# better62/MM-VQA-Healthcare

Measured on AMD Instinct MI355X. Metric: image-question pairs/sec, M3AE-base fine-tune step (fwd+bwd+AdamW) @384px, higher is better.
Workload: dtype bf16

## Files before the change

include/m3ae_hip.h:

```cpp
#ifndef M3AE_HIP_H
#define M3AE_HIP_H

#include <stdint.h>

#ifdef __cplusplus
extern "C" {
#endif

#define M3AE_ABI_VERSION 4

enum { M3AE_F32 = 0, M3AE_BF16 = 1 };
enum { M3AE_ACT_NONE = 0, M3AE_ACT_GELU = 1, M3AE_ACT_QUICKGELU = 2, M3AE_ACT_TANH = 3, M3AE_ACT_RELU = 4,
       M3AE_ACT_MULAUX = 5  };
enum { M3AE_ERR_ARG = -1, M3AE_ERR_UNSUPPORTED = -2, M3AE_ERR_ALIGN = -3, M3AE_ERR_WORKSPACE = -4 };

int m3ae_abi_version(void);
void m3ae_desc_sizes(int64_t out3[3]);
const char* m3ae_last_gemm_path(void);

typedef struct {
    int64_t M, N, K;
    int64_t batch1, batch2;
    const void* A; int64_t a_sm, a_sk, a_sb1, a_sb2;
    const void* B; int64_t b_sk, b_sn, b_sb1, b_sb2;
    void* C;       int64_t c_sm, c_sn, c_sb1, c_sb2;
    int32_t dtype_a, dtype_b, dtype_c;
    float alpha;
    int32_t accumulate;
    const float* bias;
    int32_t act;
    void* preact;
    const void* residual;
    const void* dact_aux;
    int32_t dact;
    int32_t force_generic;
    float* a_rowsum;
    float dropout_p;
    uint64_t dropout_seed;
    int32_t preact_grad;
    int32_t launch_flags;
    const void* dropout_salt;
} m3ae_gemm_desc;
enum { M3AE_GEMM_NO_PERSISTENT = 1,
       M3AE_GEMM_F32_X3 = 2,
       M3AE_GEMM_DETERMINISTIC = 4  };
#define M3AE_GEMM_NT_VARIANT(v) ((((v) + 1) & 0xf) << 8)
#define M3AE_GEMM_TN_VARIANT(v) ((((v) + 1) & 0xf) << 12)
#define M3AE_GEMM_COL_GROUP(g) (((g) & 0xf) << 16)
int m3ae_gemm(const m3ae_gemm_desc* d, void* stream);
int m3ae_gemm_rows(const m3ae_gemm_desc* d, int64_t row_base, int64_t row_step, void* stream);
int64_t m3ae_gemm_det_workspace_bytes(const m3ae_gemm_desc* d);
int m3ae_gemm_det(const m3ae_gemm_desc* d, void* workspace, int64_t workspace_bytes, void* stream);

typedef struct {
    int64_t B, H, Lq, Lk, Dh;
    const void* q; int64_t q_sb, q_sl;
    const void* k; int64_t k_sb, k_sl;
    const void* v; int64_t v_sb, v_sl;
    void* o;       int64_t o_sb, o_sl;
    const float* key_mask;
    const float* pos_bias;
    float scale;
    int32_t causal;
    float* lse; int64_t lse_stride;
    int32_t dtype;
    void* workspace; int64_t workspace_bytes;
    const void* d_o;
    void* dq; void* dk; void* dv;
    float* delta;
    float* d_pos_bias;
    float dropout_p;
    uint64_t dropout_seed;
    const void* dropout_salt;
    int32_t launch_flags;
} m3ae_attn_desc;
enum { M3AE_ATTN_LEGACY_KERNELS = 1,
       M3AE_ATTN_F32_X3 = 2    };
int64_t m3ae_attn_workspace_bytes(const m3ae_attn_desc* d, int backward);
int m3ae_attn_fwd(const m3ae_attn_desc* d, void* stream);
int m3ae_attn_bwd(const m3ae_attn_desc* d, void* stream);
int m3ae_attn_fwd_rows(const m3ae_attn_desc* d, int64_t row_base, int64_t row_step, void* stream);
int m3ae_attn_bwd_rows(const m3ae_attn_desc* d, int64_t row_base, int64_t row_step, void* stream);
int m3ae_attn_probs(const m3ae_attn_desc* d, float* probs, int64_t p_sb, int64_t p_sh, int64_t p_sq, void* stream);

typedef struct {
    int32_t dir;
    int64_t B, Lq, Lk, D, H;
    const void* x;
    const void* y;
    const float* key_mask;
    const void *wq, *wq_t, *wkv, *wkv_t, *wo, *wo_t;
    const float *bq, *bkv, *bo, *ln_g, *ln_b;
    float ln_eps;
    float dropout_p;
    uint64_t seed_attn, seed_hidden;
    void* proj;
    void* prime;
    float* colbias;
    void* probs;
    void* probs_drop;
    float* rowsum;
    void* zctx;
    void* ctx;
    void* s;
    void* out;
    float *mean, *rstd;
    const void* d_out;
    void* dx;
    void* dy;
    float *g_wq, *g_wkv, *g_wo, *g_bq, *g_bkv, *g_bo, *g_ln_g, *g_ln_b;
    void* ws_ds;
    void* ws_dsd;
    void* ws_dscores;
    void* ws_dprime;
    void* ws_dproj;
    void* ws_dz;
    void* ws_dctx;
    float* ws_vec;
    float* ws_ln;
    int32_t launch_flags;
    const void* dropout_salt;
} m3ae_xattn_desc;
enum { M3AE_XATTN_NO_PERSISTENT = 1,
       M3AE_XATTN_LEGACY_CHAIN = 2     };
int m3ae_xattn_supported(const m3ae_xattn_desc* d);
int m3ae_xattn_bwd_supported(const m3ae_xattn_desc* d);
int64_t m3ae_xattn_probs_ld(const m3ae_xattn_desc* d);
int m3ae_xattn_fwd(const m3ae_xattn_desc* d, void* stream);
int m3ae_xattn_bwd(const m3ae_xattn_desc* d, void* stream);
int m3ae_xattn_probs_export(const m3ae_xattn_desc* d, int dropped, float* out, int64_t o_sb, int64_t o_sh, int64_t o_sq,
                            void* stream);

int m3ae_layernorm_fwd(const void* x, const float* gamma, const float* beta, void* y, float* mean, float* rstd,
                       int64_t M, int64_t D, float eps, int dtype, int act, int rms, void* stream);
int64_t m3ae_layernorm_bwd_blocks(int64_t M);
int m3ae_layernorm_bwd(const void* dy, const void* x, const float* gamma, const float* beta, const float* mean,
                       const float* rstd, void* dx, const void* dx_add, float* dgamma, float* dbeta, float* workspace,
                       int64_t M, int64_t D, int dtype, int act, int rms, void* stream);
int m3ae_layernorm_bwd_drop(const void* dy, const void* x, const float* gamma, const float* beta, const float* mean,
                            const float* rstd, void* dx, void* dx_drop, float dropout_p, uint64_t dropout_seed,
                            const void* dropout_salt, float* dgamma, float* dbeta, float* workspace, int64_t M, int64_t D,
                            int dtype, void* stream);
int m3ae_layernorm_bwd_drop_rows(const void* dy, const void* x, const float* gamma, const float* beta, const float* mean,
                                 const float* rstd, void* dx, void* dx_drop, float dropout_p, uint64_t dropout_seed,
                                 const void* dropout_salt, float* dgamma, float* dbeta, float* workspace, int64_t M, int64_t D,
                                 int dtype, int64_t row_base, int64_t row_step, void* stream);
int m3ae_layernorm_fwd_mixed(const float* x, const float* gamma, const float* beta, void* y, float* mean, float* rstd,
                             int64_t M, int64_t D, float eps, void* stream);
int m3ae_layernorm_bwd_mixed(const void* dy, const float* x, const float* gamma, const float* mean, const float* rstd,
                             float* dx, const float* dx_add, void* dx_lo, float* dgamma, float* dbeta, float* workspace,
                             int64_t M, int64_t D, void* stream);
int m3ae_layernorm_bwd_mixed_det(const void* dy, const float* x, const float* gamma, const float* mean, const float* rstd,
                                 float* dx, const float* dx_add, void* dx_lo, float* dgamma, float* dbeta, float* workspace,
                                 int64_t M, int64_t D, void* stream);
int m3ae_dropout(const void* x, void* out, uint8_t* keep_mask, int64_t rows, int64_t cols, float p, uint64_t seed,
                 const void* salt, int dtype, void* stream);
int m3ae_dropout_rows(const void* x, void* out, uint8_t* keep_mask, int64_t rows, int64_t cols, float p, uint64_t seed,
                      const void* salt, int dtype, int64_t row_base, int64_t row_step, void* stream);

int m3ae_colsum(const void* x, float* out, int64_t M, int64_t N, int64_t ldx, int dtype, int accumulate,
                void* stream);

int m3ae_roberta_embed_fwd(const int64_t* ids, const float* word, const float* pos, const float* type, void* out,
                           int64_t B, int64_t S, int64_t D, int64_t pad_id, int dtype, void* stream);
int m3ae_roberta_embed_bwd(const int64_t* ids, const void* d_out, float* d_word, float* d_pos, float* d_type,
                           int64_t B, int64_t S, int64_t D, int64_t pad_id, int dtype, void* stream);

int m3ae_patchify(const float* img, void* out, int64_t B, int64_t R, int64_t P, int dtype, void* stream);
int m3ae_image_normalize_u8(const uint8_t* in, float* out, int64_t B, int64_t H, int64_t W, const float* mean3,
                            const float* std3, void* stream);
int64_t m3ae_image_resample_workspace_bytes(int64_t total_rows, int64_t size);
int m3ae_image_resample_u8(const uint8_t* src, int64_t src_bytes, const int64_t* plan, const int32_t* tab, int64_t tab_ints, int64_t B,
                           int64_t size, uint8_t* workspace, int64_t workspace_bytes, float* out, uint8_t* out_u8,
                           const float* mean3, const float* std3, void* stream);
int m3ae_vit_tokens_fwd(const void* patch, const float* cls, const float* pos, void* out, int64_t B, int64_t G,
                        int64_t D, int dtype, void* stream);
int m3ae_vit_tokens_bwd(const void* d_out, void* d_patch, float* d_cls, float* d_pos, int64_t B, int64_t G,
                        int64_t D, int dtype, void* stream);

int m3ae_bce_logits(const void* logits, const float* targets, float* loss, void* d_logits, int64_t B, int64_t C,
                    float grad_scale, int dtype, void* stream);
int m3ae_xent(const void* logits, const int64_t* labels, float* loss, void* d_logits, float* workspace,
              int64_t rows, int64_t C, int64_t ld, float grad_scale, int dtype, void* stream);

int m3ae_adamw(float* p, const float* g, float* m, float* v, void* shadow_bf16, int64_t n, float lr, float beta1,
               float beta2, float eps, float wd, int64_t step, float grad_scale, const float* hyper_dev, void* stream);

int m3ae_cast_transpose(const float* in, void* out, void* out_t, int64_t R, int64_t C, void* stream);
int m3ae_cast_transpose_batched(const void* jobs_dev, int njobs, int64_t total_tiles, void* stream);
int m3ae_transpose_bf16_batched(const void* jobs_dev, int njobs, int64_t total_tiles, void* stream);
int m3ae_cast(const void* in, void* out, int64_t n, int dtype_in, int dtype_out, void* stream);
int m3ae_zero(void* p, int64_t bytes, void* stream);
int m3ae_add(const void* a, const void* b, void* out, int64_t n, int dtype, void* stream);
int m3ae_act_fwd(const void* x, void* y, int64_t n, int act, int dtype, void* stream);
int m3ae_act_bwd(const void* dy, const void* x_pre, void* dx, int64_t n, int act, int dtype, void* stream);
int m3ae_gather_rows(const void* in, const int64_t* idx, void* out, int64_t n_out, int64_t D, int dtype,
                     void* stream);
int m3ae_scatter_add_rows(const void* d_out, const int64_t* idx, void* d_in, int64_t n_out, int64_t D, int dtype,
                          void* stream);

int m3ae_mask_ranks(const float* noise, int64_t* ids_restore, int64_t* keep_rows, float* mask, int64_t B, int64_t L,
                    int64_t len_keep, void* stream);
int m3ae_mim_targets(const float* img, float* out, int64_t B, int64_t C, int64_t H, int64_t W, int64_t P, int norm_pix,
                     void* stream);
int m3ae_mim_loss_fwd(const void* x, const float* target, const float* mask, float* acc, float* loss, int64_t B, int64_t L,
                      int64_t D, int dtype, void* stream);
int m3ae_mim_loss_bwd(const void* x, const float* target, const float* mask, const float* acc, const float* gout, void* dx,
                      int64_t B, int64_t L, int64_t D, int dtype, void* stream);

enum { M3AE_DET_COLSUM = 0, M3AE_DET_EMBED_BWD = 1, M3AE_DET_BCE = 2, M3AE_DET_XENT = 3, M3AE_DET_MIM = 4 };
int64_t m3ae_det_workspace_bytes(int op, int64_t rows, int64_t cols);
int m3ae_colsum_det(const void* x, float* out, int64_t M, int64_t N, int64_t ldx, int dtype, int accumulate, void* workspace,
                    int64_t workspace_bytes, void* stream);
int m3ae_layernorm_bwd_det(const void* dy, const void* x, const float* gamma, const float* beta, const float* mean,
                           const float* rstd, void* dx, const void* dx_add, float* dgamma, float* dbeta, float* workspace,
                           int64_t M, int64_t D, int dtype, int act, int rms, void* stream);
int m3ae_layernorm_bwd_drop_det(const void* dy, const void* x, const float* gamma, const float* beta, const float* mean,
                                const float* rstd, void* dx, void* dx_drop, float dropout_p, uint64_t dropout_seed,
                                const void* dropout_salt, float* dgamma, float* dbeta, float* workspace, int64_t M, int64_t D,
                                int dtype, void* stream);
int m3ae_roberta_embed_bwd_det(const int64_t* ids, const void* d_out, float* d_word, float* d_pos, float* d_type, int64_t B,
                               int64_t S, int64_t D, int64_t pad_id, int dtype, void* workspace, int64_t workspace_bytes,
                               void* stream);
int m3ae_bce_logits_det(const void* logits, const float* targets, float* loss, void* d_logits, int64_t B, int64_t C,
                        float grad_scale, int dtype, void* workspace, int64_t workspace_bytes, void* stream);
int m3ae_xent_det(const void* logits, const int64_t* labels, float* loss, void* d_logits, int64_t rows, int64_t C, int64_t ld,
                  float grad_scale, int dtype, void* workspace, int64_t workspace_bytes, void* stream);
int m3ae_mim_loss_fwd_det(const void* x, const float* target, const float* mask, float* acc, float* loss, int64_t B, int64_t L,
                          int64_t D, int dtype, void* workspace, int64_t workspace_bytes, void* stream);

int64_t m3ae_beam_topk_workspace_bytes(int64_t B, int64_t nb, int64_t V, int64_t chunk);
int m3ae_beam_topk(const float* logits, int64_t ld, const float* beam_scores, int64_t B, int64_t nb, int64_t V, int64_t chunk,
                   void* workspace, int64_t workspace_bytes, float* top_s, int32_t* top_i, void* stream);
int m3ae_beam_step(const float* top_s, const int32_t* top_i, const int64_t* ids_in, int64_t* ids_out, int64_t* last_tok,
                   float* beam_scores, int64_t* order, int32_t* done, int32_t* n_hyp, double* hyp_score, int32_t* hyp_len,
                   int64_t* hyp_tok, int32_t* open_count, int64_t* err, int64_t B, int64_t nb, int64_t V, int64_t max_length,
                   int64_t cur_len, int64_t eos, int64_t pad, double div, void* stream);
int m3ae_beam_finalize(const int64_t* ids, const float* beam_scores, const int32_t* done, int32_t* n_hyp, double* hyp_score,
                       int32_t* hyp_len, int64_t* hyp_tok, int64_t* seq, int64_t* len, int64_t B, int64_t nb, int64_t max_length,
                       int64_t cur_len, int64_t eos, int64_t pad, double div, void* stream);

int m3ae_expand_samples(const void* in, const int64_t* src, void* out, int64_t n_out, int64_t n_in, int64_t R, int dtype,
                        void* stream);
int m3ae_segment_sum_rows(const void* d_out, const int64_t* offsets, const int64_t* members, void* d_in, int64_t n_in,
                          int64_t n_out, int64_t R, int dtype, void* stream);

int m3ae_selftest(int32_t* out, void* stream);

#ifdef __cplusplus
}
#endif
#endif
```

mm-vqa-healthcare_amd/csrc/norm.hip:

```cpp
#include "common.h"
#include "det_fold.h"
#include "launch.h"
#include <type_traits>

namespace {

template <typename T> DEVINL void ld4(const T* p, float* x);
template <> DEVINL void ld4<float>(const float* p, float* x) {
    const f32x4 v = *(const f32x4*)p;
    x[0] = v[0]; x[1] = v[1]; x[2] = v[2]; x[3] = v[3];
}
template <> DEVINL void ld4<bf16_t>(const bf16_t* p, float* x) {
    const u32x2 v = *(const u32x2*)p;
    x[0] = __uint_as_float(v[0] << 16); x[1] = __uint_as_float(v[0] & 0xffff0000u);
    x[2] = __uint_as_float(v[1] << 16); x[3] = __uint_as_float(v[1] & 0xffff0000u);
}
template <typename T> struct Raw4;
template <> struct Raw4<float> {
    f32x4 v;
    DEVINL void ld(const float* p) { v = *(const f32x4*)p; }
    DEVINL void get(float* x) const { x[0] = v[0]; x[1] = v[1]; x[2] = v[2]; x[3] = v[3]; }
};
template <> struct Raw4<bf16_t> {
    u32x2 v;
    DEVINL void ld(const bf16_t* p) { v = *(const u32x2*)p; }
    DEVINL void get(float* x) const {
        x[0] = __uint_as_float(v[0] << 16); x[1] = __uint_as_float(v[0] & 0xffff0000u);
        x[2] = __uint_as_float(v[1] << 16); x[3] = __uint_as_float(v[1] & 0xffff0000u);
    }
};
template <typename T> DEVINL void st4(T* p, const float* x);
template <> DEVINL void st4<float>(float* p, const float* x) { *(f32x4*)p = (f32x4){x[0], x[1], x[2], x[3]}; }
template <> DEVINL void st4<bf16_t>(bf16_t* p, const float* x) {
    *(u32x2*)p = (u32x2){pack2bf(x[0], x[1]), pack2bf(x[2], x[3])};
}

template <typename T, int CPL, typename TO = T>
__global__ __launch_bounds__(256) void ln_fwd_kernel(const T* x, const float* gamma, const float* beta, TO* y,
                                                     float* mean_o, float* rstd_o, int64_t M, int D, float eps,
                                                     int act, int rms) {
    const int lane = threadIdx.x & 63;
    const int nch = D >> 2;
    const int64_t stride = (int64_t)gridDim.x * 4;
    int64_t row = (int64_t)blockIdx.x * 4 + (threadIdx.x >> 6);
    Raw4<T> raw[CPL];
    if (row < M) {
#pragma unroll
        for (int c = 0; c < CPL; ++c) {
            const int ch = lane + c * 64;
            if (ch < nch) raw[c].ld(x + row * D + ch * 4);
        }
    }
    for (; row < M; row += stride) {
        float v[CPL][4];
        float sum = 0.f;
#pragma unroll
        for (int c = 0; c < CPL; ++c) {
            const int ch = lane + c * 64;
            if (ch < nch) {
                raw[c].get(v[c]);
                sum += (v[c][0] + v[c][1]) + (v[c][2] + v[c][3]);
            } else {
                v[c][0] = v[c][1] = v[c][2] = v[c][3] = 0.f;
            }
        }
        const int64_t nrow = row + stride;
        if (nrow < M) {
#pragma unroll
            for (int c = 0; c < CPL; ++c) {
                const int ch = lane + c * 64;
                if (ch < nch) raw[c].ld(x + nrow * D + ch * 4);
            }
        }
        const float mean = rms ? 0.f : wave_sum(sum) / (float)D;
        float sq = 0.f;
#pragma unroll
        for (int c = 0; c < CPL; ++c) {
            const int ch = lane + c * 64;
            if (ch < nch) {
#pragma unroll
                for (int t = 0; t < 4; ++t) {
                    const float dlt = v[c][t] - mean;
                    sq += dlt * dlt;
                }
            }
        }
        const float var = wave_sum(sq) / (float)D;
        const float rstd = 1.0f / sqrtf(var + eps);
        if (lane == 0) {
            if (mean_o) mean_o[row] = mean;
            if (rstd_o) rstd_o[row] = rstd;
        }
        TO* yr = y + row * D;
#pragma unroll
        for (int c = 0; c < CPL; ++c) {
            const int ch = lane + c * 64;
            if (ch < nch) {
                float g[4], b[4] = {0.f, 0.f, 0.f, 0.f}, o[4];
                ld4<float>(gamma + ch * 4, g);
                if (beta) ld4<float>(beta + ch * 4, b);
#pragma unroll
                for (int t = 0; t < 4; ++t) o[t] = act_fwd((v[c][t] - mean) * rstd * g[t] + b[t], act);
                st4<TO>(yr + ch * 4, o);
            }
        }
    }
}

template <int NP>
__global__ __launch_bounds__(256) void ln_fwd_pair_kernel(const bf16_t* x, const float* gamma, const float* beta, bf16_t* y,
                                                          float* mean_o, float* rstd_o, int64_t M, float eps) {
    constexpr int D = NP * 256, PPR = D / 8;
    const int lane = threadIdx.x & 63;
    const int64_t npair = (M + 1) >> 1;
    const int64_t stride = (int64_t)gridDim.x * 4;
    int64_t pr = (int64_t)blockIdx.x * 4 + (threadIdx.x >> 6);
    int sel[NP], col[NP];
#pragma unroll
    for (int c = 0; c < NP; ++c) {
        const int p = lane + 64 * c;
        sel[c] = p >= PPR;
        col[c] = (p - sel[c] * PPR) * 8;
    }
    u32x4 raw[NP];
    auto load = [&](int64_t pair) {
        const bf16_t* base = x + pair * 2 * D;
        const bool two = pair * 2 + 1 < M;
#pragma unroll
        for (int c = 0; c < NP; ++c)
            raw[c] = (two || !sel[c]) ? *(const u32x4*)(base + (lane + 64 * c) * 8) : (u32x4){0u, 0u, 0u, 0u};
    };
    if (pr < npair) load(pr);
    for (; pr < npair; pr += stride) {
        float v[NP][8];
        float s0 = 0.f, s1 = 0.f;
#pragma unroll
        for (int c = 0; c < NP; ++c) {
            float t = 0.f;
#pragma unroll
            for (int q = 0; q < 4; ++q) {
                v[c][2 * q] = __uint_as_float(raw[c][q] << 16);
                v[c][2 * q + 1] = __uint_as_float(raw[c][q] & 0xffff0000u);
                t += v[c][2 * q] + v[c][2 * q + 1];
            }
            if (sel[c]) s1 += t; else s0 += t;
        }
        const int64_t cur = pr;
        if (pr + stride < npair) load(pr + stride);
        const float m0 = wave_sum(s0) / (float)D, m1 = wave_sum(s1) / (float)D;
        float q0 = 0.f, q1 = 0.f;
#pragma unroll
        for (int c = 0; c < NP; ++c) {
            const float mu = sel[c] ? m1 : m0;
            float t = 0.f;
#pragma unroll
            for (int e = 0; e < 8; ++e) { const float dlt = v[c][e] - mu; t += dlt * dlt; }
            if (sel[c]) q1 += t; else q0 += t;
        }
        const float r0 = 1.0f / sqrtf(wave_sum(q0) / (float)D + eps), r1 = 1.0f / sqrtf(wave_sum(q1) / (float)D + eps);
        const bool two = cur * 2 + 1 < M;
        if (lane == 0) {
            if (mean_o) { mean_o[cur * 2] = m0; if (two) mean_o[cur * 2 + 1] = m1; }
            if (rstd_o) { rstd_o[cur * 2] = r0; if (two) rstd_o[cur * 2 + 1] = r1; }
        }
        bf16_t* yb = y + cur * 2 * D;
#pragma unroll
        for (int c = 0; c < NP; ++c) {
            if (!two && sel[c]) continue;
            const float mu = sel[c] ? m1 : m0, rs = sel[c] ? r1 : r0;
            const f32x4 g0 = *(const f32x4*)(gamma + col[c]), g1 = *(const f32x4*)(gamma + col[c] + 4);
            f32x4 b0 = {0.f, 0.f, 0.f, 0.f}, b1 = {0.f, 0.f, 0.f, 0.f};
            if (beta) { b0 = *(const f32x4*)(beta + col[c]); b1 = *(const f32x4*)(beta + col[c] + 4); }
            float o[8];
#pragma unroll
            for (int e = 0; e < 4; ++e) {
                o[e] = (v[c][e] - mu) * rs * g0[e] + b0[e];
                o[4 + e] = (v[c][4 + e] - mu) * rs * g1[e] + b1[e];
            }
            *(u32x4*)(yb + (lane + 64 * c) * 8) = (u32x4){pack2bf(o[0], o[1]), pack2bf(o[2], o[3]), pack2bf(o[4], o[5]), pack2bf(o[6], o[7])};
        }
    }
}

template <typename T, int CPL, bool ACT, typename TD = T>
__global__ __launch_bounds__(256) void ln_bwd_kernel(const TD* dy, const T* x, const float* gamma, const float* beta,
                                                     const float* mean_i, const float* rstd_i, T* dx, const T* dx_add,
                                                     float* part, int64_t M, int D, int act, int rms, T* dx_drop,
                                                     DropState drop, bf16_t* dx_lo) {
    if (dx_drop) drop_resolve(drop);
    extern __shared__ float red[];
    const int lane = threadIdx.x & 63, wave = threadIdx.x >> 6;
    const int nch = D >> 2;
    float dg[CPL][4], db[CPL][4], g[CPL][4], bt[ACT ? CPL : 1][4];
#pragma unroll
    for (int c = 0; c < CPL; ++c) {
        const int ch = lane + c * 64;
#pragma unroll
        for (int t = 0; t < 4; ++t) { dg[c][t] = 0.f; db[c][t] = 0.f; g[c][t] = 0.f; if (ACT) bt[c][t] = 0.f; }
        if (ch < nch) {
            ld4<float>(gamma + ch * 4, g[c]);
            if (ACT && beta) ld4<float>(beta + ch * 4, bt[c]);
        }
    }
    const int64_t stride = (int64_t)gridDim.x * 4;
    int64_t row = (int64_t)blockIdx.x * 4 + wave;
    Raw4<T> xr[CPL];
    Raw4<TD> dr[CPL];
    float mean_n = 0.f, rstd_n = 0.f;
    if (row < M) {
#pragma unroll
        for (int c = 0; c < CPL; ++c) {
            const int ch = lane + c * 64;
            if (ch < nch) { xr[c].ld(x + row * D + ch * 4); dr[c].ld(dy + row * D + ch * 4); }
        }
        mean_n = rms ? 0.f : mean_i[row];
        rstd_n = rstd_i[row];
    }
    for (; row < M; row += stride) {
        const float mean = mean_n;
        const float rstd = rstd_n;
        float xh[CPL][4], dxh[CPL][4];
        float s1 = 0.f, s2 = 0.f;
#pragma unroll
        for (int c = 0; c < CPL; ++c) {
            const int ch = lane + c * 64;
            if (ch < nch) {
                float xv[4], dv[4];
                xr[c].get(xv);
                dr[c].get(dv);
#pragma unroll
                for (int t = 0; t < 4; ++t) {
                    const float h = (xv[t] - mean) * rstd;
                    float d = dv[t];
                    if (ACT) d *= act_bwd(h * g[c][t] + bt[c][t], act);
                    dg[c][t] += d * h;
                    db[c][t] += d;
                    const float dh = d * g[c][t];
                    xh[c][t] = h;
                    dxh[c][t] = dh;
                    s1 += dh;
                    s2 += dh * h;
                }
            } else {
#pragma unroll
                for (int t = 0; t < 4; ++t) { xh[c][t] = 0.f; dxh[c][t] = 0.f; }
            }
        }
        const int64_t nrow = row + stride;
        if (nrow < M) {
#pragma unroll
            for (int c = 0; c < CPL; ++c) {
                const int ch = lane + c * 64;
                if (ch < nch) { xr[c].ld(x + nrow * D + ch * 4); dr[c].ld(dy + nrow * D + ch * 4); }
            }
            mean_n = rms ? 0.f : mean_i[nrow];
            rstd_n = rstd_i[nrow];
        }
        const float c1 = rms ? 0.f : wave_sum(s1) / (float)D;
        const float c2 = wave_sum(s2) / (float)D;
#pragma unroll
        for (int c = 0; c < CPL; ++c) {
            const int ch = lane + c * 64;
            if (ch < nch) {
                float o[4];
#pragma unroll
                for (int t = 0; t < 4; ++t) o[t] = rstd * (dxh[c][t] - c1 - xh[c][t] * c2);
                if (dx_drop) {
                    float od[4];
#pragma unroll
                    for (int t = 0; t < 4; ++t) od[t] = o[t];
                    drop_apply4(drop, (uint64_t)(drop_row(drop, row) * D + ch * 4), od);
                    st4<T>(dx_drop + row * D + ch * 4, od);
                }
                if (dx_add) {
                    float e[4];
                    ld4<T>(dx_add + row * D + ch * 4, e);
#pragma unroll
                    for (int t = 0; t < 4; ++t) o[t] += e[t];
                }
                st4<T>(dx + row * D + ch * 4, o);
                if constexpr (!std::is_same<TD, T>::value) {
                    if (dx_lo) st4<bf16_t>(dx_lo + row * D + ch * 4, o);
                }
            }
        }
    }
#pragma unroll
    for (int c = 0; c < CPL; ++c) {
        const int ch = lane + c * 64;
        if (ch < nch) {
#pragma unroll
            for (int t = 0; t < 4; ++t) {
                red[(wave * 2 + 0) * D + ch * 4 + t] = dg[c][t];
                red[(wave * 2 + 1) * D + ch * 4 + t] = db[c][t];
            }
        }
    }
    __syncthreads();
    for (int i = threadIdx.x; i < 2 * D; i += 256) {
        const int which = i / D, col = i - which * D;
        float s = 0.f;
#pragma unroll
        for (int w = 0; w < 4; ++w) s += red[(w * 2 + which) * D + col];
        part[((int64_t)blockIdx.x * 2 + which) * D + col] = s;
    }
}

__global__ __launch_bounds__(256) void ln_bwd_reduce_kernel(const float* part, float* dgamma, float* dbeta, int nblk,
                                                            int D) {
    __shared__ float red[8][33];
    const int cl = threadIdx.x & 31, rl = threadIdx.x >> 5;
    const int i = blockIdx.x * 32 + cl;
    const int b0 = blockIdx.y * 64;
    const int b1 = b0 + 64 < nblk ? b0 + 64 : nblk;
    float s = 0.f;
    if (i < 2 * D) {
        const int which = i / D, col = i - which * D;
        for (int b = b0 + rl; b < b1; b += 8) s += part[((int64_t)b * 2 + which) * D + col];
    }
    red[rl][cl] = s;
    __syncthreads();
    if (rl == 0 && i < 2 * D) {
        float t = 0.f;
#pragma unroll
        for (int r = 0; r < 8; ++r) t += red[r][cl];
        const int which = i / D, col = i - which * D;
        if (which == 0) atomicAdd(dgamma + col, t);
        else if (dbeta) atomicAdd(dbeta + col, t);
    }
}

inline int ln_bwd_fold(const float* part, float* dgamma, float* dbeta, int nblk, int D, int det, hipStream_t s) {
    if (det)
        det_fold(part, dgamma, dbeta, nblk, dbeta ? 2 * D : D, 2 * D, D, 1.0f, 1, s);
    else
        hipLaunchKernelGGL(ln_bwd_reduce_kernel, dim3((unsigned)cdiv(2 * D, 32), (unsigned)cdiv(nblk, 64)), dim3(256), 0, s, part, dgamma,
                           dbeta, nblk, D);
    return hip_launch_status();
}

template <typename K> int resident_blocks(K kernel, size_t lds) {
    int per_cu = 0;
    if (hipOccupancyMaxActiveBlocksPerMultiprocessor(&per_cu, kernel, 256, lds) != hipSuccess || per_cu <= 0) return 1 << 30;
    return per_cu * device_cus();
}
template <typename T, int CPL, typename TO = T>
int launch_fwd(const void* x, const float* g, const float* b, void* y, float* mean, float* rstd, int64_t M, int D,
               float eps, int act, int rms, hipStream_t s) {
    static const int cap = resident_blocks(ln_fwd_kernel<T, CPL, TO>, 0);
    const int64_t want = cdiv(M, 4);
    hipLaunchKernelGGL((ln_fwd_kernel<T, CPL, TO>), dim3((unsigned)(want < cap ? want : cap)), dim3(256), 0, s, (const T*)x, g, b,
                       (TO*)y, mean, rstd, M, D, eps, act, rms);
    return hip_launch_status();
}
template <typename T, int CPL, typename TD = T>
int launch_bwd(const void* dy, const void* x, const float* g, const float* b, const float* mean, const float* rstd,
               void* dx, const void* dx_add, float* part, int* nblk_io, int64_t M, int D, int act, int rms, hipStream_t s,
               void* dx_drop = nullptr, DropState drop = DropState{}, void* dx_lo = nullptr) {
    const size_t lds = (size_t)8 * D * sizeof(float);
    static int cap_act = 0, cap_plain = 0, cap_d = -1;
    constexpr bool MIXED = !std::is_same<TD, T>::value;
    if (cap_d != D) {
        if constexpr (!MIXED) cap_act = resident_blocks(ln_bwd_kernel<T, CPL, true, TD>, lds);
        cap_plain = resident_blocks(ln_bwd_kernel<T, CPL, false, TD>, lds);
        cap_d = D;
    }
    const int cap = act != M3AE_ACT_NONE ? cap_act : cap_plain;
    const int nblk = *nblk_io < cap ? *nblk_io : cap;
    *nblk_io = nblk;
    if constexpr (MIXED) {
        if (act != M3AE_ACT_NONE) return M3AE_ERR_UNSUPPORTED;
    }
    if (act != M3AE_ACT_NONE) {
        if constexpr (!MIXED)
            hipLaunchKernelGGL((ln_bwd_kernel<T, CPL, true, TD>), dim3((unsigned)nblk), dim3(256), lds, s,
                               (const TD*)dy, (const T*)x, g, b, mean, rstd, (T*)dx, (const T*)dx_add, part, M, D, act, rms,
                               (T*)dx_drop, drop, (bf16_t*)dx_lo);
    } else
        hipLaunchKernelGGL((ln_bwd_kernel<T, CPL, false, TD>), dim3((unsigned)nblk), dim3(256), lds, s,
                           (const TD*)dy, (const T*)x, g, b, mean, rstd, (T*)dx, (const T*)dx_add, part, M, D, act, rms,
                           (T*)dx_drop, drop, (bf16_t*)dx_lo);
    return hip_launch_status();
}

template <typename T, int CPL>
int launch_fwd_mixed(const void* x, const float* g, const float* b, void* y, float* mean, float* rstd, int64_t M, int D, float eps,
                     hipStream_t s) {
    return launch_fwd<T, CPL, bf16_t>(x, g, b, y, mean, rstd, M, D, eps, M3AE_ACT_NONE, 0, s);
}
template <typename T, int CPL>
int launch_bwd_mixed(const void* dy, const void* x, const float* g, const float* mean, const float* rstd, void* dx, const void* dx_add,
                     void* dx_lo, float* part, int* nblk_io, int64_t M, int D, hipStream_t s) {
    return launch_bwd<T, CPL, bf16_t>(dy, x, g, nullptr, mean, rstd, dx, dx_add, part, nblk_io, M, D, M3AE_ACT_NONE, 0, s, nullptr,
                                      DropState{}, dx_lo);
}

#define DISPATCH_CPL(FN, T, ...)                                                  \
    do {                                                                          \
        const int cpl = (int)cdiv(D / 4, 64);                                     \
        if (cpl <= 1) return FN<T, 1>(__VA_ARGS__);                               \
        if (cpl <= 2) return FN<T, 2>(__VA_ARGS__);                               \
        if (cpl <= 3) return FN<T, 3>(__VA_ARGS__);                               \
        if (cpl <= 4) return FN<T, 4>(__VA_ARGS__);                               \
        if (cpl <= 6) return FN<T, 6>(__VA_ARGS__);                               \
        if (cpl <= 8) return FN<T, 8>(__VA_ARGS__);                               \
        if (cpl <= 16) return FN<T, 16>(__VA_ARGS__);                             \
        return M3AE_ERR_UNSUPPORTED;                                              \
    } while (0)

}

template <int NP>
int launch_fwd_pair(const void* x, const float* g, const float* b, void* y, float* mean, float* rstd, int64_t M, float eps,
                    hipStream_t s) {
    static const int cap = resident_blocks(ln_fwd_pair_kernel<NP>, 0);
    const int64_t want = cdiv((M + 1) / 2, 4);
    hipLaunchKernelGGL((ln_fwd_pair_kernel<NP>), dim3((unsigned)(want < cap ? want : cap)), dim3(256), 0, s, (const bf16_t*)x, g, b,
                       (bf16_t*)y, mean, rstd, M, eps);
    return hip_launch_status();
}

extern "C" int m3ae_layernorm_fwd(const void* x, const float* gamma, const float* beta, void* y, float* mean,
                                  float* rstd, int64_t M, int64_t D, float eps, int dtype, int act, int rms,
                                  void* stream) {
    if (!x || !gamma || !y || M <= 0 || D <= 0) return M3AE_ERR_ARG;
    if (D % 4 != 0 || D > 4096) return M3AE_ERR_UNSUPPORTED;
    hipStream_t s = (hipStream_t)stream;
    const bool pair_off = (rms & 2) != 0;
    rms &= 1;
    if (dtype == M3AE_BF16 && act == M3AE_ACT_NONE && !rms && M >= 1024 && ((((uintptr_t)x) | ((uintptr_t)y)) & 15) == 0 &&
        ((((uintptr_t)gamma) | ((uintptr_t)beta)) & 15) == 0 && !pair_off) {
        if (D == 512) return launch_fwd_pair<2>(x, gamma, beta, y, mean, rstd, M, eps, s);
        if (D == 768) return launch_fwd_pair<3>(x, gamma, beta, y, mean, rstd, M, eps, s);
        if (D == 1024) return launch_fwd_pair<4>(x, gamma, beta, y, mean, rstd, M, eps, s);
    }
    if (dtype == M3AE_F32) DISPATCH_CPL(launch_fwd, float, x, gamma, beta, y, mean, rstd, M, (int)D, eps, act, rms, s);
    if (dtype == M3AE_BF16) DISPATCH_CPL(launch_fwd, bf16_t, x, gamma, beta, y, mean, rstd, M, (int)D, eps, act, rms, s);
    return M3AE_ERR_UNSUPPORTED;
}

extern "C" int64_t m3ae_layernorm_bwd_blocks(int64_t M) {
    int64_t n = cdiv(M, 4);
    return n < 1024 ? n : 1024;
}

static int layernorm_bwd_impl(const void* dy, const void* x, const float* gamma, const float* beta, const float* mean,
                              const float* rstd, void* dx, const void* dx_add, float* dgamma, float* dbeta, float* workspace,
                              int64_t M, int64_t D, int dtype, int act, int rms, void* stream, int det) {
    if (!dy || !x || !gamma || !rstd || !dx || !workspace || M <= 0) return M3AE_ERR_ARG;
    if (D % 4 != 0 || D > 2048) return M3AE_ERR_UNSUPPORTED;
    hipStream_t s = (hipStream_t)stream;
    int nblk = (int)m3ae_layernorm_bwd_blocks(M);
    int rc = M3AE_ERR_UNSUPPORTED;
    auto run = [&]() -> int {
        if (dtype == M3AE_F32)
            DISPATCH_CPL(launch_bwd, float, dy, x, gamma, beta, mean, rstd, dx, dx_add, workspace, &nblk, M, (int)D, act, rms, s);
        if (dtype == M3AE_BF16)
            DISPATCH_CPL(launch_bwd, bf16_t, dy, x, gamma, beta, mean, rstd, dx, dx_add, workspace, &nblk, M, (int)D, act, rms, s);
        return M3AE_ERR_UNSUPPORTED;
    };
    rc = run();
    if (rc) return rc;
    if (!dgamma) return 0;
    return ln_bwd_fold(workspace, dgamma, dbeta, nblk, (int)D, det, s);
}
extern "C" int m3ae_layernorm_bwd(const void* dy, const void* x, const float* gamma, const float* beta,
                                  const float* mean, const float* rstd, void* dx, const void* dx_add, float* dgamma,
                                  float* dbeta, float* workspace, int64_t M, int64_t D, int dtype, int act, int rms,
                                  void* stream) {
    return layernorm_bwd_impl(dy, x, gamma, beta, mean, rstd, dx, dx_add, dgamma, dbeta, workspace, M, D, dtype, act, rms, stream, 0);
}
extern "C" int m3ae_layernorm_bwd_det(const void* dy, const void* x, const float* gamma, const float* beta,
                                      const float* mean, const float* rstd, void* dx, const void* dx_add, float* dgamma,
                                      float* dbeta, float* workspace, int64_t M, int64_t D, int dtype, int act, int rms,
                                      void* stream) {
    return layernorm_bwd_impl(dy, x, gamma, beta, mean, rstd, dx, dx_add, dgamma, dbeta, workspace, M, D, dtype, act, rms, stream, 1);
}

static int layernorm_bwd_drop_impl(const void* dy, const void* x, const float* gamma, const float* beta, const float* mean,
                                   const float* rstd, void* dx, void* dx_drop, float dropout_p, uint64_t dropout_seed,
                                   const void* dropout_salt, float* dgamma, float* dbeta, float* workspace, int64_t M, int64_t D,
                                   int dtype, void* stream, int det, DropRows rows = DropRows{0, 1}) {
    if (!dy || !x || !gamma || !rstd || !dx || !dx_drop || !workspace || M <= 0) return M3AE_ERR_ARG;
    if (!drop_rows_ok(rows, M, D)) return M3AE_ERR_ARG;
    if (D % 4 != 0 || D > 2048) return M3AE_ERR_UNSUPPORTED;
    hipStream_t s = (hipStream_t)stream;
    int nblk = (int)m3ae_layernorm_bwd_blocks(M);
    const DropState drop = make_drop(dropout_p, dropout_seed, dropout_salt, rows);
    auto run = [&]() -> int {
        if (dtype == M3AE_F32)
            DISPATCH_CPL(launch_bwd, float, dy, x, gamma, beta, mean, rstd, dx, nullptr, workspace, &nblk, M, (int)D, 0, 0, s, dx_drop, drop);
        if (dtype == M3AE_BF16)
            DISPATCH_CPL(launch_bwd, bf16_t, dy, x, gamma, beta, mean, rstd, dx, nullptr, workspace, &nblk, M, (int)D, 0, 0, s, dx_drop, drop);
        return M3AE_ERR_UNSUPPORTED;
    };
    int rc = run();
    if (rc) return rc;
    if (!dgamma) return 0;
    return ln_bwd_fold(workspace, dgamma, dbeta, nblk, (int)D, det, s);
}
extern "C" int m3ae_layernorm_bwd_drop(const void* dy, const void* x, const float* gamma, const float* beta,
                                       const float* mean, const float* rstd, void* dx, void* dx_drop, float dropout_p,
                                       uint64_t dropout_seed, const void* dropout_salt, float* dgamma, float* dbeta,
                                       float* workspace, int64_t M, int64_t D, int dtype, void* stream) {
    return layernorm_bwd_drop_impl(dy, x, gamma, beta, mean, rstd, dx, dx_drop, dropout_p, dropout_seed, dropout_salt, dgamma, dbeta,
                                   workspace, M, D, dtype, stream, 0);
}
extern "C" int m3ae_layernorm_bwd_drop_rows(const void* dy, const void* x, const float* gamma, const float* beta,
                                            const float* mean, const float* rstd, void* dx, void* dx_drop, float dropout_p,
                                            uint64_t dropout_seed, const void* dropout_salt, float* dgamma, float* dbeta,
                                            float* workspace, int64_t M, int64_t D, int dtype, int64_t row_base, int64_t row_step,
                                            void* stream) {
    return layernorm_bwd_drop_impl(dy, x, gamma, beta, mean, rstd, dx, dx_drop, dropout_p, dropout_seed, dropout_salt, dgamma, dbeta,
                                   workspace, M, D, dtype, stream, 0, DropRows{row_base, row_step});
}
extern "C" int m3ae_layernorm_bwd_drop_det(const void* dy, const void* x, const float* gamma, const float* beta,
                                           const float* mean, const float* rstd, void* dx, void* dx_drop, float dropout_p,
                                           uint64_t dropout_seed, const void* dropout_salt, float* dgamma, float* dbeta,
                                           float* workspace, int64_t M, int64_t D, int dtype, void* stream) {
    return layernorm_bwd_drop_impl(dy, x, gamma, beta, mean, rstd, dx, dx_drop, dropout_p, dropout_seed, dropout_salt, dgamma, dbeta,
                                   workspace, M, D, dtype, stream, 1);
}

extern "C" int m3ae_layernorm_fwd_mixed(const float* x, const float* gamma, const float* beta, void* y, float* mean, float* rstd,
                                        int64_t M, int64_t D, float eps, void* stream) {
    if (!x || !gamma || !y || M <= 0 || D <= 0) return M3AE_ERR_ARG;
    if (D % 4 != 0 || D > 2048) return M3AE_ERR_UNSUPPORTED;
    if (((((uintptr_t)x) | ((uintptr_t)gamma) | ((uintptr_t)beta)) & 15) != 0 || (((uintptr_t)y) & 7) != 0) return M3AE_ERR_ALIGN;
    hipStream_t s = (hipStream_t)stream;
    DISPATCH_CPL(launch_fwd_mixed, float, x, gamma, beta, y, mean, rstd, M, (int)D, eps, s);
}

static int layernorm_bwd_mixed_impl(const void* dy, const float* x, const float* gamma, const float* mean, const float* rstd,
                                    float* dx, const float* dx_add, void* dx_lo, float* dgamma, float* dbeta, float* workspace,
                                    int64_t M, int64_t D, void* stream, int det) {
    if (!dy || !x || !gamma || !mean || !rstd || !dx || !workspace || M <= 0) return M3AE_ERR_ARG;
    if (D % 4 != 0 || D > 2048) return M3AE_ERR_UNSUPPORTED;
    if (((((uintptr_t)x) | ((uintptr_t)dx) | ((uintptr_t)dx_add) | ((uintptr_t)gamma)) & 15) != 0 ||
        ((((uintptr_t)dy) | ((uintptr_t)dx_lo)) & 7) != 0)
        return M3AE_ERR_ALIGN;
    hipStream_t s = (hipStream_t)stream;
    int nblk = (int)m3ae_layernorm_bwd_blocks(M);
    auto run = [&]() -> int {
        DISPATCH_CPL(launch_bwd_mixed, float, dy, x, gamma, mean, rstd, dx, dx_add, dx_lo, workspace, &nblk, M, (int)D, s);
    };
    int rc = run();
    if (rc) return rc;
    if (!dgamma) return 0;
    return ln_bwd_fold(workspace, dgamma, dbeta, nblk, (int)D, det, s);
}
extern "C" int m3ae_layernorm_bwd_mixed(const void* dy, const float* x, const float* gamma, const float* mean, const float* rstd,
                                        float* dx, const float* dx_add, void* dx_lo, float* dgamma, float* dbeta, float* workspace,
                                        int64_t M, int64_t D, void* stream) {
    return layernorm_bwd_mixed_impl(dy, x, gamma, mean, rstd, dx, dx_add, dx_lo, dgamma, dbeta, workspace, M, D, stream, 0);
}
extern "C" int m3ae_layernorm_bwd_mixed_det(const void* dy, const float* x, const float* gamma, const float* mean, const float* rstd,
                                            float* dx, const float* dx_add, void* dx_lo, float* dgamma, float* dbeta,
                                            float* workspace, int64_t M, int64_t D, void* stream) {
    return layernorm_bwd_mixed_impl(dy, x, gamma, mean, rstd, dx, dx_add, dx_lo, dgamma, dbeta, workspace, M, D, stream, 1);
}
```

mm-vqa-healthcare_amd/csrc/xattn.hip:

```cpp
#include "xattn_common.h"
#include "launch.h"

namespace {

enum { FORM_K = 0, FORM_T = 1 };
enum { XE_STORE = 0, XE_DENSE = 1, XE_SOFTMAX32 = 2, XE_SOFTMAXROW = 3, XE_ATOMIC = 4, XE_DSOFT = 5 };

struct XgArgs {
    const bf16_t* A; int64_t lda, a_sb;
    const bf16_t* B; int64_t ldb, b_sb;
    int M, N, K;
    int tiles_m, tiles_n;
    bf16_t* C; int64_t ldc, c_sb;
    bf16_t* C2;
    int rdiv, rmul;
    float alpha;
    const float* bias; int64_t bias_sb;
    const float* rowscale; int64_t rs_sm, rs_sb;
    int rs_div, rs_mul;
    int b_rows;
    const bf16_t* residual;
    const float* colbias; int64_t cb_sb;
    float* rowsum_out;
    int n_valid;
// ... 827 lines not shown
            u32x4 v[4];
#pragma unroll
            for (int u = 0; u < 4; ++u) v[u] = *(const u32x4*)(p + (int64_t)(i + 16 * u) * R);
#pragma unroll
            for (int u = 0; u < 4; ++u) add(v[u]);
        }
        for (; i < I; i += 16) add(*(const u32x4*)(p + (int64_t)i * R));
    }
#pragma unroll
    for (int t = 0; t < 8; ++t) part[rl][cg][t] = acc[t];
    __syncthreads();
    if (rl == 0 && n0 < R) {
#pragma unroll
        for (int t = 0; t < 8; ++t) {
            float s_ = 0.f;
#pragma unroll
            for (int r = 0; r < 16; ++r) s_ += part[r][cg][t];
            out[(int64_t)b * R + n0 + t] = scale * s_;
        }
    }
}

__global__ __launch_bounds__(256) void xattn_headvec_kernel(const float* w, const bf16_t* X, int64_t ldx, float* out, int Mrows,
                                                            int T, int R, int w_t, int w_h, int dh) {
    __shared__ float part[256];
    const int h = blockIdx.x, d = threadIdx.x % dh, sub = threadIdx.x / dh, nsub = 256 / dh;
    const int r0 = blockIdx.y * 256, r1 = r0 + 256 < Mrows ? r0 + 256 : Mrows;
    float acc = 0.f;
    if (sub < nsub)
        for (int m = r0 + sub; m < r1; m += nsub) {
            const float wt = w ? w[(int64_t)(m / T) * R + (m % T) * w_t + h * w_h] : 1.0f;
            acc = fmaf(wt, bf2f(X[(int64_t)m * ldx + h * dh + d]), acc);
        }
    part[threadIdx.x] = acc;
    __syncthreads();
    if (sub == 0) {
        for (int q = 1; q < nsub; ++q) acc += part[q * dh + d];
        atomicAdd(out + h * dh + d, acc);
    }
}

__global__ __launch_bounds__(256) void xattn_rowdot_kernel(const bf16_t* dZ, const bf16_t* Z, const bf16_t* dctx, const float* bv,
                                                           const float* rowsum, float* delta, float* radd, int64_t rows, int D,
                                                           int T, int H, int dh) {
    const int lane = threadIdx.x & 63;
    const int64_t row = (int64_t)blockIdx.x * 4 + (threadIdx.x >> 6);
    if (row >= rows) return;
    const bf16_t* a = dZ + row * D;
    const bf16_t* z = Z + row * D;
    float acc = 0.f;
    for (int c = lane * 8; c < D; c += 512) {
        const u32x4 x = *(const u32x4*)(a + c), y = *(const u32x4*)(z + c);
#pragma unroll
        for (int q = 0; q < 4; ++q) {
            acc = fmaf(__uint_as_float(x[q] << 16), __uint_as_float(y[q] << 16), acc);
            acc = fmaf(__uint_as_float(x[q] & 0xffff0000u), __uint_as_float(y[q] & 0xffff0000u), acc);
        }
    }
    acc = wave_sum(acc);
    float ra = 0.f;
    if (radd) {
        const int R = T * H, r = (int)(row % R), b = (int)(row / R), t = r / H, h = r % H;
        float s_ = 0.f;
        for (int d = lane; d < dh; d += 64) s_ = fmaf(bf2f(dctx[((int64_t)b * T + t) * D + h * dh + d]), bv[h * dh + d], s_);
        ra = wave_sum(s_);
    }
    if (lane == 0) {
        if (radd) radd[row] = ra;
        delta[row] = acc + (radd ? ra * rowsum[row] : 0.f);
    }
}

}

#ifdef M3AE_XG_TRACE
extern "C" int m3ae_xg_trace_dump(uint64_t* host_out) {
    g_trace_next = 0;
    return (int)hipMemcpyFromSymbol(host_out, HIP_SYMBOL(g_xg_trace), sizeof(uint64_t) * 8 * 16 * 4096);
}
#endif

extern "C" int m3ae_xattn_supported(const m3ae_xattn_desc* d) {
    if (!d) return 0;
    const int64_t T = d->dir == 0 ? d->Lq : d->Lk, I = d->dir == 0 ? d->Lk : d->Lq;
    if (d->H <= 0 || d->D % d->H != 0) return 0;
    const int64_t dh = d->D / d->H;
    if (I < 1 || dh % 32 != 0 || d->D % 128 != 0) return 0;
    if (d->dir == 0) return ((T == 32 || T == 64) && I <= 640) ? 1 : 0;
    if (d->launch_flags & M3AE_XATTN_LEGACY_CHAIN) return (T == 32 && I <= 640) ? 1 : 0;
    return ((T == 32 || T == 64) && d->H * T == (T == 32 ? 384 : 768) && d->D % 256 == 0) ? 1 : 0;
}

extern "C" int m3ae_xattn_bwd_supported(const m3ae_xattn_desc* d) {
    if (!m3ae_xattn_supported(d)) return 0;
    return 1;
}

extern "C" int64_t m3ae_xattn_probs_ld(const m3ae_xattn_desc* d) {
    return d->dir == 0 ? 640 : d->H * d->Lk;
}

#define XCHK(e) do { const int rc_ = (e); if (rc_ != 0) return rc_; } while (0)

namespace {
m3ae_gemm_desc dense_desc(const m3ae_xattn_desc& d, const void* A, const void* B, void* C) {
    m3ae_gemm_desc g{};
    g.batch1 = g.batch2 = 1;
    g.dtype_a = g.dtype_b = g.dtype_c = M3AE_BF16;
    g.alpha = 1.0f;
    g.launch_flags = (d.launch_flags & M3AE_XATTN_NO_PERSISTENT) ? M3AE_GEMM_NO_PERSISTENT : 0;
    g.A = A; g.B = B; g.C = C; g.c_sn = 1;
    return g;
}
int64_t text_rows(const m3ae_xattn_desc& d) { return d.B * (d.dir == 0 ? d.Lq : d.Lk); }
m3ae_gemm_desc dense_fwd(const m3ae_xattn_desc& d, int64_t N, const void* X, const void* W, const float* bias, void* Y) {
    m3ae_gemm_desc g = dense_desc(d, X, W, Y);
    g.M = text_rows(d); g.N = N; g.K = d.D;
    g.a_sm = d.D; g.a_sk = 1; g.b_sk = 1; g.b_sn = d.D; g.c_sm = N; g.bias = bias;
    return g;
}
m3ae_gemm_desc dense_wgrad(const m3ae_xattn_desc& d, int64_t N, const void* dY, const void* X, float* dW, float* db) {
    m3ae_gemm_desc g = dense_desc(d, dY, X, dW);
    g.M = N; g.N = d.D; g.K = text_rows(d);
    g.a_sm = 1; g.a_sk = N; g.b_sk = d.D; g.b_sn = 1; g.c_sm = d.D; g.dtype_c = M3AE_F32; g.accumulate = 1; g.a_rowsum = db;
    return g;
}
m3ae_gemm_desc dense_dgrad(const m3ae_xattn_desc& d, int64_t K, const void* dY, const void* Wt, void* dX, const void* residual = nullptr) {
    m3ae_gemm_desc g = dense_desc(d, dY, Wt, dX);
    g.M = text_rows(d); g.N = d.D; g.K = K;
    g.a_sm = K; g.a_sk = 1; g.b_sk = 1; g.b_sn = K; g.c_sm = d.D; g.residual = residual;
    return g;
}
}

extern "C" int m3ae_xattn_fwd(const m3ae_xattn_desc* dp, void* stream) {
    if (!dp || !m3ae_xattn_supported(dp)) return M3AE_ERR_UNSUPPORTED;
    const m3ae_xattn_desc& d = *dp;
    hipStream_t s = (hipStream_t)stream;
    const int B = (int)d.B, H = (int)d.H, D = (int)d.D, dh = D / H;
    const int Lq = (int)d.Lq, Lk = (int)d.Lk;
    const float scale = 1.0f / sqrtf((float)dh);
    const bool drop = d.dropout_p > 0.f;
    if (!d.x || !d.y || !d.proj || !d.prime || !d.s || !d.out) return M3AE_ERR_ARG;
    if (d.dir == 0 && (!d.probs || (drop && !d.probs_drop))) return M3AE_ERR_ARG;

    const DropState drop_attn = make_drop(d.dropout_p, d.seed_attn, d.dropout_salt);
    const DropState drop_hidden = make_drop(d.dropout_p, d.seed_hidden, d.dropout_salt);

    if (d.dir == 0) {
        const int T = Lq, I = Lk, R = T * H;
        if (!d.zctx || !d.ctx || (drop && !d.rowsum)) return M3AE_ERR_ARG;
        const m3ae_gemm_desc g = dense_fwd(d, D, d.x, d.wq, d.bq, d.proj);
        XCHK(m3ae_gemm(&g, stream));
        {
            XgArgs a{};
            a.A = (const bf16_t*)d.proj; a.lda = D; a.a_sb = dh;
            a.B = (const bf16_t*)d.wkv_t; a.ldb = 2 * D; a.b_sb = dh;
            a.M = B * T; a.N = D; a.K = dh;
            a.C = (bf16_t*)d.prime; a.ldc = (int64_t)H * D; a.c_sb = D;
            a.alpha = scale;
            XCHK(launch_xbuild(a, H, s));
        }
        {
            XgArgs a{};
            a.A = (const bf16_t*)d.prime; a.lda = D; a.a_sb = (int64_t)R * D;
            a.B = (const bf16_t*)d.y; a.ldb = D; a.b_sb = (int64_t)I * D;
            a.M = R; a.N = I; a.K = D;
            a.C = (bf16_t*)d.probs; a.ldc = 640; a.c_sb = (int64_t)R * 640;
            a.C2 = drop ? (bf16_t*)d.probs_drop : nullptr;
            a.alpha = 1.0f;
            a.colbias = d.key_mask; a.cb_sb = I;
            a.rowsum_out = drop ? d.rowsum : nullptr;
            a.n_valid = I;
            a.has_drop = drop; a.drop = drop_attn;
            a.H = H; a.Lq = T; a.drop_ld = (int)drop_ld(I);
            XCHK((launch_xg<128, 640, 2, 3, 0, FORM_K, FORM_K, XE_SOFTMAXROW>(a, B, s)));
        }
        {
            XgArgs a{};
            a.A = (const bf16_t*)(drop ? d.probs_drop : d.probs); a.lda = 640; a.a_sb = (int64_t)R * 640;
            a.B = (const bf16_t*)d.y; a.ldb = D; a.b_sb = (int64_t)I * D;
            a.M = R; a.N = D; a.K = I;
            a.C = (bf16_t*)d.zctx; a.ldc = D; a.c_sb = (int64_t)R * D;
            a.alpha = 1.0f;
            XCHK((launch_xg<128, 384, 2, 4, 4, FORM_K, FORM_T, XE_STORE>(a, B, s)));
        }
        {
            XgArgs a{};
            a.A = (const bf16_t*)d.zctx; a.lda = (int64_t)H * D; a.a_sb = D;
            a.B = (const bf16_t*)d.wkv + (int64_t)D * D; a.ldb = D; a.b_sb = (int64_t)dh * D;
            a.M = B * T; a.N = dh; a.K = D;
            a.C = (bf16_t*)d.ctx; a.ldc = D; a.c_sb = dh;
            a.alpha = 1.0f;
            a.bias = d.bkv + D; a.bias_sb = dh;
            if (drop) { a.rowscale = d.rowsum; a.rs_sm = H; a.rs_sb = 1; }
            XCHK((launch_xg<384, 128, 4, 4, 4, FORM_K, FORM_K, XE_STORE>(a, H, s)));
        }
        m3ae_gemm_desc o = dense_fwd(d, D, d.ctx, d.wo, d.bo, d.s);
        o.residual = d.x;
        o.dropout_p = d.dropout_p; o.dropout_seed = d.seed_hidden; o.dropout_salt = d.dropout_salt;
        XCHK(m3ae_gemm(&o, stream));
    } else {
        const int I = Lq, T = Lk, R = H * T;
        if (!d.colbias) return M3AE_ERR_ARG;
        const m3ae_gemm_desc g = dense_fwd(d, 2 * D, d.y, d.wkv, d.bkv, d.proj);
        XCHK(m3ae_gemm(&g, stream));
        bf16_t* Kp = (bf16_t*)d.prime;
        bf16_t* Vp = Kp + (int64_t)B * R * D;
        bool fused_build = false;
        {
            XgArgs a{};
            a.A = (const bf16_t*)d.proj; a.lda = 2 * D; a.a_sb = dh;
            a.B = (const bf16_t*)d.wq_t; a.ldb = D; a.b_sb = dh;
            a.M = B * T; a.N = D; a.K = dh;
            a.C = Kp; a.ldc = D; a.c_sb = (int64_t)T * D;
            a.rdiv = T; a.rmul = R;
            a.alpha = scale;
            fused_build = dh == 64;
            if (fused_build) {
                XbPair pr{};
                pr.A2 = (const bf16_t*)d.proj + D; pr.B2 = (const bf16_t*)d.wo; pr.C2 = Vp; pr.alpha2 = 1.0f;
                pr.bq = d.bq; pr.mask = d.key_mask; pr.cb = d.colbias; pr.T = T; pr.H = H; pr.scale = scale;
                XCHK(launch_xbuild_pair(a, pr, s));
            } else {
                XCHK(launch_xbuild(a, H, s));
                a.A = (const bf16_t*)d.proj + D;
                a.B = (const bf16_t*)d.wo; a.ldb = D; a.b_sb = dh;
                a.C = Vp;
                a.alpha = 1.0f;
                XCHK(launch_xbuild(a, H, s));
            }
        }
        if (!fused_build) {
            const int rows = B * T;
            hipLaunchKernelGGL(xattn_colbias_kernel, dim3((rows + 3) / 4), dim3(256), 0, s, (const bf16_t*)d.proj,
                               (int64_t)2 * D, d.bq, d.key_mask, d.colbias, rows, T, H, dh, scale);
            XCHK(hip_launch_status());
        }
        if (!(d.launch_flags & M3AE_XATTN_LEGACY_CHAIN)) {
            if (drop && d.probs && !d.probs_drop) return M3AE_ERR_ARG;
            XfArgs f{};
            f.X = (const bf16_t*)d.x; f.Kp = Kp; f.Vp = Vp; f.colbias = d.colbias; f.bo = d.bo;
            f.S = (bf16_t*)d.s; f.P = (bf16_t*)d.probs; f.Pd = drop ? (bf16_t*)d.probs_drop : nullptr;
            f.B = B; f.I = I; f.D = D; f.H = H;
            f.has_drop = drop; f.drop_a = drop_attn; f.drop_h = drop_hidden;
            f.drop_ld = (int)drop_ld(T);
            XCHK(m3ae_xflash_dir1(f, T, s));
        } else {
            if (T != 32 || !d.probs || (drop && !d.probs_drop)) return M3AE_ERR_UNSUPPORTED;
            {
                XgArgs a{};
                a.A = (const bf16_t*)d.x; a.lda = D; a.a_sb = (int64_t)I * D;
                a.B = Kp; a.ldb = D; a.b_sb = (int64_t)R * D;
                a.M = I; a.N = R; a.K = D;
                a.C = (bf16_t*)d.probs; a.ldc = R; a.c_sb = (int64_t)I * R;
                a.C2 = drop ? (bf16_t*)d.probs_drop : nullptr;
                a.alpha = 1.0f;
                a.colbias = d.colbias; a.cb_sb = R;
                a.has_drop = drop; a.drop = drop_attn;
                a.H = H; a.Lq = I; a.drop_ld = (int)drop_ld(T);
                XCHK((launch_xg<128, 384, 2, 4, 4, FORM_K, FORM_K, XE_SOFTMAX32>(a, B, s)));
            }
            {
                XgArgs a{};
                a.A = (const bf16_t*)(drop ? d.probs_drop : d.probs); a.lda = R; a.a_sb = (int64_t)I * R;
                a.B = Vp; a.ldb = D; a.b_sb = (int64_t)R * D;
                a.M = I; a.N = D; a.K = R;
                a.C = (bf16_t*)d.s; a.ldc = D;
                a.bias = d.bo;
                a.residual = (const bf16_t*)d.x;
                a.has_drop = drop; a.drop = drop_hidden;
                XCHK((launch_xg<128, 384, 2, 4, 4, FORM_K, FORM_T, XE_DENSE>(a, B, s)));
            }
        }
    }
    return m3ae_layernorm_fwd(d.s, d.ln_g, d.ln_b, d.out, d.mean, d.rstd, (int64_t)B * Lq, D, d.ln_eps, M3AE_BF16,
                              M3AE_ACT_NONE, 0, stream);
}

namespace {
void pick_split(XgArgs& a, int nchunks, int tiles) {
    int ks = 256 / (tiles > 0 ? tiles : 1);
    if (ks > nchunks / 8) ks = nchunks / 8;
    if (ks < 1) ks = 1;
    a.kchunks = (nchunks + ks - 1) / ks;
    a.ksplit = (nchunks + a.kchunks - 1) / a.kchunks;
}
}

extern "C" int m3ae_xattn_bwd(const m3ae_xattn_desc* dp, void* stream) {
    if (!dp || !m3ae_xattn_bwd_supported(dp)) return M3AE_ERR_UNSUPPORTED;
    const m3ae_xattn_desc& d = *dp;
    hipStream_t s = (hipStream_t)stream;
    const int B = (int)d.B, H = (int)d.H, D = (int)d.D, dh = D / H;
    const int Lq = (int)d.Lq, Lk = (int)d.Lk;
    const float scale = 1.0f / sqrtf((float)dh);
    const bool drop = d.dropout_p > 0.f;
    if (!d.d_out || !d.dx || !d.x || !d.y || !d.proj || !d.prime || !d.probs || !d.s || !d.mean || !d.rstd || !d.ws_ds ||
        !d.ws_dscores || !d.ws_dprime || !d.ws_dproj || !d.ws_vec || !d.ws_ln || (drop && (!d.probs_drop || !d.ws_dsd)) ||
        !d.g_wq || !d.g_wkv || !d.g_wo || !d.g_bq || !d.g_bkv || !d.g_bo)
        return M3AE_ERR_ARG;
    const int64_t Mq = (int64_t)B * Lq;
    const void* dsd = d.ws_ds;
    if (drop) {
        XCHK(m3ae_layernorm_bwd_drop(d.d_out, d.s, d.ln_g, d.ln_b, d.mean, d.rstd, d.ws_ds, d.ws_dsd, d.dropout_p, d.seed_hidden,
                                     d.dropout_salt, d.g_ln_g, d.g_ln_b, d.ws_ln, Mq, D, M3AE_BF16, stream));
        dsd = d.ws_dsd;
    } else {
        XCHK(m3ae_layernorm_bwd(d.d_out, d.s, d.ln_g, d.ln_b, d.mean, d.rstd, d.ws_ds, nullptr, d.g_ln_g, d.g_ln_b, d.ws_ln, Mq, D,
                                M3AE_BF16, M3AE_ACT_NONE, 0, stream));
    }
    const bf16_t* Pd = (const bf16_t*)(drop ? d.probs_drop : d.probs);
    const DropState drop_attn = make_drop(d.dropout_p, d.seed_attn, d.dropout_salt);

    if (d.dir == 1) {
        const int I = Lq, T = Lk, R = H * T;
        if (!d.colbias) return M3AE_ERR_ARG;
        const bf16_t* Kp = (const bf16_t*)d.prime;
        const bf16_t* Vp = Kp + (int64_t)B * R * D;
        bf16_t* dKp = (bf16_t*)d.ws_dprime;
        bf16_t* dVp = dKp + (int64_t)B * R * D;
        bf16_t* dS = (bf16_t*)d.ws_dscores;
        bf16_t* dkv = (bf16_t*)d.ws_dproj;
        float* dcb = d.ws_vec;
        XCHK(m3ae_colsum(dsd, d.g_bo, Mq, D, D, M3AE_BF16, 1, stream));
        {
            XgArgs a{};
            a.A = (const bf16_t*)dsd; a.lda = D; a.a_sb = (int64_t)I * D;
            a.B = Vp; a.ldb = D; a.b_sb = (int64_t)R * D;
            a.M = I; a.N = R; a.K = D;
            a.C = dS; a.ldc = R; a.c_sb = (int64_t)I * R;
            a.P = (const bf16_t*)d.probs;
            a.has_drop = drop; a.drop = drop_attn;
            a.drop_mode = 1; a.H = H; a.Lq = I; a.drop_ld = (int)drop_ld(T); a.tkeys = T;
            if (T == 32) XCHK((launch_xg<128, 384, 2, 4, 4, FORM_K, FORM_K, XE_DSOFT>(a, B, s)));
            else XCHK((launch_xg<128, 256, 2, 4, 4, FORM_K, FORM_K, XE_DSOFT>(a, B, s)));
        }
        {
            XgArgs a{};
            a.A = Pd; a.lda = R; a.a_sb = (int64_t)I * R;
            a.B = (const bf16_t*)dsd; a.ldb = D; a.b_sb = (int64_t)I * D;
            a.M = R; a.N = D; a.K = I;
            a.C = dVp; a.ldc = D; a.c_sb = (int64_t)R * D; a.alpha = 1.0f;
            XCHK((launch_xg<128, 384, 2, 4, 4, FORM_T, FORM_T, XE_STORE>(a, B, s)));
            a.A = dS; a.B = (const bf16_t*)d.x; a.C = dKp;
            XCHK((launch_xg<128, 384, 2, 4, 4, FORM_T, FORM_T, XE_STORE>(a, B, s)));
        }
        {
            XgArgs a{};
            a.A = dS; a.lda = R; a.a_sb = (int64_t)I * R;
            a.B = Kp; a.ldb = D; a.b_sb = (int64_t)R * D;
            a.M = I; a.N = D; a.K = R;
            a.C = (bf16_t*)d.dx; a.ldc = D;
            a.residual = (const bf16_t*)d.ws_ds;
            XCHK((launch_xg<128, 384, 2, 4, 4, FORM_K, FORM_T, XE_DENSE>(a, B, s)));
        }
        hipLaunchKernelGGL(xattn_colsum_kernel, dim3((R + 127) / 128, B), dim3(256), 0, s, dS, dcb, I, R, scale);
        XCHK(hip_launch_status());
        {
            XgArgs a{};
            a.A = dKp; a.lda = D; a.a_sb = (int64_t)T * D; a.a_div = T; a.a_mul = R;
            a.B = (const bf16_t*)d.wq; a.ldb = D; a.b_sb = (int64_t)dh * D;
            a.M = B * T; a.N = dh; a.K = D;
            a.C = dkv; a.ldc = 2 * D; a.c_sb = dh; a.alpha = scale;
            a.bias = d.bq; a.bias_sb = dh;
            a.rowscale = dcb; a.rs_sm = 1; a.rs_sb = T; a.rs_div = T; a.rs_mul = R;
            XCHK((launch_xg<384, 128, 4, 4, 4, FORM_K, FORM_K, XE_STORE, 1>(a, H, s)));
            XgArgs v{};
            v.A = dVp; v.lda = D; v.a_sb = (int64_t)T * D; v.a_div = T; v.a_mul = R;
            v.B = (const bf16_t*)d.wo_t; v.ldb = D; v.b_sb = (int64_t)dh * D;
            v.M = B * T; v.N = dh; v.K = D;
            v.C = dkv + D; v.ldc = 2 * D; v.c_sb = dh; v.alpha = 1.0f;
            XCHK((launch_xg<384, 128, 4, 4, 4, FORM_K, FORM_K, XE_STORE, 1>(v, H, s)));
        }
        {
            XgArgs a{};
            a.A = (const bf16_t*)d.proj; a.lda = 2 * D; a.a_sb = dh;
            a.B = dKp; a.ldb = D; a.b_sb = (int64_t)T * D; a.b_div = T; a.b_mul = R;
            a.M = dh; a.N = D; a.K = B * T;
            a.Cf = d.g_wq; a.ldc = D; a.c_sb = (int64_t)dh * D; a.alpha = scale;
            pick_split(a, (B * T + 31) / 32, H * ((D + 383) / 384));
            XCHK((launch_xg<128, 384, 2, 4, 4, FORM_T, FORM_T, XE_ATOMIC, 1>(a, H, s)));
            XgArgs o{};
            o.A = dVp; o.lda = D; o.a_sb = (int64_t)T * D; o.a_div = T; o.a_mul = R;
            o.B = (const bf16_t*)d.proj + D; o.ldb = 2 * D; o.b_sb = dh;
            o.M = D; o.N = dh; o.K = B * T;
            o.Cf = d.g_wo; o.ldc = D; o.c_sb = dh; o.alpha = 1.0f;
            pick_split(o, (B * T + 31) / 32, H * ((D + 383) / 384));
            XCHK((launch_xg<384, 128, 4, 4, 4, FORM_T, FORM_T, XE_ATOMIC, 1>(o, H, s)));
        }
        hipLaunchKernelGGL(xattn_headvec_kernel, dim3(H, (B * T + 255) / 256), dim3(256), 0, s, (const float*)dcb,
                           (const bf16_t*)d.proj, (int64_t)2 * D, d.g_bq, B * T, T, R, 1, T, dh);
        XCHK(hip_launch_status());
        const m3ae_gemm_desc w = dense_wgrad(d, 2 * D, dkv, d.y, d.g_wkv, d.g_bkv);
        XCHK(m3ae_gemm(&w, stream));
        if (d.dy) {
            const m3ae_gemm_desc y = dense_dgrad(d, 2 * D, dkv, d.wkv_t, d.dy);
            XCHK(m3ae_gemm(&y, stream));
        }
        return 0;
    }

    const int T = Lq, I = Lk, R = T * H;
    if (!d.zctx || !d.ctx || !d.ws_dz || !d.ws_dctx || (drop && !d.rowsum)) return M3AE_ERR_ARG;
    bf16_t* dctx = (bf16_t*)d.ws_dctx;
    bf16_t* dZ = (bf16_t*)d.ws_dz;
    bf16_t* dS = (bf16_t*)d.ws_dscores;
    bf16_t* dQp = (bf16_t*)d.ws_dprime;
    bf16_t* dq = (bf16_t*)d.ws_dproj;
    float* delta = d.ws_vec;
    float* radd = drop ? d.ws_vec + (int64_t)B * R : nullptr;
    const m3ae_gemm_desc wo_grad = dense_wgrad(d, D, dsd, d.ctx, d.g_wo, d.g_bo), dctx_grad = dense_dgrad(d, D, dsd, d.wo_t, dctx);
    XCHK(m3ae_gemm(&wo_grad, stream));
    XCHK(m3ae_gemm(&dctx_grad, stream));
    {
        XgArgs a{};
        a.A = dctx; a.lda = D; a.a_sb = dh;
        a.B = (const bf16_t*)d.wkv_t + D; a.ldb = 2 * D; a.b_sb = dh;
        a.M = B * T; a.N = D; a.K = dh;
        a.C = dZ; a.ldc = (int64_t)H * D; a.c_sb = D; a.alpha = 1.0f;
        XCHK(launch_xbuild(a, H, s));
        XgArgs w{};
        w.A = dctx; w.lda = D; w.a_sb = dh;
        w.B = (const bf16_t*)d.zctx; w.ldb = (int64_t)H * D; w.b_sb = D;
        w.M = dh; w.N = D; w.K = B * T;
        w.Cf = d.g_wkv + (int64_t)D * D; w.ldc = D; w.c_sb = (int64_t)dh * D; w.alpha = 1.0f;
        pick_split(w, (B * T + 31) / 32, H * ((D + 383) / 384));
        XCHK((launch_xg<128, 384, 2, 4, 4, FORM_T, FORM_T, XE_ATOMIC>(w, H, s)));
        hipLaunchKernelGGL(xattn_headvec_kernel, dim3(H, (B * T + 255) / 256), dim3(256), 0, s,
                           (const float*)(drop ? d.rowsum : nullptr), (const bf16_t*)dctx, (int64_t)D, d.g_bkv + D, B * T, T, R, H, 1, dh);
        XCHK(hip_launch_status());
    }
    hipLaunchKernelGGL(xattn_rowdot_kernel, dim3((unsigned)(((int64_t)B * R + 3) / 4)), dim3(256), 0, s, (const bf16_t*)dZ,
                       (const bf16_t*)d.zctx, (const bf16_t*)dctx, d.bkv + D, (const float*)d.rowsum, delta, radd, (int64_t)B * R, D, T, H, dh);
    XCHK(hip_launch_status());
    {
        XgArgs a{};
        a.A = dZ; a.lda = D; a.a_sb = (int64_t)R * D;
        a.B = (const bf16_t*)d.y; a.ldb = D; a.b_sb = (int64_t)I * D; a.b_rows = I;
        a.M = R; a.N = 640; a.K = D;
        a.C = dS; a.ldc = 640; a.c_sb = (int64_t)R * 640;
        a.P = (const bf16_t*)d.probs; a.delta = delta; a.radd = radd;
        a.has_drop = drop; a.drop = drop_attn;
        a.drop_mode = 0; a.H = H; a.Lq = T; a.drop_ld = (int)drop_ld(I);
        XCHK((launch_xg<128, 640, 2, 3, 0, FORM_K, FORM_K, XE_DSOFT>(a, B, s)));
    }
    {
        XgArgs a{};
        a.A = dS; a.lda = 640; a.a_sb = (int64_t)R * 640;
        a.B = (const bf16_t*)d.y; a.ldb = D; a.b_sb = (int64_t)I * D;
        a.M = R; a.N = D; a.K = I;
        a.C = dQp; a.ldc = D; a.c_sb = (int64_t)R * D; a.alpha = 1.0f;
        XCHK((launch_xg<128, 384, 2, 4, 4, FORM_K, FORM_T, XE_STORE>(a, B, s)));
    }
    if (d.dy) {
        XgArgs a{};
        a.A = Pd; a.lda = 640; a.a_sb = (int64_t)R * 640;
        a.B = dZ; a.ldb = D; a.b_sb = (int64_t)R * D;
        a.M = I; a.N = D; a.K = 2 * R;
        a.A2 = dS; a.B2 = (const bf16_t*)d.prime; a.k_switch = R / 32;
        a.C = (bf16_t*)d.dy; a.ldc = D; a.c_sb = (int64_t)I * D; a.alpha = 1.0f;
        XCHK((launch_xg<128, 384, 2, 4, 4, FORM_T, FORM_T, XE_STORE, 1>(a, B, s)));
    }
    {
        XgArgs a{};
        a.A = dQp; a.lda = (int64_t)H * D; a.a_sb = D;
        a.B = (const bf16_t*)d.wkv; a.ldb = D; a.b_sb = (int64_t)dh * D;
        a.M = B * T; a.N = dh; a.K = D;
        a.C = dq; a.ldc = D; a.c_sb = dh; a.alpha = scale;
        XCHK((launch_xg<384, 128, 4, 4, 4, FORM_K, FORM_K, XE_STORE>(a, H, s)));
        XgArgs w{};
        w.A = (const bf16_t*)d.proj; w.lda = D; w.a_sb = dh;
        w.B = dQp; w.ldb = (int64_t)H * D; w.b_sb = D;
        w.M = dh; w.N = D; w.K = B * T;
        w.Cf = d.g_wkv; w.ldc = D; w.c_sb = (int64_t)dh * D; w.alpha = scale;
        pick_split(w, (B * T + 31) / 32, H * ((D + 383) / 384));
        XCHK((launch_xg<128, 384, 2, 4, 4, FORM_T, FORM_T, XE_ATOMIC>(w, H, s)));
    }
    const m3ae_gemm_desc wq_grad = dense_wgrad(d, D, dq, d.x, d.g_wq, d.g_bq), dx_grad = dense_dgrad(d, D, dq, d.wq_t, d.dx, d.ws_ds);
    XCHK(m3ae_gemm(&wq_grad, stream));
    XCHK(m3ae_gemm(&dx_grad, stream));
    return 0;
}

namespace {
__global__ __launch_bounds__(256) void xattn_probs_export_kernel(const bf16_t* __restrict__ src, int64_t s_b, int64_t s_h,
                                                                  int64_t s_q, float* __restrict__ out, int64_t o_sb, int64_t o_sh,
                                                                  int64_t o_sq, int64_t H, int64_t Lq, int64_t Lk, int64_t rows) {
    const int lane = threadIdx.x & 63;
    const int64_t row = (int64_t)blockIdx.x * 4 + __builtin_amdgcn_readfirstlane(threadIdx.x >> 6);
    if (row >= rows) return;
    const int64_t q = row % Lq, bh = row / Lq;
    const int64_t h = bh % H, b = bh / H;
    const bf16_t* sp = src + b * s_b + h * s_h + q * s_q;
    float* op = out + b * o_sb + h * o_sh + q * o_sq;
    for (int64_t k = lane; k < Lk; k += 64) op[k] = bf2f(sp[k]);
}
}

extern "C" int m3ae_xattn_probs_export(const m3ae_xattn_desc* d, int dropped, float* out, int64_t o_sb, int64_t o_sh, int64_t o_sq,
                                       void* stream) {
    if (!d || !out) return M3AE_ERR_ARG;
    const void* src = dropped ? d->probs_drop : d->probs;
    if (!src || d->B <= 0 || d->H <= 0 || d->Lq <= 0 || d->Lk <= 0) return M3AE_ERR_ARG;
    if (o_sq < d->Lk || o_sh <= 0 || o_sb <= 0) return M3AE_ERR_ARG;
    const int64_t H = d->H, Lq = d->Lq, Lk = d->Lk;
    int64_t s_b, s_h, s_q;
    if (d->dir == 0) {
        if (Lk > 640) return M3AE_ERR_UNSUPPORTED;
        s_h = 640; s_q = H * 640; s_b = Lq * H * 640;
    } else if (d->dir == 1) {
        s_h = Lk; s_q = H * Lk; s_b = Lq * H * Lk;
    } else {
        return M3AE_ERR_ARG;
    }
    const int64_t rows = d->B * H * Lq;
    hipLaunchKernelGGL(xattn_probs_export_kernel, dim3((unsigned)cdiv(rows, 4)), dim3(256), 0, (hipStream_t)stream,
                       (const bf16_t*)src, s_b, s_h, s_q, out, o_sb, o_sh, o_sq, H, Lq, Lk, rows);
    return hip_launch_status();
}
```

mm-vqa-healthcare_amd/m3ae_amd/_lib.py:

```python
import ctypes as C
import os

_PKG = os.path.dirname(os.path.abspath(__file__))
DIAGNOSTIC = os.environ.get("M3AE_DIAGNOSTIC_LIB", "") == "1"
LIB_PATH = os.path.join(_PKG, "lib_diag" if DIAGNOSTIC else "lib", "libm3ae_hip.so")

F32, BF16 = 0, 1
ACT_NONE, ACT_GELU, ACT_QUICKGELU, ACT_TANH, ACT_RELU, ACT_MULAUX = 0, 1, 2, 3, 4, 5

vp, i64, i32, f32 = C.c_void_p, C.c_int64, C.c_int32, C.c_float


class GemmDesc(C.Structure):
    _fields_ = [
        ("M", i64), ("N", i64), ("K", i64), ("batch1", i64), ("batch2", i64),
        ("A", vp), ("a_sm", i64), ("a_sk", i64), ("a_sb1", i64), ("a_sb2", i64),
        ("B", vp), ("b_sk", i64), ("b_sn", i64), ("b_sb1", i64), ("b_sb2", i64),
        ("C", vp), ("c_sm", i64), ("c_sn", i64), ("c_sb1", i64), ("c_sb2", i64),
        ("dtype_a", i32), ("dtype_b", i32), ("dtype_c", i32),
        ("alpha", f32), ("accumulate", i32), ("bias", vp), ("act", i32), ("preact", vp), ("residual", vp),
        ("dact_aux", vp), ("dact", i32), ("force_generic", i32), ("a_rowsum", vp),
        ("dropout_p", f32), ("dropout_seed", C.c_uint64), ("preact_grad", i32), ("launch_flags", i32), ("dropout_salt", vp),
    ]


class AttnDesc(C.Structure):
    _fields_ = [
        ("B", i64), ("H", i64), ("Lq", i64), ("Lk", i64), ("Dh", i64),
        ("q", vp), ("q_sb", i64), ("q_sl", i64),
        ("k", vp), ("k_sb", i64), ("k_sl", i64),
        ("v", vp), ("v_sb", i64), ("v_sl", i64),
        ("o", vp), ("o_sb", i64), ("o_sl", i64),
        ("key_mask", vp), ("pos_bias", vp), ("scale", f32), ("causal", i32),
        ("lse", vp), ("lse_stride", i64), ("dtype", i32), ("workspace", vp), ("workspace_bytes", i64),
        ("d_o", vp), ("dq", vp), ("dk", vp), ("dv", vp), ("delta", vp), ("d_pos_bias", vp),
        ("dropout_p", f32), ("dropout_seed", C.c_uint64), ("dropout_salt", vp), ("launch_flags", i32),
    ]


class XattnDesc(C.Structure):
    _fields_ = [
        ("dir", i32), ("B", i64), ("Lq", i64), ("Lk", i64), ("D", i64), ("H", i64),
        ("x", vp), ("y", vp), ("key_mask", vp),
        ("wq", vp), ("wq_t", vp), ("wkv", vp), ("wkv_t", vp), ("wo", vp), ("wo_t", vp),
        ("bq", vp), ("bkv", vp), ("bo", vp), ("ln_g", vp), ("ln_b", vp),
        ("ln_eps", f32), ("dropout_p", f32), ("seed_attn", C.c_uint64), ("seed_hidden", C.c_uint64),
        ("proj", vp), ("prime", vp), ("colbias", vp), ("probs", vp), ("probs_drop", vp), ("rowsum", vp),
        ("zctx", vp), ("ctx", vp), ("s", vp), ("out", vp), ("mean", vp), ("rstd", vp),
        ("d_out", vp), ("dx", vp), ("dy", vp),
        ("g_wq", vp), ("g_wkv", vp), ("g_wo", vp), ("g_bq", vp), ("g_bkv", vp), ("g_bo", vp), ("g_ln_g", vp), ("g_ln_b", vp),
        ("ws_ds", vp), ("ws_dsd", vp), ("ws_dscores", vp), ("ws_dprime", vp), ("ws_dproj", vp), ("ws_dz", vp), ("ws_dctx", vp),
        ("ws_vec", vp), ("ws_ln", vp), ("launch_flags", i32), ("dropout_salt", vp),
    ]


GEMM_NO_PERSISTENT, GEMM_F32_X3, GEMM_DETERMINISTIC = 1, 2, 4
DET_COLSUM, DET_EMBED_BWD, DET_BCE, DET_XENT, DET_MIM = 0, 1, 2, 3, 4
ATTN_LEGACY_KERNELS, ATTN_F32_X3 = 1, 2
XATTN_NO_PERSISTENT, XATTN_LEGACY_CHAIN = 1, 2
ABI_VERSION = 4


_SIGS = {
    "m3ae_abi_version": (C.c_int, []),
    "m3ae_desc_sizes": (None, [C.POINTER(i64)]),
    "m3ae_last_gemm_path": (C.c_char_p, []),
    "m3ae_gemm": (C.c_int, [C.POINTER(GemmDesc), vp]),
    "m3ae_attn_workspace_bytes": (i64, [C.POINTER(AttnDesc), C.c_int]),
    "m3ae_attn_fwd": (C.c_int, [C.POINTER(AttnDesc), vp]),
    "m3ae_attn_bwd": (C.c_int, [C.POINTER(AttnDesc), vp]),
    "m3ae_attn_probs": (C.c_int, [C.POINTER(AttnDesc), vp, i64, i64, i64, vp]),
    "m3ae_xattn_supported": (C.c_int, [C.POINTER(XattnDesc)]),
    "m3ae_xattn_bwd_supported": (C.c_int, [C.POINTER(XattnDesc)]),
    "m3ae_xattn_probs_ld": (i64, [C.POINTER(XattnDesc)]),
    "m3ae_xattn_fwd": (C.c_int, [C.POINTER(XattnDesc), vp]),
    "m3ae_xattn_bwd": (C.c_int, [C.POINTER(XattnDesc), vp]),
    "m3ae_xattn_probs_export": (C.c_int, [C.POINTER(XattnDesc), C.c_int, vp, i64, i64, i64, vp]),
    "m3ae_layernorm_fwd": (C.c_int, [vp, vp, vp, vp, vp, vp, i64, i64, f32, C.c_int, C.c_int, C.c_int, vp]),
    "m3ae_layernorm_bwd_blocks": (i64, [i64]),
    "m3ae_layernorm_bwd": (C.c_int, [vp, vp, vp, vp, vp, vp, vp, vp, vp, vp, vp, i64, i64, C.c_int, C.c_int, C.c_int, vp]),
    "m3ae_layernorm_bwd_drop": (C.c_int, [vp, vp, vp, vp, vp, vp, vp, vp, f32, C.c_uint64, vp, vp, vp, vp, i64, i64, C.c_int, vp]),
    "m3ae_dropout": (C.c_int, [vp, vp, vp, i64, i64, f32, C.c_uint64, vp, C.c_int, vp]),
    "m3ae_colsum": (C.c_int, [vp, vp, i64, i64, i64, C.c_int, C.c_int, vp]),
    "m3ae_roberta_embed_fwd": (C.c_int, [vp, vp, vp, vp, vp, i64, i64, i64, i64, C.c_int, vp]),
    "m3ae_roberta_embed_bwd": (C.c_int, [vp, vp, vp, vp, vp, i64, i64, i64, i64, C.c_int, vp]),
    "m3ae_patchify": (C.c_int, [vp, vp, i64, i64, i64, C.c_int, vp]),
    "m3ae_image_normalize_u8": (C.c_int, [vp, vp, i64, i64, i64, C.POINTER(C.c_float), C.POINTER(C.c_float), vp]),
    "m3ae_vit_tokens_fwd": (C.c_int, [vp, vp, vp, vp, i64, i64, i64, C.c_int, vp]),
    "m3ae_vit_tokens_bwd": (C.c_int, [vp, vp, vp, vp, i64, i64, i64, C.c_int, vp]),
    "m3ae_bce_logits": (C.c_int, [vp, vp, vp, vp, i64, i64, f32, C.c_int, vp]),
    "m3ae_xent": (C.c_int, [vp, vp, vp, vp, vp, i64, i64, i64, f32, C.c_int, vp]),
    "m3ae_adamw": (C.c_int, [vp, vp, vp, vp, vp, i64, f32, f32, f32, f32, f32, i64, f32, vp, vp]),
    "m3ae_cast_transpose": (C.c_int, [vp, vp, vp, i64, i64, vp]),
    "m3ae_cast_transpose_batched": (C.c_int, [vp, C.c_int, i64, vp]),
    "m3ae_transpose_bf16_batched": (C.c_int, [vp, C.c_int, i64, vp]),
    "m3ae_cast": (C.c_int, [vp, vp, i64, C.c_int, C.c_int, vp]),
    "m3ae_zero": (C.c_int, [vp, i64, vp]),
    "m3ae_add": (C.c_int, [vp, vp, vp, i64, C.c_int, vp]),
    "m3ae_act_fwd": (C.c_int, [vp, vp, i64, C.c_int, C.c_int, vp]),
    "m3ae_act_bwd": (C.c_int, [vp, vp, vp, i64, C.c_int, C.c_int, vp]),
    "m3ae_gather_rows": (C.c_int, [vp, vp, vp, i64, i64, C.c_int, vp]),
    "m3ae_scatter_add_rows": (C.c_int, [vp, vp, vp, i64, i64, C.c_int, vp]),
    "m3ae_mask_ranks": (C.c_int, [vp, vp, vp, vp, i64, i64, i64, vp]),
    "m3ae_mim_targets": (C.c_int, [vp, vp, i64, i64, i64, i64, i64, C.c_int, vp]),
    "m3ae_mim_loss_fwd": (C.c_int, [vp, vp, vp, vp, vp, i64, i64, i64, C.c_int, vp]),
    "m3ae_mim_loss_bwd": (C.c_int, [vp, vp, vp, vp, vp, vp, i64, i64, i64, C.c_int, vp]),
    "m3ae_selftest": (C.c_int, [vp, vp]),
    "m3ae_gemm_det_workspace_bytes": (i64, [C.POINTER(GemmDesc)]),
    "m3ae_gemm_det": (C.c_int, [C.POINTER(GemmDesc), vp, i64, vp]),
    "m3ae_det_workspace_bytes": (i64, [C.c_int, i64, i64]),
    "m3ae_colsum_det": (C.c_int, [vp, vp, i64, i64, i64, C.c_int, C.c_int, vp, i64, vp]),
    "m3ae_layernorm_bwd_det": (C.c_int, [vp, vp, vp, vp, vp, vp, vp, vp, vp, vp, vp, i64, i64, C.c_int, C.c_int, C.c_int, vp]),
    "m3ae_layernorm_bwd_drop_det": (C.c_int, [vp, vp, vp, vp, vp, vp, vp, vp, f32, C.c_uint64, vp, vp, vp, vp, i64, i64, C.c_int, vp]),
    "m3ae_roberta_embed_bwd_det": (C.c_int, [vp, vp, vp, vp, vp, i64, i64, i64, i64, C.c_int, vp, i64, vp]),
    "m3ae_bce_logits_det": (C.c_int, [vp, vp, vp, vp, i64, i64, f32, C.c_int, vp, i64, vp]),
    "m3ae_xent_det": (C.c_int, [vp, vp, vp, vp, i64, i64, i64, f32, C.c_int, vp, i64, vp]),
    "m3ae_mim_loss_fwd_det": (C.c_int, [vp, vp, vp, vp, vp, i64, i64, i64, C.c_int, vp, i64, vp]),
    "m3ae_image_resample_workspace_bytes": (i64, [i64, i64]),
    "m3ae_image_resample_u8": (C.c_int, [vp, i64, vp, vp, i64, i64, i64, vp, i64, vp, vp, C.POINTER(C.c_float), C.POINTER(C.c_float), vp]),
    "m3ae_gemm_rows": (C.c_int, [C.POINTER(GemmDesc), i64, i64, vp]),
    "m3ae_attn_fwd_rows": (C.c_int, [C.POINTER(AttnDesc), i64, i64, vp]),
    "m3ae_attn_bwd_rows": (C.c_int, [C.POINTER(AttnDesc), i64, i64, vp]),
    "m3ae_layernorm_bwd_drop_rows": (C.c_int, [vp, vp, vp, vp, vp, vp, vp, vp, f32, C.c_uint64, vp, vp, vp, vp, i64, i64, C.c_int, i64, i64, vp]),
    "m3ae_dropout_rows": (C.c_int, [vp, vp, vp, i64, i64, f32, C.c_uint64, vp, C.c_int, i64, i64, vp]),
    "m3ae_beam_topk_workspace_bytes": (i64, [i64, i64, i64, i64]),
    "m3ae_beam_topk": (C.c_int, [vp, i64, vp, i64, i64, i64, i64, vp, i64, vp, vp, vp]),
    "m3ae_beam_step": (C.c_int, [vp, vp, vp, vp, vp, vp, vp, vp, vp, vp, vp, vp, vp, vp, i64, i64, i64, i64, i64, i64, i64, C.c_double, vp]),
    "m3ae_beam_finalize": (C.c_int, [vp, vp, vp, vp, vp, vp, vp, vp, vp, i64, i64, i64, i64, i64, i64, C.c_double, vp]),
    "m3ae_expand_samples": (C.c_int, [vp, vp, vp, i64, i64, i64, C.c_int, vp]),
    "m3ae_segment_sum_rows": (C.c_int, [vp, vp, vp, vp, i64, i64, i64, C.c_int, vp]),
    "m3ae_layernorm_fwd_mixed": (C.c_int, [vp, vp, vp, vp, vp, vp, i64, i64, f32, vp]),
    "m3ae_layernorm_bwd_mixed": (C.c_int, [vp, vp, vp, vp, vp, vp, vp, vp, vp, vp, vp, i64, i64, vp]),
    "m3ae_layernorm_bwd_mixed_det": (C.c_int, [vp, vp, vp, vp, vp, vp, vp, vp, vp, vp, vp, i64, i64, vp]),
}

EXPORTS = tuple(_SIGS)
_lib = None


class M3AEHipError(RuntimeError):
    pass


def lib():
    global _lib
    if _lib is None:
        if not os.path.exists(LIB_PATH):
            raise M3AEHipError(f"{LIB_PATH} is missing: build it with `python -m m3ae_amd.build` "
                               f"(or __graft_entry__.build()); this package has no CPU fallback")
        import torch
        if DIAGNOSTIC:
            import warnings
            warnings.warn(f"m3ae_amd: loading the DIAGNOSTIC library {LIB_PATH} (timing-only builds may compute wrong results)")
        l = C.CDLL(LIB_PATH)
        for name, (res, args) in _SIGS.items():
            fn = getattr(l, name)
            fn.restype, fn.argtypes = res, args
        if l.m3ae_abi_version() != ABI_VERSION:
            raise M3AEHipError(f"ABI version mismatch: library {l.m3ae_abi_version()}, binding {ABI_VERSION}")
        sizes = (i64 * 3)()
        l.m3ae_desc_sizes(sizes)
        mine = (C.sizeof(GemmDesc), C.sizeof(AttnDesc), C.sizeof(XattnDesc))
        if tuple(sizes) != mine:
            raise M3AEHipError(f"descriptor layout mismatch: library {tuple(sizes)}, binding {mine}")
        _lib = l
    return _lib


def check(rc, what):
    if rc != 0:
        kind = {-1: "invalid argument", -2: "unsupported shape/dtype", -3: "misaligned", -4: "workspace too small"}.get(
            rc, f"hipError_t {rc}" if rc > 0 else f"error {rc}")
        raise M3AEHipError(f"{what} failed: {kind}")
```

mm-vqa-healthcare_amd/m3ae_amd/ops.py:

```python
import contextlib
import ctypes as C
import functools
import math
import os
import threading

import torch

from . import _lib
from ._lib import (ACT_GELU, ACT_MULAUX, ACT_NONE, ACT_QUICKGELU, ACT_RELU, ACT_TANH, BF16, F32, AttnDesc, GemmDesc, XattnDesc,
                   check)

grad_ready_hook = None
SAVE_DACT = os.environ.get("M3AE_SAVE_DACT", "1") != "0"
NT_NO_PERSISTENT = os.environ.get("M3AE_NT_NO_PERSISTENT", "0") == "1"
GEMM_NT_VARIANT, GEMM_TN_VARIANT, GEMM_COL_GROUP = int(os.environ.get("M3AE_GEMM_NT_VARIANT", -1)), int(os.environ.get("M3AE_GEMM_TN_VARIANT", -1)), int(os.environ.get("M3AE_GEMM_COL_GROUP", 0))


ATTN_LEGACY = os.environ.get("M3AE_ATTN_LEGACY", "0") == "1"
GEMM_ST_POLICY = int(os.environ.get("M3AE_GEMM_ST_POLICY", 0))


def _gemm_flags():
    return ((1 if NT_NO_PERSISTENT else 0) | (((GEMM_NT_VARIANT + 1) & 0xF) << 8) | (((GEMM_TN_VARIANT + 1) & 0xF) << 12)
            | ((GEMM_COL_GROUP & 0xF) << 16) | ((GEMM_ST_POLICY & 0x3) << 20))
PROFILE = None


class _Mode(threading.local):
    x3 = False


_MODE = _Mode()


@contextlib.contextmanager
def f32x3_mode(on):
    prev, _MODE.x3 = _MODE.x3, bool(on)
    try:
        yield
    finally:
        _MODE.x3 = prev


def f32x3_active():
    return _MODE.x3


def model_mode(fn):
    @functools.wraps(fn)
    def run(self, *args, **kwargs):
        with f32x3_mode(getattr(self, "f32x3", False)):
            return fn(self, *args, **kwargs)
    return run


class DeterministicError(_lib.M3AEHipError):
    pass


_DETERMINISTIC = False


def set_deterministic(on):
    global _DETERMINISTIC
    _DETERMINISTIC = bool(on)


def deterministic():
    return _DETERMINISTIC


@contextlib.contextmanager
def deterministic_mode(on=True):
    prev = deterministic()
    set_deterministic(on)
    try:
        yield
    finally:
        set_deterministic(prev)


def _no_ordered_form(op):
    if _DETERMINISTIC:
        raise DeterministicError(f"{op} has no deterministic form (it adds with fp32 atomics) and ops.deterministic() is on: "
                                 f"switch the mode off for this op with ops.set_deterministic(False)")


def _det_ws(nbytes, device):
    return torch.empty(max(int(nbytes), 16), dtype=torch.uint8, device=device)


def _small_ws(op, rows, cols, device):
    n = _lib.lib().m3ae_det_workspace_bytes(op, rows, cols)
    if n < 0:
        check(int(n), "m3ae_det_workspace_bytes")
    return _det_ws(n, device), n


class Function(torch.autograd.Function):

    def __init_subclass__(cls, **kwargs):
        super().__init_subclass__(**kwargs)
        fwd, bwd = cls.__dict__.get("forward"), cls.__dict__.get("backward")
        if fwd is not None:
            f = fwd.__func__ if isinstance(fwd, staticmethod) else fwd

            def forward(ctx, *args):
                ctx.m3ae_x3 = _MODE.x3
                return f(ctx, *args)
            cls.forward = staticmethod(functools.wraps(f)(forward))
        if bwd is not None:
            b = bwd.__func__ if isinstance(bwd, staticmethod) else bwd

            def backward(ctx, *grads):
                prev, _MODE.x3 = _MODE.x3, getattr(ctx, "m3ae_x3", False)
                try:
                    return b(ctx, *grads)
                finally:
                    _MODE.x3 = prev
            cls.backward = staticmethod(functools.wraps(b)(backward))


def _prof_begin():
    if PROFILE is None:
        return None
    e0 = torch.cuda.Event(enable_timing=True)
    e0.record()
    return e0


def _prof_end(e0, kind, dims):
    if e0 is None:
        return
    e1 = torch.cuda.Event(enable_timing=True)
    e1.record()
    PROFILE.append((kind, dims, e0, e1))


_drop_base, _drop_ctr = 0x5EED, 0


def set_dropout_seed(seed):
    global _drop_base, _drop_ctr
    _drop_base, _drop_ctr = int(seed) & 0xFFFFFFFF, 0


DROPOUT_SALT = None


def _salt():
    return None if DROPOUT_SALT is None else C.c_void_p(DROPOUT_SALT.data_ptr())


def next_dropout_seed():
    global _drop_ctr
    _drop_ctr += 1
    return ((_drop_base << 32) | (_drop_ctr & 0xFFFFFFFF)) & 0xFFFFFFFFFFFFFFFF


def dropout_pair(p):
    return (p, next_dropout_seed()) if p > 0 else None


def _set_dropout(d, dropout):
    if dropout is not None and dropout[0] > 0:
        d.dropout_p, d.dropout_seed = dropout
        d.dropout_salt = _salt()


def _dt(t):
    if t.dtype == torch.float32:
        return F32
    if t.dtype == torch.bfloat16:
        return BF16
    raise TypeError(f"unsupported dtype {t.dtype}")


_raw_stream = getattr(torch._C, "_cuda_getCurrentRawStream", None)
_dev_index = None


def _stream():
    global _dev_index
    if _raw_stream is None:
        return C.c_void_p(torch.cuda.current_stream().cuda_stream)
    if _dev_index is None:
        _dev_index = torch.cuda.current_device()
    return C.c_void_p(_raw_stream(_dev_index))


def _p(t):
    return None if t is None else C.c_void_p(t.data_ptr())


def _need_cuda(t):
    if not t.is_cuda:
        raise _lib.M3AEHipError("m3ae_amd ops run on the GPU only (no CPU fallback); got a CPU tensor")
    if _dev_index is not None and t.device.index != _dev_index:
        raise _lib.M3AEHipError(f"m3ae_amd ops were first used on cuda:{_dev_index}; got a tensor on {t.device} "
                                f"(one process drives one GPU: call torch.cuda.set_device before the first op)")


def compute_weight(w):
    return getattr(w, "m3ae_c", w)


def gemm(a, a_sm, a_sk, b, b_sk, b_sn, c, c_sm, M, N, K, *, alpha=1.0, accumulate=False, bias=None, act=ACT_NONE,
         preact=None, residual=None, dact_aux=None, dact=ACT_NONE, force_generic=False, batch=(1, 1),
         a_sb=(0, 0), b_sb=(0, 0), c_sb=(0, 0), a_rowsum=None, dropout=None, preact_grad=False, rows=None):
    _need_cuda(c)
    d = GemmDesc()
    d.M, d.N, d.K = M, N, K
    d.batch1, d.batch2 = batch
    d.A, d.a_sm, d.a_sk, d.a_sb1, d.a_sb2 = a.data_ptr(), a_sm, a_sk, a_sb[0], a_sb[1]
    d.B, d.b_sk, d.b_sn, d.b_sb1, d.b_sb2 = b.data_ptr(), b_sk, b_sn, b_sb[0], b_sb[1]
    d.C, d.c_sm, d.c_sn, d.c_sb1, d.c_sb2 = c.data_ptr(), c_sm, 1, c_sb[0], c_sb[1]
    d.dtype_a, d.dtype_b, d.dtype_c = _dt(a), _dt(b), _dt(c)
    d.alpha = alpha
    d.accumulate = int(accumulate)
    if bias is not None:
        assert bias.dtype == torch.float32
        d.bias = bias.data_ptr()
    d.act = act
    for name, t in (("preact", preact), ("residual", residual), ("dact_aux", dact_aux)):
        if t is not None:
            assert t.dtype == c.dtype and t.stride(-1) == 1 and t.stride(-2) == c_sm, name
            setattr(d, name, t.data_ptr())
    d.dact = dact
    d.preact_grad = int(preact_grad)
    d.launch_flags = _gemm_flags()
    if _MODE.x3 and d.dtype_a == F32 and d.dtype_b == F32 and d.dtype_c == F32:
        d.launch_flags |= _lib.GEMM_F32_X3
    d.force_generic = int(force_generic)
    if a_rowsum is not None:
        assert a_rowsum.dtype == torch.float32 and a_rowsum.numel() >= M and batch == (1, 1)
        d.a_rowsum = a_rowsum.data_ptr()
    _set_dropout(d, dropout)
    e0 = _prof_begin()
    nws = _lib.lib().m3ae_gemm_det_workspace_bytes(C.byref(d)) if _DETERMINISTIC else 0
    if nws > 0:
        d.launch_flags |= _lib.GEMM_DETERMINISTIC
        ws = _det_ws(nws, c.device)
        check(_lib.lib().m3ae_gemm_det(C.byref(d), _p(ws), nws, _stream()), "m3ae_gemm_det")
        del ws
    elif rows is not None:
        check(_lib.lib().m3ae_gemm_rows(C.byref(d), rows[0], rows[1], _stream()), "m3ae_gemm_rows")
    else:
        check(_lib.lib().m3ae_gemm(C.byref(d), _stream()), "m3ae_gemm")
    if e0 is not None:
        _prof_end(e0, "gemm:" + last_gemm_path(), (M, N, K, batch[0] * batch[1]))


def last_gemm_path():
    return _lib.lib().m3ae_last_gemm_path().decode()


def _rows(x):
    K = x.shape[-1]
    if x.dim() == 2:
        assert x.stride(1) == 1
        return x, x.shape[0], K, x.stride(0)
    if not x.is_contiguous():
        x = x.contiguous()
    x2 = x.view(-1, K)
    return x2, x2.shape[0], K, K


_LAUNCH_STREAM = None


def launch_stream():
    global _LAUNCH_STREAM
    if _LAUNCH_STREAM is None:
        _LAUNCH_STREAM = torch.cuda.Stream(priority=-1)
    return _LAUNCH_STREAM


def use_launch_stream():
    prev = torch.cuda.current_stream()
    if os.environ.get("M3AE_LAUNCH_PRIORITY", "high") != "high":
        return prev
    torch.cuda.synchronize()
    torch.cuda.set_stream(launch_stream())
    return prev


def mm_nt(x2, ldx, M, w, bias=None, act=ACT_NONE, residual=None, want_preact=False, out_dtype=None, dact_aux=None,
          dact=ACT_NONE, force_generic=False, alpha=1.0, dropout=None, preact_grad=False, rows=None):
    N, K = w.shape
    y = torch.empty((M, N), dtype=out_dtype or x2.dtype, device=x2.device)
    pre = torch.empty_like(y) if want_preact else None
    gemm(x2, ldx, 1, w, 1, w.stride(0), y, N, M, N, K, bias=bias, act=act, preact=pre, residual=residual,
         dact_aux=dact_aux, dact=dact, force_generic=force_generic, alpha=alpha, dropout=dropout,
         preact_grad=preact_grad and want_preact, rows=rows)
    return y, pre


def mm_dgrad(dy, w_param, dact_aux=None, dact=ACT_NONE, residual=None, alpha=1.0, dropout=None, out=None, ld_out=None, rows=None):
    M, N = dy.shape
    wt = getattr(w_param, "m3ae_t", None)
    if wt is not None:
        b, b_sk, b_sn, K = wt, 1, wt.stride(0), wt.shape[0]
    else:
        b = compute_weight(w_param)
        b_sk, b_sn, K = b.stride(0), 1, b.shape[1]
    if out is None:
        out, ld_out = torch.empty((M, K), dtype=dy.dtype, device=dy.device), K
    gemm(dy, dy.stride(0), 1, b, b_sk, b_sn, out, ld_out, M, K, N, dact_aux=dact_aux, dact=dact, residual=residual,
         alpha=alpha, dropout=dropout, rows=rows)
    return out


def mm_wgrad(dy, x2, ldx, w_param, b_param=None, alpha=1.0):
    want_b = b_param is not None and b_param.requires_grad
    if not w_param.requires_grad:
        if want_b:
            bias_grad(dy, b_param)
        return
    g = _grad_buf(w_param)
    M, N = dy.shape
    K = g.shape[1]
    gemm(dy, 1, dy.stride(0), x2, ldx, 1, g, g.stride(0), N, K, M, accumulate=True, alpha=alpha,
         a_rowsum=_grad_buf(b_param) if want_b else None)
    _done(w_param)
    if want_b:
        _done(b_param)


def colsum(x, out, accumulate):
    M, N = x.shape
    if _DETERMINISTIC:
        ws, n = _small_ws(_lib.DET_COLSUM, M, N, x.device)
        check(_lib.lib().m3ae_colsum_det(_p(x), _p(out), M, N, x.stride(0), _dt(x), int(accumulate), _p(ws), n, _stream()),
              "m3ae_colsum_det")
        return
    check(_lib.lib().m3ae_colsum(_p(x), _p(out), M, N, x.stride(0), _dt(x), int(accumulate), _stream()), "m3ae_colsum")


def bias_grad(dy, b_param):
    if b_param is None or not b_param.requires_grad:
        return
    colsum(dy, _grad_buf(b_param), True)
    _done(b_param)


def act_bwd(dy, pre, act):
    dx = torch.empty_like(dy)
    check(_lib.lib().m3ae_act_bwd(_p(dy), _p(pre), _p(dx), dy.numel(), act, _dt(dy), _stream()), "m3ae_act_bwd")
    return dx


def _members(p):
    return getattr(p, "members", None) or ([p] if p is not None else [])


def _done(p):
    if grad_ready_hook is not None and p is not None:
        for m in _members(p):
            grad_ready_hook(m)


def _grad_buf(p):
    if getattr(p, "members", None) is not None:
        g = p.grad
        if g is None:
            raise _lib.M3AEHipError("packed parameters need ParamStore-managed gradients")
        return g
    if p.grad is None:
        p.grad = torch.zeros_like(p, dtype=torch.float32)
    return p.grad


def add(a, b, out=None):
    _need_cuda(a)
    a, b = a.contiguous(), b.contiguous()
    out = torch.empty_like(a) if out is None else out
    check(_lib.lib().m3ae_add(_p(a), _p(b), _p(out), a.numel(), _dt(a), _stream()), "m3ae_add")
    return out


def cast(x, dtype):
    if x.dtype == dtype:
        return x
    _need_cuda(x)
    x = x.contiguous()
    out = torch.empty_like(x, dtype=dtype)
    check(_lib.lib().m3ae_cast(_p(x), _p(out), x.numel(), _dt(x), _dt(out), _stream()), "m3ae_cast")
    return out


class Fork2Fn(Function):

    @staticmethod
    def forward(ctx, x):
        return x.view_as(x), x.view_as(x)

    @staticmethod
    def backward(ctx, ga, gb):
        if ga is None:
            return gb
        if gb is None:
            return ga
        return add(ga, gb)


def fork2(x):
    return Fork2Fn.apply(x) if (x.requires_grad and torch.is_grad_enabled()) else (x, x)


class LinearFn(Function):

    @staticmethod
    def forward(ctx, x, residual, extra_bias, weight, bias, act, alpha, *anchors):
        x2, M, K, ldx = _rows(x)
        w = compute_weight(weight)
        b = None if bias is None else (bias.data if hasattr(bias, "members") else bias.detach())
        if extra_bias is not None:
            b = extra_bias.detach().float() if b is None else b + extra_bias.detach().float()
        res2 = None
        if residual is not None:
            res2 = residual.contiguous().view(M, -1)
        y, pre = mm_nt(x2, ldx, M, w, bias=b, act=act, residual=res2, want_preact=(act != ACT_NONE), alpha=alpha,
                       out_dtype=None if res2 is None else res2.dtype)
        ctx.save_for_backward(x2, pre)
        ctx.weight, ctx.bias, ctx.act, ctx.ldx, ctx.alpha = weight, bias, act, ldx, alpha
        ctx.x_shape, ctx.has_res = x.shape, residual is not None
        ctx.x_needs = x.requires_grad
        ctx.extra_needs = extra_bias is not None and extra_bias.requires_grad
        ctx.n_anchor = len(anchors)
        return y.view(*x.shape[:-1], y.shape[-1])

    @staticmethod
    def backward(ctx, dy):
        x2, pre = ctx.saved_tensors
        N = dy.shape[-1]
        dy2 = cast(dy.contiguous().view(-1, N), x2.dtype)
        dres = dy if ctx.has_res else None
        dz = act_bwd(dy2, pre, ctx.act) if ctx.act != ACT_NONE else dy2
        dextra = None
        dx = None
        if ctx.x_needs:
            dx = mm_dgrad(dz, ctx.weight, alpha=ctx.alpha).view(ctx.x_shape)
        if ctx.extra_needs:
            mm_wgrad(dz, x2, ctx.ldx, ctx.weight, alpha=ctx.alpha)
            dextra = torch.empty(N, dtype=torch.float32, device=dz.device)
            colsum(dz, dextra, False)
            if ctx.bias is not None and ctx.bias.requires_grad:
                _grad_buf(ctx.bias).add_(dextra)
                _done(ctx.bias)
        else:
            mm_wgrad(dz, x2, ctx.ldx, ctx.weight, ctx.bias, alpha=ctx.alpha)
        return (dx, dres, dextra, None, None, None, None) + (None,) * ctx.n_anchor


class GatherLinearFn(Function):

    @staticmethod
    def forward(ctx, x, weight, bias, act):
        B, L, D = x.shape
        xc = x.contiguous()
        w = compute_weight(weight)
        y, pre = mm_nt(xc, L * D, B, w, bias=bias, act=act, want_preact=(act != ACT_NONE))
        ctx.save_for_backward(xc, pre)
        ctx.weight, ctx.bias, ctx.act = weight, bias, act
        return y

    @staticmethod
    def backward(ctx, dy):
        xc, pre = ctx.saved_tensors
        B, L, D = xc.shape
        dy2 = dy.contiguous()
        dz = act_bwd(dy2, pre, ctx.act) if ctx.act != ACT_NONE else dy2
        mm_wgrad(dz, xc, L * D, ctx.weight, ctx.bias)
        dx = mm_dgrad(dz, ctx.weight, out=torch.zeros_like(xc), ld_out=L * D)
        return dx, None, None, None


class MLPFn(Function):

    @staticmethod
    def forward(ctx, x, residual, w1, b1, w2, b2, act):
        x2, M, K, ldx = _rows(x)
        g, u = mm_nt(x2, ldx, M, compute_weight(w1), bias=b1, act=act, want_preact=True, preact_grad=SAVE_DACT)
        res2 = residual.contiguous().view(M, -1) if residual is not None else None
        y, _ = mm_nt(g, g.stride(0), M, compute_weight(w2), bias=b2, residual=res2, out_dtype=None if res2 is None else res2.dtype)
        ctx.save_for_backward(x2, u, g)
        ctx.p = (w1, b1, w2, b2)
        ctx.act, ctx.ldx, ctx.x_shape, ctx.has_res = act, ldx, x.shape, residual is not None
        return y.view(*x.shape[:-1], y.shape[-1])

    @staticmethod
    def backward(ctx, dy):
        x2, u, g = ctx.saved_tensors
        w1, b1, w2, b2 = ctx.p
        dy2 = cast(dy.contiguous().view(-1, dy.shape[-1]), g.dtype)
        dres = dy if ctx.has_res else None
        mm_wgrad(dy2, g, g.stride(0), w2, b2)
        du = mm_dgrad(dy2, w2, dact_aux=u, dact=ACT_MULAUX if SAVE_DACT else ctx.act)
        mm_wgrad(du, x2, ctx.ldx, w1, b1)
        dx = mm_dgrad(du, w1).view(ctx.x_shape)
        return dx, dres, None, None, None, None, None


def linear(x, weight, bias=None, act=ACT_NONE, residual=None, extra_bias=None, alpha=1.0):
    anchors = tuple(_members(weight)) if hasattr(weight, "members") else ()
    if hasattr(bias, "members"):
        anchors = anchors + tuple(bias.members)
    return LinearFn.apply(x, residual, extra_bias, weight, bias, act, alpha, *anchors)


def mlp(x, w1, b1, w2, b2, act, residual=None):
    return MLPFn.apply(x, residual, w1, b1, w2, b2, act)


class LayerNormFn(Function):
    @staticmethod
    def forward(ctx, x, gamma, beta, eps, act, rms, out_dtype=None):
        xc = x.contiguous()
        D = xc.shape[-1]
        M = xc.numel() // D
        y = torch.empty_like(xc, dtype=out_dtype or xc.dtype)
        mean = torch.empty(M, dtype=torch.float32, device=x.device)
        rstd = torch.empty(M, dtype=torch.float32, device=x.device)
        if y.dtype != xc.dtype:
            _ln_mixed_ok(xc, y, act, rms)
            check(_lib.lib().m3ae_layernorm_fwd_mixed(_p(xc), _p(gamma), _p(beta), _p(y), _p(mean), _p(rstd), M, D, eps, _stream()),
                  "m3ae_layernorm_fwd_mixed")
        else:
            check(_lib.lib().m3ae_layernorm_fwd(_p(xc), _p(gamma), _p(beta), _p(y), _p(mean), _p(rstd), M, D, eps, _dt(xc),
                                                act, int(rms), _stream()), "m3ae_layernorm_fwd")
        ctx.save_for_backward(xc, mean, rstd)
        ctx.gamma, ctx.beta, ctx.act, ctx.rms = gamma, beta, act, rms
        return y

    @staticmethod
    def backward(ctx, dy):
        xc, mean, rstd = ctx.saved_tensors
        D = xc.shape[-1]
        M = xc.numel() // D
        dyc = dy.contiguous()
        dx = torch.empty_like(xc)
        L = _lib.lib()
        nblk = L.m3ae_layernorm_bwd_blocks(M)
        ws = torch.empty(2 * nblk * D, dtype=torch.float32, device=xc.device)
        gg = _grad_buf(ctx.gamma)
        gb = _grad_buf(ctx.beta) if ctx.beta is not None else None
        if dyc.dtype != xc.dtype:
            ln_bwd = L.m3ae_layernorm_bwd_mixed_det if _DETERMINISTIC else L.m3ae_layernorm_bwd_mixed
            check(ln_bwd(_p(dyc), _p(xc), _p(ctx.gamma), _p(mean), _p(rstd), _p(dx), None, None, _p(gg), _p(gb), _p(ws), M, D,
                         _stream()), "m3ae_layernorm_bwd_mixed")
        else:
            ln_bwd = L.m3ae_layernorm_bwd_det if _DETERMINISTIC else L.m3ae_layernorm_bwd
            check(ln_bwd(_p(dyc), _p(xc), _p(ctx.gamma), _p(ctx.beta), _p(mean), _p(rstd), _p(dx), None,
                         _p(gg), _p(gb), _p(ws), M, D, _dt(xc), ctx.act, int(ctx.rms), _stream()),
                  "m3ae_layernorm_bwd")
        _done(ctx.gamma)
        _done(ctx.beta)
        return dx, None, None, None, None, None, None


def layer_norm(x, gamma, beta, eps, act=ACT_NONE, rms=False, out_dtype=None):
    return LayerNormFn.apply(x, gamma, beta, eps, act, rms, out_dtype)


def _ln_mixed_ok(x, y, act, rms):
    if not (x.dtype == torch.float32 and y.dtype == torch.bfloat16 and act == ACT_NONE and not rms):
        raise _lib.M3AEHipError(f"LayerNorm from {x.dtype} rows to {y.dtype} rows: only plain LayerNorm from float32 to bfloat16 "
                                "has a kernel")


def ln_fwd_raw(x2, ln, act=ACT_NONE, rms=False, out_dtype=None):
    M, D = x2.shape
    y = torch.empty_like(x2, dtype=out_dtype or x2.dtype)
    mean = None if rms else torch.empty(M, dtype=torch.float32, device=x2.device)
    rstd = torch.empty(M, dtype=torch.float32, device=x2.device)
    if y.dtype != x2.dtype:
        _ln_mixed_ok(x2, y, act, rms)
        check(_lib.lib().m3ae_layernorm_fwd_mixed(_p(x2), _p(ln.weight), _p(ln.bias), _p(y), _p(mean), _p(rstd), M, D, ln.eps,
                                                  _stream()), "m3ae_layernorm_fwd_mixed")
        return y, mean, rstd
    check(_lib.lib().m3ae_layernorm_fwd(_p(x2), _p(ln.weight), _p(ln.bias), _p(y), _p(mean), _p(rstd), M, D, ln.eps,
                                        _dt(x2), act, int(rms), _stream()), "m3ae_layernorm_fwd")
    return y, mean, rstd


def ln_bwd_raw(dy, x2, ln, mean, rstd, dx_add=None, act=ACT_NONE, rms=False, drop=None, rows=None, want_lo=False):
    M, D = x2.shape
    L = _lib.lib()
    dx = torch.empty_like(x2)
    nblk = L.m3ae_layernorm_bwd_blocks(M)
    ws = torch.empty(2 * nblk * D, dtype=torch.float32, device=x2.device)
    train = ln.weight.requires_grad
    gg = _grad_buf(ln.weight) if train else None
    gb = _grad_buf(ln.bias) if (train and ln.bias is not None) else None
    if drop is not None and drop[0] > 0:
        assert dx_add is None and act == ACT_NONE and not rms
        dxd = torch.empty_like(x2)
        if rows is not None:
            check(L.m3ae_layernorm_bwd_drop_rows(_p(dy), _p(x2), _p(ln.weight), _p(ln.bias), _p(mean), _p(rstd), _p(dx), _p(dxd),
                                                 drop[0], drop[1], _salt(), _p(gg), _p(gb), _p(ws), M, D, _dt(x2), rows[0], rows[1],
                                                 _stream()), "m3ae_layernorm_bwd_drop_rows")
            if train:
                _done(ln.weight)
                _done(ln.bias)
            return dx, dxd
        ln_bwd_drop = L.m3ae_layernorm_bwd_drop_det if _DETERMINISTIC else L.m3ae_layernorm_bwd_drop
        check(ln_bwd_drop(_p(dy), _p(x2), _p(ln.weight), _p(ln.bias), _p(mean), _p(rstd), _p(dx), _p(dxd),
                          drop[0], drop[1], _salt(), _p(gg), _p(gb), _p(ws), M, D, _dt(x2), _stream()),
              "m3ae_layernorm_bwd_drop")
        if train:
            _done(ln.weight)
            _done(ln.bias)
        return dx, dxd
    dx_lo = None
    if dy.dtype != x2.dtype:
        _ln_mixed_ok(x2, dy, act, rms)
        assert dx_add is None or dx_add.dtype == torch.float32
        dx_lo = torch.empty_like(dy) if want_lo else None
        ln_bwd = L.m3ae_layernorm_bwd_mixed_det if _DETERMINISTIC else L.m3ae_layernorm_bwd_mixed
        check(ln_bwd(_p(dy), _p(x2), _p(ln.weight), _p(mean), _p(rstd), _p(dx), _p(dx_add), _p(dx_lo), _p(gg), _p(gb), _p(ws), M, D,
                     _stream()), "m3ae_layernorm_bwd_mixed")
    else:
        assert not want_lo
        ln_bwd = L.m3ae_layernorm_bwd_det if _DETERMINISTIC else L.m3ae_layernorm_bwd
        check(ln_bwd(_p(dy), _p(x2), _p(ln.weight), _p(ln.bias), _p(mean), _p(rstd), _p(dx), _p(dx_add),
                     _p(gg), _p(gb), _p(ws), M, D, _dt(x2), act, int(rms), _stream()), "m3ae_layernorm_bwd")
    if train:
        _done(ln.weight)
        _done(ln.bias)
    return (dx, dx_lo) if want_lo else dx


def _attn_desc(B, H, Lq, Lk, Dh, q, k, v, o, key_mask, pos_bias, scale, causal, lse, lse_stride, dtype):
    d = AttnDesc()
    d.B, d.H, d.Lq, d.Lk, d.Dh = B, H, Lq, Lk, Dh
    d.q, d.q_sb, d.q_sl = q.data_ptr(), q.stride(0), q.stride(1)
    d.k, d.k_sb, d.k_sl = k.data_ptr(), k.stride(0), k.stride(1)
    d.v, d.v_sb, d.v_sl = v.data_ptr(), v.stride(0), v.stride(1)
    d.o, d.o_sb, d.o_sl = o.data_ptr(), o.stride(0), o.stride(1)
    d.key_mask = key_mask.data_ptr() if key_mask is not None else None
    d.pos_bias = pos_bias.data_ptr() if pos_bias is not None else None
    d.scale, d.causal = scale, int(causal)
    d.lse = lse.data_ptr() if lse is not None else None
    d.lse_stride = lse_stride
    d.dtype = dtype
    d.launch_flags = _lib.ATTN_LEGACY_KERNELS if ATTN_LEGACY else 0
    if _MODE.x3 and dtype == F32:
        d.launch_flags |= _lib.ATTN_F32_X3
    return d


def _attn_ws(d, backward, device):
    n = _lib.lib().m3ae_attn_workspace_bytes(C.byref(d), int(backward))
    if n <= 0:
        return None
    ws = torch.empty(n, dtype=torch.uint8, device=device)
    d.workspace, d.workspace_bytes = ws.data_ptr(), n
    return ws


def attn_forward(q, k, v, heads, key_mask=None, pos_bias=None, scale=None, causal=False, dropout=None, rows=None):
    _need_cuda(q)
    B, Lq, D = q.shape
    Lk = k.shape[1]
    Dh = D // heads
    if q.dtype == torch.bfloat16 and Dh != 64:
        o32, lse = attn_forward(q.float(), k.float(), v.float(), heads, key_mask, pos_bias, scale, causal, dropout, rows)
        return o32.to(torch.bfloat16), lse
    scale = (1.0 / math.sqrt(Dh)) if scale is None else scale
    o = torch.empty((B, Lq, D), dtype=q.dtype, device=q.device)
    lse_stride = (Lq + 31) // 32 * 32
    lse = (torch.empty if q.dtype == torch.bfloat16 else torch.zeros)((B, heads, lse_stride), dtype=torch.float32, device=q.device)
    d = _attn_desc(B, heads, Lq, Lk, Dh, q, k, v, o, key_mask, pos_bias, scale, causal, lse, lse_stride, _dt(q))
    _set_dropout(d, dropout)
    ws = _attn_ws(d, False, q.device)
    e0 = _prof_begin()
    if rows is not None:
        check(_lib.lib().m3ae_attn_fwd_rows(C.byref(d), rows[0], rows[1], _stream()), "m3ae_attn_fwd_rows")
    else:
        check(_lib.lib().m3ae_attn_fwd(C.byref(d), _stream()), "m3ae_attn_fwd")
    _prof_end(e0, "attn_fwd", (B, heads, Lq, Lk, Dh))
    del ws
    return o, lse


def attn_backward(q, k, v, o, lse, do, dq, dk, dv, heads, key_mask=None, pos_bias=None, scale=None, causal=False,
                  d_pos_bias=None, dropout=None, rows=None):
    if d_pos_bias is not None:
        _no_ordered_form("the relative-position-bias gradient of m3ae_attn_bwd (d_pos_bias, T5 attention)")
    B, Lq, D = q.shape
    Lk = k.shape[1]
    Dh = D // heads
    if q.dtype == torch.bfloat16 and Dh != 64:
        f = [t.float() for t in (q, k, v, o, do)]
        g = [torch.empty_like(t) for t in f[:3]]
        attn_backward(f[0], f[1], f[2], f[3].contiguous(), lse, f[4].contiguous(), g[0], g[1], g[2], heads, key_mask,
                      pos_bias, scale, causal, d_pos_bias, dropout, rows)
        for dst, src in zip((dq, dk, dv), g):
            dst.copy_(src)
        return
    scale = (1.0 / math.sqrt(Dh)) if scale is None else scale
    assert do.stride() == o.stride() and dq.stride() == q.stride() and dk.stride() == k.stride() and dv.stride() == v.stride()
    d = _attn_desc(B, heads, Lq, Lk, Dh, q, k, v, o, key_mask, pos_bias, scale, causal, lse, lse.shape[-1], _dt(q))
    delta = torch.empty_like(lse) if q.dtype == torch.bfloat16 else torch.zeros_like(lse)
    d.d_o, d.dq, d.dk, d.dv, d.delta = do.data_ptr(), dq.data_ptr(), dk.data_ptr(), dv.data_ptr(), delta.data_ptr()
    d.d_pos_bias = d_pos_bias.data_ptr() if d_pos_bias is not None else None
    _set_dropout(d, dropout)
    ws = _attn_ws(d, True, q.device)
    e0 = _prof_begin()
    if rows is not None:
        check(_lib.lib().m3ae_attn_bwd_rows(C.byref(d), rows[0], rows[1], _stream()), "m3ae_attn_bwd_rows")
    else:
        check(_lib.lib().m3ae_attn_bwd(C.byref(d), _stream()), "m3ae_attn_bwd")
    _prof_end(e0, "attn_bwd", (B, heads, Lq, Lk, Dh))
    del ws, delta


def attn_probs(q, k, lse, heads, key_mask=None, scale=None, dropout=None):
    _need_cuda(q)
    B, Lq, D = q.shape
    Lk = k.shape[1]
    Dh = D // heads
    if q.dtype == torch.bfloat16 and Dh != 64:
        return attn_probs(q.float(), k.float(), None, heads, key_mask, scale, dropout)
    scale = (1.0 / math.sqrt(Dh)) if scale is None else scale
    out = torch.empty((B, heads, Lq, Lk), dtype=torch.float32, device=q.device)
    lse_stride = lse.shape[-1] if lse is not None else 0
    d = _attn_desc(B, heads, Lq, Lk, Dh, q, k, k, q, key_mask, None, scale, False, lse, lse_stride, _dt(q))
    _set_dropout(d, dropout)
    e0 = _prof_begin()
    check(_lib.lib().m3ae_attn_probs(C.byref(d), C.c_void_p(out.data_ptr()), out.stride(0), out.stride(1), out.stride(2),
                                     _stream()), "m3ae_attn_probs")
    _prof_end(e0, "attn_probs", (B, heads, Lq, Lk, Dh))
    return out


class SelfAttnFn(Function):

    @staticmethod
    def forward(ctx, qkv, key_mask, heads, dropout=None, causal=False):
        D = qkv.shape[-1] // 3
        q, k, v = qkv[..., :D], qkv[..., D:2 * D], qkv[..., 2 * D:]
        o, lse = attn_forward(q, k, v, heads, key_mask, dropout=dropout, causal=causal)
        ctx.save_for_backward(qkv, o, lse, key_mask)
        ctx.heads, ctx.dropout, ctx.causal = heads, dropout, causal
        return o

    @staticmethod
    def backward(ctx, do):
        qkv, o, lse, key_mask = ctx.saved_tensors
        D = qkv.shape[-1] // 3
        dqkv = torch.empty_like(qkv)
        attn_backward(qkv[..., :D], qkv[..., D:2 * D], qkv[..., 2 * D:], o, lse, do.contiguous(), dqkv[..., :D],
                      dqkv[..., D:2 * D], dqkv[..., 2 * D:], ctx.heads, key_mask, dropout=ctx.dropout, causal=ctx.causal)
        return dqkv, None, None, None, None


class CrossAttnFn(Function):

    @staticmethod
    def forward(ctx, q, kv, key_mask, heads, dropout=None):
        D = q.shape[-1]
        o, lse = attn_forward(q, kv[..., :D], kv[..., D:], heads, key_mask, dropout=dropout)
        ctx.save_for_backward(q, kv, o, lse, key_mask)
        ctx.heads, ctx.dropout = heads, dropout
        return o

    @staticmethod
    def backward(ctx, do):
        q, kv, o, lse, key_mask = ctx.saved_tensors
        D = q.shape[-1]
        dq = torch.empty_strided(q.shape, q.stride(), dtype=q.dtype, device=q.device)
        dkv = torch.empty_strided(kv.shape, kv.stride(), dtype=kv.dtype, device=kv.device)
        attn_backward(q, kv[..., :D], kv[..., D:], o, lse, do.contiguous(), dq, dkv[..., :D], dkv[..., D:], ctx.heads,
                      key_mask, dropout=ctx.dropout)
        return dq, dkv, None, None, None


def self_attention(qkv, key_mask, heads, dropout=None, causal=False):
    return SelfAttnFn.apply(qkv, key_mask, heads, dropout, causal)


def cross_attention(q, kv, key_mask, heads, dropout=None):
    return CrossAttnFn.apply(q, kv, key_mask, heads, dropout)


def _bdata(b):
    return None if b is None else (b.data if hasattr(b, "members") else b.detach())


XATTN = os.environ.get("M3AE_XATTN", "auto")
XATTN_TRAIN = os.environ.get("M3AE_XATTN_TRAIN", "auto")
XATTN_TRAIN_MIN_BATCH = int(os.environ.get("M3AE_XATTN_TRAIN_MIN_BATCH", 96))
XATTN_LEGACY_CHAIN = False
CLS_ONLY = os.environ.get("M3AE_CLS_ONLY", "1") != "0"


def _xattn_desc(h2, B, L, other2, Lo, mask, P, pdrop, seeds):
    D = h2.shape[1]
    d = XattnDesc()
    d.dir = 0 if L <= Lo else 1
    d.B, d.Lq, d.Lk, d.D, d.H = B, L, Lo, D, P.heads
    d.x, d.y = h2.data_ptr(), other2.data_ptr()
    d.key_mask = mask.data_ptr() if mask is not None else None
    wq, wkv, wo = P.w_q, P.w_kv, P.w_o
    d.wq, d.wkv, d.wo = compute_weight(wq).data_ptr(), compute_weight(wkv).data_ptr(), compute_weight(wo).data_ptr()
    d.wq_t, d.wkv_t, d.wo_t = wq.m3ae_t.data_ptr(), wkv.m3ae_t.data_ptr(), wo.m3ae_t.data_ptr()
    d.bq, d.bkv, d.bo = _bdata(P.b_q).data_ptr(), _bdata(P.b_kv).data_ptr(), _bdata(P.b_o).data_ptr()
    d.ln_g, d.ln_b, d.ln_eps = P.ln.weight.data_ptr(), P.ln.bias.data_ptr(), P.ln.eps
    if pdrop > 0:
        d.dropout_p, d.seed_attn, d.seed_hidden = pdrop, seeds[0], seeds[1]
        d.dropout_salt = _salt()
    d.launch_flags = (_lib.XATTN_NO_PERSISTENT if NT_NO_PERSISTENT else 0) | (_lib.XATTN_LEGACY_CHAIN if XATTN_LEGACY_CHAIN else 0)
    return d


def xattn_supported(h2, L, other2, Lo, mask, P, backward=False):
    if XATTN == "off" or h2.dtype != torch.bfloat16 or other2.shape[1] != h2.shape[1]:
        return False
    if XATTN != "always" and P.heads * min(L, Lo) >= h2.shape[1]:
        return False
    if getattr(P.w_q, "m3ae_t", None) is None or getattr(P.w_kv, "m3ae_t", None) is None or getattr(P.w_o, "m3ae_t", None) is None:
        return False
    d = XattnDesc()
    d.dir = 0 if L <= Lo else 1
    d.B, d.Lq, d.Lk, d.D, d.H = 1, L, Lo, h2.shape[1], P.heads
    d.launch_flags = _lib.XATTN_LEGACY_CHAIN if XATTN_LEGACY_CHAIN else 0
    if not backward:
        return bool(_lib.lib().m3ae_xattn_supported(C.byref(d)))
    if not all(p.requires_grad for p in (P.w_q, P.w_kv, P.w_o, P.b_q, P.b_kv, P.b_o)):
        return False
    if _DETERMINISTIC:
        return False
    return bool(_lib.lib().m3ae_xattn_bwd_supported(C.byref(d)))


def xattn_fwd(h2, B, L, other2, Lo, mask, P, pdrop=0.0, need_bwd=True, want_probs=False):
    _need_cuda(h2)
    dev, D, H = h2.device, h2.shape[1], P.heads
    seeds = (next_dropout_seed(), next_dropout_seed()) if pdrop > 0 else None
    d = _xattn_desc(h2, B, L, other2, Lo, mask, P, pdrop, seeds)
    bf = torch.bfloat16
    T, R = min(L, Lo), H * min(L, Lo)
    e = lambda *shape, dt=bf: torch.empty(shape, dtype=dt, device=dev)
    t = {}
    if d.dir == 0:
        t["proj"] = e(B * L, D)
        t["prime"] = e(B, R, D)
        t["probs"] = e(B, R, 640)
        t["zctx"] = e(B, R, D)
        t["ctx"] = e(B * L, D)
        if pdrop > 0:
            t["probs_drop"] = e(B, R, 640)
            t["rowsum"] = e(B, R, dt=torch.float32)
    else:
        t["proj"] = e(B * Lo, 2 * D)
        t["prime"] = e(2, B, R, D)
        t["colbias"] = e(B, R, dt=torch.float32)
        if need_bwd or XATTN_LEGACY_CHAIN or want_probs:
            t["probs"] = e(B, L, R)
            if pdrop > 0:
                t["probs_drop"] = e(B, L, R)
    t["s"] = e(B * L, D)
    t["out"] = e(B * L, D)
    t["mean"] = e(B * L, dt=torch.float32)
    t["rstd"] = e(B * L, dt=torch.float32)
    for k, v in t.items():
        setattr(d, k, v.data_ptr())
    e0 = _prof_begin()
    check(_lib.lib().m3ae_xattn_fwd(C.byref(d), _stream()), "m3ae_xattn_fwd")
    _prof_end(e0, "xattn_fwd", (B, H, L, Lo, D // H))
    return t["out"], ("xattn", h2, other2, mask, t, seeds, pdrop)


def xattn_probs(saved):
    _, h2, other2, mask, t, seeds, pdrop = saved
    if "probs" not in t:
        raise _lib.M3AEHipError("this fused cross-attention call kept its probabilities on chip (xattn_fwd(want_probs=True))")
    d = XattnDesc()
    prime = t["prime"]
    dir1 = prime.dim() == 4
    B = prime.shape[1] if dir1 else prime.shape[0]
    L, Lo = h2.shape[0] // B, other2.shape[0] // B
    d.dir = 1 if dir1 else 0
    d.B, d.Lq, d.Lk, d.D = B, L, Lo, h2.shape[1]
    d.H = prime.shape[-2] // min(L, Lo)
    d.probs = t["probs"].data_ptr()
    dropped = pdrop > 0
    if dropped:
        d.probs_drop = t["probs_drop"].data_ptr()
    out = torch.empty((B, d.H, L, Lo), dtype=torch.float32, device=h2.device)
    check(_lib.lib().m3ae_xattn_probs_export(C.byref(d), int(dropped), C.c_void_p(out.data_ptr()), out.stride(0), out.stride(1),
                                             out.stride(2), _stream()), "m3ae_xattn_probs_export")
    return out


def xattn_bwd(dy, saved, B, L, Lo, P, need_dother=True):
    _no_ordered_form("the fused cross-attention backward (m3ae_xattn_bwd; its forward ran before the mode was switched on)")
    _, h2, other2, mask, t, seeds, pdrop = saved
    dev, D, H = h2.device, h2.shape[1], P.heads
    d = _xattn_desc(h2, B, L, other2, Lo, mask, P, pdrop, seeds)
    for k, v in t.items():
        setattr(d, k, v.data_ptr())
    bf = torch.bfloat16
    e = lambda *shape, dt=bf: torch.empty(shape, dtype=dt, device=dev)
    dyc = dy.contiguous()
    dx = e(B * L, D)
    dother = e(B * Lo, D) if need_dother else None
    L_ = _lib.lib()
    w = {"ws_ds": e(B * L, D), "ws_dscores": torch.empty_like(t["probs"]), "ws_dprime": torch.empty_like(t["prime"]),
         "ws_dproj": torch.empty_like(t["proj"]), "ws_vec": e(3 * B * H * min(L, Lo), dt=torch.float32),
         "ws_ln": e(2 * L_.m3ae_layernorm_bwd_blocks(B * L) * D, dt=torch.float32)}
    if pdrop > 0:
        w["ws_dsd"] = e(B * L, D)
    if d.dir == 0:
        w["ws_dz"] = torch.empty_like(t["zctx"])
        w["ws_dctx"] = e(B * L, D)
    for k, v in w.items():
        setattr(d, k, v.data_ptr())
    d.d_out, d.dx = dyc.data_ptr(), dx.data_ptr()
    d.dy = dother.data_ptr() if dother is not None else None
    train = P.ln.weight.requires_grad
    grads = {"g_wq": P.w_q, "g_wkv": P.w_kv, "g_wo": P.w_o, "g_bq": P.b_q, "g_bkv": P.b_kv, "g_bo": P.b_o}
    for k, prm in grads.items():
        if not prm.requires_grad:
            raise _lib.M3AEHipError("the fused cross-attention backward needs trainable projection parameters")
        setattr(d, k, _grad_buf(prm).data_ptr())
    if train:
        d.g_ln_g, d.g_ln_b = _grad_buf(P.ln.weight).data_ptr(), _grad_buf(P.ln.bias).data_ptr()
    e0 = _prof_begin()
    check(L_.m3ae_xattn_bwd(C.byref(d), _stream()), "m3ae_xattn_bwd")
    _prof_end(e0, "xattn_bwd", (B, H, L, Lo, D // H))
    for prm in (P.w_o, P.b_o, P.w_kv, P.b_kv, P.w_q, P.b_q) + ((P.ln.weight, P.ln.bias) if train else ()):
        _done(prm)
    return dx, dother


def _qkv_views(bufs, B):
    if len(bufs) == 1:
        p3 = bufs[0].view(B, -1, bufs[0].shape[1])
        n = p3.shape[2] // 3
        return p3[..., :n], p3[..., n:2 * n], p3[..., 2 * n:]
    q, kv = bufs
    n = q.shape[1]
    kv3 = kv.view(B, -1, 2 * n)
    return q.view(B, -1, n), kv3[..., :n], kv3[..., n:]


def _attn_core_fwd(x2, B, P, src2=None, kv=None, mask=None, pos_bias=None, scale=None, causal=False, dropout=None):
    M, D = x2.shape
    if src2 is None and kv is None:
        proj = (mm_nt(x2, D, M, compute_weight(P.w_qkv), bias=_bdata(P.b_qkv))[0],)
    else:
        q, _ = mm_nt(x2, D, M, compute_weight(P.w_q), bias=_bdata(P.b_q))
        if kv is None:
            kv, _ = mm_nt(src2, src2.shape[1], src2.shape[0], compute_weight(P.w_kv), bias=_bdata(P.b_kv))
        proj = (q, kv)
    q3, k3, v3 = _qkv_views(proj, B)
    o, lse = attn_forward(q3, k3, v3, P.heads, mask, pos_bias, scale, causal, dropout)
    return o, lse, proj


def _attn_core_bwd(dctx, x2, src2, proj, o, lse, B, P, mask=None, pos_bias=None, scale=None, causal=False, dropout=None,
                   d_pos_bias=None, residual=None, need_dx=True, need_dsrc=True):
    dproj = tuple(torch.empty_like(t) for t in proj)
    attn_backward(*_qkv_views(proj, B), o, lse, dctx.view(o.shape), *_qkv_views(dproj, B), P.heads, mask, pos_bias, scale,
                  causal, d_pos_bias, dropout)
    D = x2.shape[1]
    if len(proj) == 1:
        mm_wgrad(dproj[0], x2, D, P.w_qkv, P.b_qkv)
        return (mm_dgrad(dproj[0], P.w_qkv, residual=residual) if need_dx else None), None
    assert src2 is not None, "the forward was given ready-made kv (inference only): there is no source to differentiate"
    dq, dkv = dproj
    mm_wgrad(dq, x2, D, P.w_q, P.b_q)
    mm_wgrad(dkv, src2, src2.shape[1], P.w_kv, P.b_kv)
    dx = mm_dgrad(dq, P.w_q, residual=residual) if need_dx else None
    return dx, (mm_dgrad(dkv, P.w_kv) if need_dsrc else None)


def _ffn_core_fwd(x2, P, act, residual, mid_drop=None, out_drop=None, rows=None):
    M, D = x2.shape
    g, u = mm_nt(x2, D, M, compute_weight(P.w1), bias=_bdata(P.b1), act=act, want_preact=True, preact_grad=SAVE_DACT,
                 dropout=mid_drop, rows=rows)
    y, _ = mm_nt(g, g.shape[1], M, compute_weight(P.w2), bias=_bdata(P.b2), residual=residual, dropout=out_drop, rows=rows,
                 out_dtype=None if residual is None else residual.dtype)
    return y, u, g


def _ffn_core_bwd(dy, x2, u, g, P, act, mid_drop=None, residual=None, rows=None):
    mm_wgrad(dy, g, g.shape[1], P.w2, P.b2)
    du = mm_dgrad(dy, P.w2, dact_aux=u, dact=ACT_MULAUX if SAVE_DACT else act, dropout=mid_drop, rows=rows)
    mm_wgrad(du, x2, x2.shape[1], P.w1, P.b1)
    return mm_dgrad(du, P.w1, residual=residual)


def _attn_sub_fwd(h2, B, L, other2, Lo, mask, P, pdrop=0.0, fused_cross=False):
    if other2 is not None and fused_cross:
        need_bwd = getattr(P, "need_bwd", True)
        if xattn_supported(h2, L, other2, Lo, mask, P, backward=need_bwd):
            return xattn_fwd(h2, B, L, other2, Lo, mask, P, pdrop, need_bwd=need_bwd, want_probs=getattr(P, "want_probs", False))
    da, dh = dropout_pair(pdrop), dropout_pair(pdrop)
    o, lse, proj = _attn_core_fwd(h2, B, P, src2=other2, mask=mask, dropout=da)
    D = h2.shape[1]
    s, _ = mm_nt(o.view(B * L, D), D, B * L, compute_weight(P.w_o), bias=_bdata(P.b_o), residual=h2, dropout=dh)
    y, mean, rstd = ln_fwd_raw(s, P.ln)
    return y, (h2, other2, proj, o, lse, s, mean, rstd, mask, da, dh)


def _attn_sub_probs(saved, B, L, Lo, P):
    if isinstance(saved[0], str):
        return xattn_probs(saved)
    h2, other2, proj, o, lse, s, mean, rstd, mask, da, dh = saved
    q3, k3, _ = _qkv_views(proj, B)
    return attn_probs(q3, k3, lse, P.heads, mask, dropout=da)


def _post_ln_bwd(dy, s, ln, mean, rstd, dh, rows=None):
    if dh is not None:
        return ln_bwd_raw(dy, s, ln, mean, rstd, drop=dh, rows=rows)
    ds = ln_bwd_raw(dy, s, ln, mean, rstd)
    return ds, ds


def _attn_sub_bwd(dy, saved, B, L, Lo, P, need_dother=True):
    if isinstance(saved[0], str):
        return xattn_bwd(dy, saved, B, L, Lo, P, need_dother)
    h2, other2, proj, o, lse, s, mean, rstd, mask, da, dh = saved
    D = h2.shape[1]
    ds, dsd = _post_ln_bwd(dy, s, P.ln, mean, rstd, dh)
    mm_wgrad(dsd, o.view(B * L, D), D, P.w_o, P.b_o)
    dctx = mm_dgrad(dsd, P.w_o)
    return _attn_core_bwd(dctx, h2, other2, proj, o, lse, B, P, mask=mask, dropout=da, residual=ds, need_dsrc=need_dother)


def _ffn_sub_fwd(h2, P, pdrop=0.0, rows=None):
    dh = dropout_pair(pdrop)
    s, u, g = _ffn_core_fwd(h2, P, ACT_GELU, h2, out_drop=dh, rows=rows)
    y, mean, rstd = ln_fwd_raw(s, P.ln)
    return y, (h2, u, g, s, mean, rstd, dh, rows)


def _ffn_sub_bwd(dy, saved, P):
    h2, u, g, s, mean, rstd, dh, rows = saved
    ds, dsd = _post_ln_bwd(dy, s, P.ln, mean, rstd, dh, rows)
    return _ffn_core_bwd(dsd, h2, u, g, P, ACT_GELU, residual=ds, rows=rows)


class _ProjRows:

    def __init__(self, w_param, b_param, r0=None, r1=None):
        self.w_param, self.b_param, self.sl = w_param, b_param, slice(r0, r1)

    @property
    def w(self):
        return compute_weight(self.w_param)[self.sl]

    @property
    def b(self):
        return _bdata(self.b_param)[self.sl]

    def dgrad(self, dy, residual=None):
        M, n = dy.shape
        wt = getattr(self.w_param, "m3ae_t", None)
        if wt is not None:
            b = wt[:, self.sl]
            b_sk, b_sn, K = 1, wt.stride(0), wt.shape[0]
        else:
            b = self.w
            b_sk, b_sn, K = b.stride(0), 1, b.shape[1]
        out = torch.empty((M, K), dtype=dy.dtype, device=dy.device)
        gemm(dy, dy.stride(0), 1, b, b_sk, b_sn, out, K, M, K, n, residual=residual)
        return out

    def wgrad(self, dy, x2, ldx):
        want_b = self.b_param is not None and self.b_param.requires_grad
        if not self.w_param.requires_grad:
            if want_b:
                colsum(dy, _grad_buf(self.b_param)[self.sl], True)
            return
        g = _grad_buf(self.w_param)[self.sl]
        M, n = dy.shape
        gemm(dy, 1, dy.stride(0), x2, ldx, 1, g, g.stride(0), n, g.shape[1], M, accumulate=True,
             a_rowsum=_grad_buf(self.b_param)[self.sl] if want_b else None)


def _live_proj(P, D):
    if hasattr(P, "w_qkv"):
        return _ProjRows(P.w_qkv, P.b_qkv, 0, D), _ProjRows(P.w_qkv, P.b_qkv, D, 3 * D)
    return _ProjRows(P.w_q, P.b_q), _ProjRows(P.w_kv, P.b_kv)


def _attn_sub_fwd_live(hq, src2, B, Ls, Lfull, mask, P, pdrop=0.0):
    D = hq.shape[1]
    da, dh = dropout_pair(pdrop), dropout_pair(pdrop)
    pq, pkv = _live_proj(P, D)
    kv, _ = mm_nt(src2, src2.shape[1], B * Ls, pkv.w, bias=pkv.b)
    q, _ = mm_nt(hq, D, B, pq.w, bias=pq.b)
    n = q.shape[1]
    kv3 = kv.view(B, Ls, 2 * n)
    o, lse = attn_forward(q.view(B, 1, n), kv3[..., :n], kv3[..., n:], P.heads, mask, dropout=da, rows=(0, Lfull))
    s, _ = mm_nt(o.view(B, n), n, B, compute_weight(P.w_o), bias=_bdata(P.b_o), residual=hq, dropout=dh, rows=(0, Lfull))
    y, mean, rstd = ln_fwd_raw(s, P.ln)
    return y, (hq, src2, q, kv, o, lse, s, mean, rstd, mask, da, dh, Ls, Lfull)


def _attn_sub_bwd_live(dy, saved, B, P, need_dsrc=True):
    hq, src2, q, kv, o, lse, s, mean, rstd, mask, da, dh, Ls, Lfull = saved
    D, n = hq.shape[1], q.shape[1]
    ds, dsd = _post_ln_bwd(dy, s, P.ln, mean, rstd, dh, rows=(0, Lfull))
    mm_wgrad(dsd, o.view(B, n), n, P.w_o, P.b_o)
    dctx = mm_dgrad(dsd, P.w_o)
    dq, dkv = torch.empty_like(q), torch.empty_like(kv)
    kv3, dkv3 = kv.view(B, Ls, 2 * n), dkv.view(B, Ls, 2 * n)
    attn_backward(q.view(B, 1, n), kv3[..., :n], kv3[..., n:], o, lse, dctx.view(o.shape), dq.view(B, 1, n), dkv3[..., :n],
                  dkv3[..., n:], P.heads, mask, dropout=da, rows=(0, Lfull))
    pq, pkv = _live_proj(P, D)
    pq.wgrad(dq, hq, D)
    pkv.wgrad(dkv, src2, src2.shape[1])
    for prm in {id(p): p for p in (pq.w_param, pq.b_param, pkv.w_param, pkv.b_param)}.values():
        if prm.requires_grad:
            _done(prm)
    if pq.w_param is pkv.w_param:
        dh = pkv.dgrad(dkv)
        dqkv0 = torch.cat([dq, dkv3[:, 0]], dim=1)
        dh.view(B, Ls, D)[:, 0] = mm_dgrad(dqkv0, pq.w_param, residual=ds)
        return None, dh
    dhq = pq.dgrad(dq, residual=ds)
    return dhq, (pkv.dgrad(dkv) if need_dsrc else None)


class BertCrossLayerFn(Function):

    @staticmethod
    def forward(ctx, h, other, mask_self, mask_other, P, *anchors):
        B, L, D = h.shape
        Lo = other.shape[1]
        h2 = h.contiguous().view(B * L, D)
        other2 = other.contiguous().view(B * Lo, other.shape[2])
        pd = getattr(P, "pdrop", 0.0)
        ctx.live = bool(getattr(P, "cls_only", False))
        if ctx.live:
            hq = h2.view(B, L, D)[:, 0].contiguous()
            a, s1 = _attn_sub_fwd_live(hq, h2, B, L, L, mask_self, P.attn, pd)
            c, s2 = _attn_sub_fwd_live(a, other2, B, Lo, L, mask_other, P.cross, pd)
            y, s3 = _ffn_sub_fwd(c, P.ffn, pd, rows=(0, L))
            ctx.saved = (s1, s2, s3)
            ctx.P, ctx.dims, ctx.n_anchor = P, (B, L, Lo, D), len(anchors)
            ctx.need_other = other.requires_grad
            return y.view(B, 1, D)
        a, s1 = _attn_sub_fwd(h2, B, L, None, L, mask_self, P.attn, pd)
        c, s2 = _attn_sub_fwd(a, B, L, other2, Lo, mask_other, P.cross, pd, fused_cross=getattr(P, "fused_cross", False))
        y, s3 = _ffn_sub_fwd(c, P.ffn, pd)
        ctx.saved = (s1, s2, s3)
        ctx.P, ctx.dims, ctx.n_anchor = P, (B, L, Lo, D), len(anchors)
        ctx.need_other = other.requires_grad
        if getattr(P, "want_probs", False):
            maps = (_attn_sub_probs(s1, B, L, L, P.attn), _attn_sub_probs(s2, B, L, Lo, P.cross))
            ctx.mark_non_differentiable(*maps)
            return (y.view(B, L, D),) + maps
        return y.view(B, L, D)

    @staticmethod
    def backward(ctx, dy, *_maps):
        B, L, Lo, D = ctx.dims
        s1, s2, s3 = ctx.saved
        ctx.saved = None
        P = ctx.P
        if ctx.live:
            dc = _ffn_sub_bwd(dy.contiguous().view(B, D), s3, P.ffn)
            da, dother = _attn_sub_bwd_live(dc, s2, B, P.cross, need_dsrc=ctx.need_other)
            _, dh = _attn_sub_bwd_live(da, s1, B, P.attn)
            return (dh.view(B, L, D), None if dother is None else dother.view(B, Lo, -1), None, None, None) + \
                   (None,) * ctx.n_anchor
        dc = _ffn_sub_bwd(dy.contiguous().view(B * L, D), s3, P.ffn)
        da, dother = _attn_sub_bwd(dc, s2, B, L, Lo, P.cross, need_dother=ctx.need_other)
        dh, _ = _attn_sub_bwd(da, s1, B, L, L, P.attn)
        return (dh.view(B, L, D), None if dother is None else dother.view(B, Lo, -1), None, None, None) + \
               (None,) * ctx.n_anchor


class BertSelfLayerFn(Function):

    @staticmethod
    def forward(ctx, h, mask, P, *anchors):
        B, L, D = h.shape
        h2 = h.contiguous().view(B * L, D)
        pd = getattr(P, "pdrop", 0.0)
        a, s1 = _attn_sub_fwd(h2, B, L, None, L, mask, P.attn, pd)
        y, s3 = _ffn_sub_fwd(a, P.ffn, pd)
        ctx.saved = (s1, s3)
        ctx.P, ctx.dims, ctx.n_anchor = P, (B, L, D), len(anchors)
        return y.view(B, L, D)

    @staticmethod
    def backward(ctx, dy):
        B, L, D = ctx.dims
        s1, s3 = ctx.saved
        ctx.saved = None
        da = _ffn_sub_bwd(dy.contiguous().view(B * L, D), s3, ctx.P.ffn)
        dh, _ = _attn_sub_bwd(da, s1, B, L, L, ctx.P.attn)
        return (dh.view(B, L, D), None, None) + (None,) * ctx.n_anchor


class ClipBlockFn(Function):

    @staticmethod
    def forward(ctx, x, P, *anchors):
        B, L, D = x.shape
        M = B * L
        x2 = x.contiguous().view(M, D)
        lo = compute_weight(P.w_qkv).dtype
        h1, m1, r1 = ln_fwd_raw(x2, P.ln1, out_dtype=lo)
        o, lse, proj = _attn_core_fwd(h1, B, P)
        xa, _ = mm_nt(o.view(M, D), D, M, compute_weight(P.w_o), bias=_bdata(P.b_o), residual=x2, out_dtype=x2.dtype)
        h2, m2, r2 = ln_fwd_raw(xa, P.ln2, out_dtype=lo)
# ... 645 lines not shown
```

Baseline: 1428.

## Fuse bias column-sum into LayerNorm backward and add two-row-per-wave bwd kernel

Adds a LayerNorm backward variant that also accumulates the column sum of the (dropped) input gradient, so the cross-attention backward no longer runs a separate colsum pass over dsd to get the output-projection bias gradient. It also adds a pair kernel that processes two rows per wave with register prefetch, gamma staged in LDS and optional nontemporal loads and stores, selected through new flag bits. The extra partial plane raises LDS and workspace use and can lower occupancy, and the deterministic path rejects the fused form.

Result: no change. 1433, median of 6 (+0.3%).

```diff
diff --git a/include/m3ae_hip.h b/include/m3ae_hip.h
--- a/include/m3ae_hip.h
+++ b/include/m3ae_hip.h
@@ -122,7 +122,9 @@
     const void* dropout_salt;
 } m3ae_xattn_desc;
 enum { M3AE_XATTN_NO_PERSISTENT = 1,
-       M3AE_XATTN_LEGACY_CHAIN = 2     };
+       M3AE_XATTN_LEGACY_CHAIN = 2,
+       M3AE_XATTN_LN_ONE_ROW = 4,
+       M3AE_XATTN_LN_NT = 8            };
 int m3ae_xattn_supported(const m3ae_xattn_desc* d);
 int m3ae_xattn_bwd_supported(const m3ae_xattn_desc* d);
 int64_t m3ae_xattn_probs_ld(const m3ae_xattn_desc* d);
@@ -131,6 +133,10 @@
 int m3ae_xattn_probs_export(const m3ae_xattn_desc* d, int dropped, float* out, int64_t o_sb, int64_t o_sh, int64_t o_sq,
                             void* stream);
 
+enum { M3AE_LN_RMS = 1,
+       M3AE_LN_ONE_ROW = 2,
+       M3AE_LN_NT = 4,
+       M3AE_LN_PAIR_ANY_M = 8  };
 int m3ae_layernorm_fwd(const void* x, const float* gamma, const float* beta, void* y, float* mean, float* rstd,
                        int64_t M, int64_t D, float eps, int dtype, int act, int rms, void* stream);
 int64_t m3ae_layernorm_bwd_blocks(int64_t M);
@@ -141,6 +147,13 @@
                             const float* rstd, void* dx, void* dx_drop, float dropout_p, uint64_t dropout_seed,
                             const void* dropout_salt, float* dgamma, float* dbeta, float* workspace, int64_t M, int64_t D,
                             int dtype, void* stream);
+int m3ae_layernorm_bwd_colsum(const void* dy, const void* x, const float* gamma, const float* beta, const float* mean,
+                              const float* rstd, void* dx, const void* dx_add, float* dgamma, float* dbeta, float* dx_colsum,
+                              float* workspace, int64_t M, int64_t D, int dtype, int act, int flags, void* stream);
+int m3ae_layernorm_bwd_drop_colsum(const void* dy, const void* x, const float* gamma, const float* beta, const float* mean,
+                                   const float* rstd, void* dx, void* dx_drop, float dropout_p, uint64_t dropout_seed,
+                                   const void* dropout_salt, float* dgamma, float* dbeta, float* dx_colsum, float* workspace,
+                                   int64_t M, int64_t D, int dtype, int flags, void* stream);
 int m3ae_layernorm_bwd_drop_rows(const void* dy, const void* x, const float* gamma, const float* beta, const float* mean,
                                  const float* rstd, void* dx, void* dx_drop, float dropout_p, uint64_t dropout_seed,
                                  const void* dropout_salt, float* dgamma, float* dbeta, float* workspace, int64_t M, int64_t D,
diff --git a/mm-vqa-healthcare_amd/csrc/norm.hip b/mm-vqa-healthcare_amd/csrc/norm.hip
--- a/mm-vqa-healthcare_amd/csrc/norm.hip
+++ b/mm-vqa-healthcare_amd/csrc/norm.hip
@@ -182,21 +182,22 @@
     }
 }
 
-template <typename T, int CPL, bool ACT, typename TD = T>
+template <typename T, int CPL, bool ACT, typename TD = T, bool CS = false>
 __global__ __launch_bounds__(256) void ln_bwd_kernel(const TD* dy, const T* x, const float* gamma, const float* beta,
                                                      const float* mean_i, const float* rstd_i, T* dx, const T* dx_add,
                                                      float* part, int64_t M, int D, int act, int rms, T* dx_drop,
                                                      DropState drop, bf16_t* dx_lo) {
     if (dx_drop) drop_resolve(drop);
     extern __shared__ float red[];
+    constexpr int NPL = CS ? 3 : 2;
     const int lane = threadIdx.x & 63, wave = threadIdx.x >> 6;
     const int nch = D >> 2;
-    float dg[CPL][4], db[CPL][4], g[CPL][4], bt[ACT ? CPL : 1][4];
+    float dg[CPL][4], db[CPL][4], g[CPL][4], bt[ACT ? CPL : 1][4], dc[CS ? CPL : 1][4];
 #pragma unroll
     for (int c = 0; c < CPL; ++c) {
         const int ch = lane + c * 64;
 #pragma unroll
-        for (int t = 0; t < 4; ++t) { dg[c][t] = 0.f; db[c][t] = 0.f; g[c][t] = 0.f; if (ACT) bt[c][t] = 0.f; }
+        for (int t = 0; t < 4; ++t) { dg[c][t] = 0.f; db[c][t] = 0.f; g[c][t] = 0.f; if (ACT) bt[c][t] = 0.f; if (CS) dc[c][t] = 0.f; }
         if (ch < nch) {
             ld4<float>(gamma + ch * 4, g[c]);
             if (ACT && beta) ld4<float>(beta + ch * 4, bt[c]);
@@ -271,6 +272,13 @@
                     for (int t = 0; t < 4; ++t) od[t] = o[t];
                     drop_apply4(drop, (uint64_t)(drop_row(drop, row) * D + ch * 4), od);
                     st4<T>(dx_drop + row * D + ch * 4, od);
+                    if constexpr (CS) {
+#pragma unroll
+                        for (int t = 0; t < 4; ++t) dc[c][t] += od[t];
+                    }
+                } else if constexpr (CS) {
+#pragma unroll
+                    for (int t = 0; t < 4; ++t) dc[c][t] += o[t];
                 }
                 if (dx_add) {
                     float e[4];
@@ -291,51 +299,225 @@
         if (ch < nch) {
 #pragma unroll
             for (int t = 0; t < 4; ++t) {
-                red[(wave * 2 + 0) * D + ch * 4 + t] = dg[c][t];
-                red[(wave * 2 + 1) * D + ch * 4 + t] = db[c][t];
+                red[(wave * NPL + 0) * D + ch * 4 + t] = dg[c][t];
+                red[(wave * NPL + 1) * D + ch * 4 + t] = db[c][t];
+                if constexpr (CS) red[(wave * NPL + 2) * D + ch * 4 + t] = dc[c][t];
             }
         }
     }
     __syncthreads();
-    for (int i = threadIdx.x; i < 2 * D; i += 256) {
+    for (int i = threadIdx.x; i < NPL * D; i += 256) {
         const int which = i / D, col = i - which * D;
         float s = 0.f;
 #pragma unroll
-        for (int w = 0; w < 4; ++w) s += red[(w * 2 + which) * D + col];
-        part[((int64_t)blockIdx.x * 2 + which) * D + col] = s;
-    }
-}
-
-__global__ __launch_bounds__(256) void ln_bwd_reduce_kernel(const float* part, float* dgamma, float* dbeta, int nblk,
-                                                            int D) {
+        for (int w = 0; w < 4; ++w) s += red[(w * NPL + which) * D + col];
+        part[((int64_t)blockIdx.x * NPL + which) * D + col] = s;
+    }
+}
+
+template <bool NT> DEVINL u32x4 ldg16(const bf16_t* p) {
+    if constexpr (NT) return __builtin_nontemporal_load((const u32x4*)p);
+    else return *(const u32x4*)p;
+}
+template <bool NT> DEVINL void stg16(bf16_t* p, const float* o) {
+    const u32x4 v = {pack2bf(o[0], o[1]), pack2bf(o[2], o[3]), pack2bf(o[4], o[5]), pack2bf(o[6], o[7])};
+    if constexpr (NT) __builtin_nontemporal_store(v, (u32x4*)p);
+    else *(u32x4*)p = v;
+}
+DEVINL void unpack8(const u32x4& r, float* v) {
+#pragma unroll
+    for (int q = 0; q < 4; ++q) {
+        v[2 * q] = __uint_as_float(r[q] << 16);
+        v[2 * q + 1] = __uint_as_float(r[q] & 0xffff0000u);
+    }
+}
+
+template <int NP, bool CS, bool NT>
+__global__ __launch_bounds__(256) __attribute__((amdgpu_waves_per_eu(NP <= 1 ? 4 : (NP == 4 && CS) ? 1 : 2))) void ln_bwd_pair_kernel(const bf16_t* dy, const bf16_t* x, const float* gamma, const float* mean_i,
+                                                          const float* rstd_i, bf16_t* dx, const bf16_t* dx_add, float* part,
+                                                          int64_t M, bf16_t* dx_drop, DropState drop) {
+    if (dx_drop) drop_resolve(drop);
+    extern __shared__ float red[];
+    constexpr int D = NP * 256, PPR = D / 8, NPL = CS ? 3 : 2;
+    const int lane = threadIdx.x & 63, wave = threadIdx.x >> 6;
+    const float* gs = red + 4 * NPL * D;
+    for (int i = threadIdx.x * 4; i < D; i += 1024) *(f32x4*)(red + 4 * NPL * D + i) = *(const f32x4*)(gamma + i);
+    __syncthreads();
+    int sel[NP], col[NP];
+    float dg[NP][8], db[NP][8], dc[CS ? NP : 1][8];
+#pragma unroll
+    for (int c = 0; c < NP; ++c) {
+        const int p = lane + 64 * c;
+        sel[c] = p >= PPR;
+        col[c] = (p - sel[c] * PPR) * 8;
+#pragma unroll
+        for (int e = 0; e < 8; ++e) { dg[c][e] = 0.f; db[c][e] = 0.f; if (CS) dc[c][e] = 0.f; }
+    }
+    const int64_t npair = (M + 1) >> 1;
+    const int64_t stride = (int64_t)gridDim.x * 4;
+    int64_t pr = (int64_t)blockIdx.x * 4 + wave;
+    u32x4 xr[NP], dr[NP], ar[NP];
+    float mn0 = 0.f, mn1 = 0.f, rn0 = 0.f, rn1 = 0.f;
+    auto load = [&](int64_t pair) {
+        const bool two = pair * 2 + 1 < M;
+#pragma unroll
+        for (int c = 0; c < NP; ++c) {
+            const int64_t o = pair * 2 * D + (lane + 64 * c) * 8;
+            if (two || !sel[c]) { xr[c] = *(const u32x4*)(x + o); dr[c] = ldg16<NT>(dy + o); }
+            else { xr[c] = (u32x4){0u, 0u, 0u, 0u}; dr[c] = (u32x4){0u, 0u, 0u, 0u}; }
+        }
+        mn0 = mean_i[pair * 2]; rn0 = rstd_i[pair * 2];
+        mn1 = two ? mean_i[pair * 2 + 1] : 0.f; rn1 = two ? rstd_i[pair * 2 + 1] : 0.f;
+    };
+    auto load_add = [&](int64_t pair) {
+        const bool two = pair * 2 + 1 < M;
+#pragma unroll
+        for (int c = 0; c < NP; ++c)
+            ar[c] = (two || !sel[c]) ? *(const u32x4*)(dx_add + pair * 2 * D + (lane + 64 * c) * 8) : (u32x4){0u, 0u, 0u, 0u};
+    };
+    if (pr < npair) {
+        load(pr);
+        if (dx_add) load_add(pr);
+    }
+    for (; pr < npair; pr += stride) {
+        const float m0 = mn0, m1 = mn1, r0 = rn0, r1 = rn1;
+        u32x4 xc[NP], dyc[NP];
+        float s10 = 0.f, s11 = 0.f, s20 = 0.f, s21 = 0.f;
+#pragma unroll
+        for (int c = 0; c < NP; ++c) {
+            const float mu = sel[c] ? m1 : m0, rs = sel[c] ? r1 : r0;
+            float xv[8], dv[8], g[8], t1 = 0.f, t2 = 0.f;
+            xc[c] = xr[c];
+            dyc[c] = dr[c];
+            unpack8(xc[c], xv);
+            unpack8(dyc[c], dv);
+            ld4<float>(gs + col[c], g);
+            ld4<float>(gs + col[c] + 4, g + 4);
+#pragma unroll
+            for (int e = 0; e < 8; ++e) {
+                const float h = (xv[e] - mu) * rs;
+                const float d = dv[e];
+                dg[c][e] += d * h;
+                db[c][e] += d;
+                const float dh = d * g[e];
+                t1 += dh;
+                t2 += dh * h;
+            }
+            if (sel[c]) { s11 += t1; s21 += t2; } else { s10 += t1; s20 += t2; }
+        }
+        const int64_t cur = pr;
+        const bool more = pr + stride < npair;
+        if (more) load(pr + stride);
+        const float c10 = wave_sum(s10) / (float)D, c11 = wave_sum(s11) / (float)D;
+        const float c20 = wave_sum(s20) / (float)D, c21 = wave_sum(s21) / (float)D;
+        const bool two = cur * 2 + 1 < M;
+#pragma unroll
+        for (int c = 0; c < NP; ++c) {
+            if (!two && sel[c]) continue;
+            const float mu = sel[c] ? m1 : m0, rs = sel[c] ? r1 : r0, c1 = sel[c] ? c11 : c10, c2 = sel[c] ? c21 : c20;
+            const int64_t row = cur * 2 + sel[c];
+            const int64_t off = cur * 2 * D + (lane + 64 * c) * 8;
+            float xv[8], dv[8], g[8], o[8];
+            unpack8(xc[c], xv);
+            unpack8(dyc[c], dv);
+            ld4<float>(gs + col[c], g);
+            ld4<float>(gs + col[c] + 4, g + 4);
+#pragma unroll
+            for (int e = 0; e < 8; ++e) {
+                const float h = (xv[e] - mu) * rs;
+                const float dh = dv[e] * g[e];
+                o[e] = rs * (dh - c1 - h * c2);
+            }
+            if (dx_drop) {
+                float od[8];
+#pragma unroll
+                for (int e = 0; e < 8; ++e) od[e] = o[e];
+                const uint64_t idx = (uint64_t)(drop_row(drop, row) * D + col[c]);
+                drop_apply4(drop, idx, od);
+                drop_apply4(drop, idx + 4, od + 4);
+                stg16<NT>(dx_drop + off, od);
+                if constexpr (CS) {
+#pragma unroll
+                    for (int e = 0; e < 8; ++e) dc[c][e] += od[e];
+                }
+            } else if constexpr (CS) {
+#pragma unroll
+                for (int e = 0; e < 8; ++e) dc[c][e] += o[e];
+            }
+            if (dx_add) {
+                float a[8];
+                unpack8(ar[c], a);
+#pragma unroll
+                for (int e = 0; e < 8; ++e) o[e] += a[e];
+            }
+            stg16<NT>(dx + off, o);
+            __builtin_amdgcn_sched_barrier(0);
+        }
+        if (dx_add && more) load_add(pr + stride);
+    }
+    float* rw = red + wave * NPL * D;
+#pragma unroll
+    for (int c = 0; c < NP; ++c) {
+        if (sel[c]) continue;
+#pragma unroll
+        for (int e = 0; e < 8; ++e) {
+            rw[col[c] + e] = dg[c][e];
+            rw[D + col[c] + e] = db[c][e];
+            if constexpr (CS) rw[2 * D + col[c] + e] = dc[c][e];
+        }
+    }
+#pragma unroll
+    for (int c = 0; c < NP; ++c) {
+        if (!sel[c]) continue;
+#pragma unroll
+        for (int e = 0; e < 8; ++e) {
+            rw[col[c] + e] += dg[c][e];
+            rw[D + col[c] + e] += db[c][e];
+            if constexpr (CS) rw[2 * D + col[c] + e] += dc[c][e];
+        }
+    }
+    __syncthreads();
+    for (int i = threadIdx.x; i < NPL * D; i += 256) {
+        const int which = i / D, cl = i - which * D;
+        float s = 0.f;
+#pragma unroll
+        for (int w = 0; w < 4; ++w) s += red[(w * NPL + which) * D + cl];
+        part[((int64_t)blockIdx.x * NPL + which) * D + cl] = s;
+    }
+}
+
+__global__ __launch_bounds__(256) void ln_bwd_reduce_kernel(const float* part, float* dgamma, float* dbeta, float* dcol, int nblk,
+                                                            int D, int npl) {
     __shared__ float red[8][33];
     const int cl = threadIdx.x & 31, rl = threadIdx.x >> 5;
     const int i = blockIdx.x * 32 + cl;
     const int b0 = blockIdx.y * 64;
     const int b1 = b0 + 64 < nblk ? b0 + 64 : nblk;
+    const int which = i / D, col = i - which * D;
+    float* dst = i >= npl * D ? nullptr : which == 0 ? dgamma : which == 1 ? dbeta : dcol;
     float s = 0.f;
-    if (i < 2 * D) {
-        const int which = i / D, col = i - which * D;
-        for (int b = b0 + rl; b < b1; b += 8) s += part[((int64_t)b * 2 + which) * D + col];
-    }
+    if (dst)
+        for (int b = b0 + rl; b < b1; b += 8) s += part[((int64_t)b * npl + which) * D + col];
     red[rl][cl] = s;
     __syncthreads();
-    if (rl == 0 && i < 2 * D) {
+    if (rl == 0 && dst) {
         float t = 0.f;
 #pragma unroll
         for (int r = 0; r < 8; ++r) t += red[r][cl];
-        const int which = i / D, col = i - which * D;
-        if (which == 0) atomicAdd(dgamma + col, t);
-        else if (dbeta) atomicAdd(dbeta + col, t);
-    }
-}
-
-inline int ln_bwd_fold(const float* part, float* dgamma, float* dbeta, int nblk, int D, int det, hipStream_t s) {
-    if (det)
+        atomicAdd(dst + col, t);
+    }
+}
+
+inline int ln_bwd_fold(const float* part, float* dgamma, float* dbeta, float* dcol, int nblk, int D, int det, hipStream_t s) {
+    if (!dgamma && !dcol) return 0;
+    if (det) {
+        if (dcol) return M3AE_ERR_UNSUPPORTED;
         det_fold(part, dgamma, dbeta, nblk, dbeta ? 2 * D : D, 2 * D, D, 1.0f, 1, s);
-    else
-        hipLaunchKernelGGL(ln_bwd_reduce_kernel, dim3((unsigned)cdiv(2 * D, 32), (unsigned)cdiv(nblk, 64)), dim3(256), 0, s, part, dgamma,
-                           dbeta, nblk, D);
+    } else {
+        const int npl = dcol ? 3 : 2;
+        hipLaunchKernelGGL(ln_bwd_reduce_kernel, dim3((unsigned)cdiv(npl * D, 32), (unsigned)cdiv(nblk, 64)), dim3(256), 0, s, part,
+                           dgamma, dbeta, dcol, nblk, D, npl);
+    }
     return hip_launch_status();
 }
 
@@ -356,22 +538,31 @@
 template <typename T, int CPL, typename TD = T>
 int launch_bwd(const void* dy, const void* x, const float* g, const float* b, const float* mean, const float* rstd,
                void* dx, const void* dx_add, float* part, int* nblk_io, int64_t M, int D, int act, int rms, hipStream_t s,
-               void* dx_drop = nullptr, DropState drop = DropState{}, void* dx_lo = nullptr) {
-    const size_t lds = (size_t)8 * D * sizeof(float);
-    static int cap_act = 0, cap_plain = 0, cap_d = -1;
+               void* dx_drop = nullptr, DropState drop = DropState{}, void* dx_lo = nullptr, bool colsum = false) {
+    const size_t lds = (size_t)(colsum ? 12 : 8) * D * sizeof(float);
+    static int cap_act = 0, cap_plain = 0, cap_cs = 0, cap_d = -1;
     constexpr bool MIXED = !std::is_same<TD, T>::value;
     if (cap_d != D) {
-        if constexpr (!MIXED) cap_act = resident_blocks(ln_bwd_kernel<T, CPL, true, TD>, lds);
-        cap_plain = resident_blocks(ln_bwd_kernel<T, CPL, false, TD>, lds);
+        if constexpr (!MIXED) {
+            cap_act = resident_blocks(ln_bwd_kernel<T, CPL, true, TD>, (size_t)8 * D * sizeof(float));
+            cap_cs = resident_blocks(ln_bwd_kernel<T, CPL, false, TD, true>, (size_t)12 * D * sizeof(float));
+        }
+        cap_plain = resident_blocks(ln_bwd_kernel<T, CPL, false, TD>, (size_t)8 * D * sizeof(float));
         cap_d = D;
     }
-    const int cap = act != M3AE_ACT_NONE ? cap_act : cap_plain;
+    if (colsum && (MIXED || act != M3AE_ACT_NONE)) return M3AE_ERR_UNSUPPORTED;
+    const int cap = colsum ? cap_cs : act != M3AE_ACT_NONE ? cap_act : cap_plain;
     const int nblk = *nblk_io < cap ? *nblk_io : cap;
     *nblk_io = nblk;
     if constexpr (MIXED) {
         if (act != M3AE_ACT_NONE) return M3AE_ERR_UNSUPPORTED;
     }
-    if (act != M3AE_ACT_NONE) {
+    if (colsum) {
+        if constexpr (!MIXED)
+            hipLaunchKernelGGL((ln_bwd_kernel<T, CPL, false, TD, true>), dim3((unsigned)nblk), dim3(256), lds, s,
+                               (const TD*)dy, (const T*)x, g, b, mean, rstd, (T*)dx, (const T*)dx_add, part, M, D, act, rms,
+                               (T*)dx_drop, drop, (bf16_t*)dx_lo);
+    } else if (act != M3AE_ACT_NONE) {
         if constexpr (!MIXED)
             hipLaunchKernelGGL((ln_bwd_kernel<T, CPL, true, TD>), dim3((unsigned)nblk), dim3(256), lds, s,
                                (const TD*)dy, (const T*)x, g, b, mean, rstd, (T*)dx, (const T*)dx_add, part, M, D, act, rms,
@@ -420,14 +611,51 @@
     return hip_launch_status();
 }
 
+template <int NP, bool CS>
+int launch_bwd_pair(const void* dy, const void* x, const float* g, const float* mean, const float* rstd, void* dx, const void* dx_add,
+                    float* part, int* nblk_io, int64_t M, hipStream_t s, void* dx_drop, DropState drop, bool nt) {
+    constexpr size_t lds = (size_t)(4 * (CS ? 3 : 2) + 1) * NP * 256 * sizeof(float);
+    static const int cap = resident_blocks(ln_bwd_pair_kernel<NP, CS, false>, lds);
+    const int64_t want = cdiv((M + 1) / 2, 4);
+    int nblk = *nblk_io < cap ? *nblk_io : cap;
+    if (want < nblk) nblk = (int)want;
+    *nblk_io = nblk;
+    if (nt)
+        hipLaunchKernelGGL((ln_bwd_pair_kernel<NP, CS, true>), dim3((unsigned)nblk), dim3(256), lds, s, (const bf16_t*)dy, (const bf16_t*)x,
+                           g, mean, rstd, (bf16_t*)dx, (const bf16_t*)dx_add, part, M, (bf16_t*)dx_drop, drop);
+    else
+        hipLaunchKernelGGL((ln_bwd_pair_kernel<NP, CS, false>), dim3((unsigned)nblk), dim3(256), lds, s, (const bf16_t*)dy, (const bf16_t*)x,
+                           g, mean, rstd, (bf16_t*)dx, (const bf16_t*)dx_add, part, M, (bf16_t*)dx_drop, drop);
+    return hip_launch_status();
+}
+int try_bwd_pair(const void* dy, const void* x, const float* g, const float* mean, const float* rstd, void* dx, const void* dx_add,
+                 float* part, int* nblk_io, int64_t M, int64_t D, int dtype, int act, int flags, hipStream_t s, void* dx_drop,
+                 DropState drop, bool colsum, int* rc_o) {
+    if (dtype != M3AE_BF16 || act != M3AE_ACT_NONE || (flags & (M3AE_LN_RMS | M3AE_LN_ONE_ROW)) || !mean || D % 256 != 0 || D > 1024 ||
+        drop.row_base != 0 || drop.row_step != 1)
+        return 0;
+    if (M < 32768 && !(flags & M3AE_LN_PAIR_ANY_M)) return 0;
+    if (((((uintptr_t)dy) | ((uintptr_t)x) | ((uintptr_t)dx) | ((uintptr_t)dx_add) | ((uintptr_t)dx_drop) | ((uintptr_t)g)) & 15) != 0) return 0;
+    const bool nt = (flags & M3AE_LN_NT) && M * D * 2 >= ((int64_t)32 << 20);
+#define PAIR_CASE(NP)                                                                                                                  \
+    if (D == NP * 256) {                                                                                                               \
+        *rc_o = colsum ? launch_bwd_pair<NP, true>(dy, x, g, mean, rstd, dx, dx_add, part, nblk_io, M, s, dx_drop, drop, nt)           \
+                       : launch_bwd_pair<NP, false>(dy, x, g, mean, rstd, dx, dx_add, part, nblk_io, M, s, dx_drop, drop, nt);         \
+        return 1;                                                                                                                      \
+    }
+    PAIR_CASE(1) PAIR_CASE(2) PAIR_CASE(3) PAIR_CASE(4)
+#undef PAIR_CASE
+    return 0;
+}
+
 extern "C" int m3ae_layernorm_fwd(const void* x, const float* gamma, const float* beta, void* y, float* mean,
                                   float* rstd, int64_t M, int64_t D, float eps, int dtype, int act, int rms,
                                   void* stream) {
     if (!x || !gamma || !y || M <= 0 || D <= 0) return M3AE_ERR_ARG;
     if (D % 4 != 0 || D > 4096) return M3AE_ERR_UNSUPPORTED;
     hipStream_t s = (hipStream_t)stream;
-    const bool pair_off = (rms & 2) != 0;
-    rms &= 1;
+    const bool pair_off = (rms & M3AE_LN_ONE_ROW) != 0;
+    rms &= M3AE_LN_RMS;
     if (dtype == M3AE_BF16 && act == M3AE_ACT_NONE && !rms && M >= 1024 && ((((uintptr_t)x) | ((uintptr_t)y)) & 15) == 0 &&
         ((((uintptr_t)gamma) | ((uintptr_t)beta)) & 15) == 0 && !pair_off) {
         if (D == 512) return launch_fwd_pair<2>(x, gamma, beta, y, mean, rstd, M, eps, s);
@@ -446,65 +674,93 @@
 
 static int layernorm_bwd_impl(const void* dy, const void* x, const float* gamma, const float* beta, const float* mean,
                               const float* rstd, void* dx, const void* dx_add, float* dgamma, float* dbeta, float* workspace,
-                              int64_t M, int64_t D, int dtype, int act, int rms, void* stream, int det) {
+                              int64_t M, int64_t D, int dtype, int act, int flags, void* stream, int det, bool pair = false,
+                              float* dcol = nullptr) {
     if (!dy || !x || !gamma || !rstd || !dx || !workspace || M <= 0) return M3AE_ERR_ARG;
     if (D % 4 != 0 || D > 2048) return M3AE_ERR_UNSUPPORTED;
+    if (dcol && (det || D > 1024)) return M3AE_ERR_UNSUPPORTED;
     hipStream_t s = (hipStream_t)stream;
+    const int rms = flags & M3AE_LN_RMS;
     int nblk = (int)m3ae_layernorm_bwd_blocks(M);
     int rc = M3AE_ERR_UNSUPPORTED;
     auto run = [&]() -> int {
         if (dtype == M3AE_F32)
-            DISPATCH_CPL(launch_bwd, float, dy, x, gamma, beta, mean, rstd, dx, dx_add, workspace, &nblk, M, (int)D, act, rms, s);
+            DISPATCH_CPL(launch_bwd, float, dy, x, gamma, beta, mean, rstd, dx, dx_add, workspace, &nblk, M, (int)D, act, rms, s, nullptr,
+                         DropState{}, nullptr, dcol != nullptr);
         if (dtype == M3AE_BF16)
-            DISPATCH_CPL(launch_bwd, bf16_t, dy, x, gamma, beta, mean, rstd, dx, dx_add, workspace, &nblk, M, (int)D, act, rms, s);
+            DISPATCH_CPL(launch_bwd, bf16_t, dy, x, gamma, beta, mean, rstd, dx, dx_add, workspace, &nblk, M, (int)D, act, rms, s, nullptr,
+                         DropState{}, nullptr, dcol != nullptr);
         return M3AE_ERR_UNSUPPORTED;
     };
-    rc = run();
+    if (!pair || !try_bwd_pair(dy, x, gamma, mean, rstd, dx, dx_add, workspace, &nblk, M, D, dtype, act, flags, s, nullptr,
+                               DropState{0, 0, 0, 0.f, nullptr, 0, 1}, dcol != nullptr, &rc))
+        rc = run();
     if (rc) return rc;
-    if (!dgamma) return 0;
-    return ln_bwd_fold(workspace, dgamma, dbeta, nblk, (int)D, det, s);
+    return ln_bwd_fold(workspace, dgamma, dbeta, dcol, nblk, (int)D, det, s);
 }
 extern "C" int m3ae_layernorm_bwd(const void* dy, const void* x, const float* gamma, const float* beta,
                                   const float* mean, const float* rstd, void* dx, const void* dx_add, float* dgamma,
                                   float* dbeta, float* workspace, int64_t M, int64_t D, int dtype, int act, int rms,
                                   void* stream) {
-    return layernorm_bwd_impl(dy, x, gamma, beta, mean, rstd, dx, dx_add, dgamma, dbeta, workspace, M, D, dtype, act, rms, stream, 0);
+    return layernorm_bwd_impl(dy, x, gamma, beta, mean, rstd, dx, dx_add, dgamma, dbeta, workspace, M, D, dtype, act, rms, stream, 0, true);
+}
+extern "C" int m3ae_layernorm_bwd_colsum(const void* dy, const void* x, const float* gamma, const float* beta,
+                                         const float* mean, const float* rstd, void* dx, const void* dx_add, float* dgamma,
+                                         float* dbeta, float* dx_colsum, float* workspace, int64_t M, int64_t D, int dtype, int act,
+                                         int flags, void* stream) {
+    return layernorm_bwd_impl(dy, x, gamma, beta, mean, rstd, dx, dx_add, dgamma, dbeta, workspace, M, D, dtype, act, flags, stream, 0, true,
+                              dx_colsum);
 }
 extern "C" int m3ae_layernorm_bwd_det(const void* dy, const void* x, const float* gamma, const float* beta,
                                       const float* mean, const float* rstd, void* dx, const void* dx_add, float* dgamma,
                                       float* dbeta, float* workspace, int64_t M, int64_t D, int dtype, int act, int rms,
                                       void* stream) {
-    return layernorm_bwd_impl(dy, x, gamma, beta, mean, rstd, dx, dx_add, dgamma, dbeta, workspace, M, D, dtype, act, rms, stream, 1);
+    return layernorm_bwd_impl(dy, x, gamma, beta, mean, rstd, dx, dx_add, dgamma, dbeta, workspace, M, D, dtype, act, rms & M3AE_LN_RMS,
+                              stream, 1);
 }
 
 static int layernorm_bwd_drop_impl(const void* dy, const void* x, const float* gamma, const float* beta, const float* mean,
                                    const float* rstd, void* dx, void* dx_drop, float dropout_p, uint64_t dropout_seed,
                                    const void* dropout_salt, float* dgamma, float* dbeta, float* workspace, int64_t M, int64_t D,
-                                   int dtype, void* stream, int det, DropRows rows = DropRows{0, 1}) {
+                                   int dtype, void* stream, int det, DropRows rows = DropRows{0, 1}, bool pair = false, int flags = 0,
+                                   float* dcol = nullptr) {
     if (!dy || !x || !gamma || !rstd || !dx || !dx_drop || !workspace || M <= 0) return M3AE_ERR_ARG;
     if (!drop_rows_ok(rows, M, D)) return M3AE_ERR_ARG;
     if (D % 4 != 0 || D > 2048) return M3AE_ERR_UNSUPPORTED;
+    if (dcol && (det || D > 1024)) return M3AE_ERR_UNSUPPORTED;
     hipStream_t s = (hipStream_t)stream;
     int nblk = (int)m3ae_layernorm_bwd_blocks(M);
     const DropState drop = make_drop(dropout_p, dropout_seed, dropout_salt, rows);
     auto run = [&]() -> int {
         if (dtype == M3AE_F32)
-            DISPATCH_CPL(launch_bwd, float, dy, x, gamma, beta, mean, rstd, dx, nullptr, workspace, &nblk, M, (int)D, 0, 0, s, dx_drop, drop);
+            DISPATCH_CPL(launch_bwd, float, dy, x, gamma, beta, mean, rstd, dx, nullptr, workspace, &nblk, M, (int)D, 0, 0, s, dx_drop, drop,
+                         nullptr, dcol != nullptr);
         if (dtype == M3AE_BF16)
-            DISPATCH_CPL(launch_bwd, bf16_t, dy, x, gamma, beta, mean, rstd, dx, nullptr, workspace, &nblk, M, (int)D, 0, 0, s, dx_drop, drop);
+            DISPATCH_CPL(launch_bwd, bf16_t, dy, x, gamma, beta, mean, rstd, dx, nullptr, workspace, &nblk, M, (int)D, 0, 0, s, dx_drop, drop,
+                         nullptr, dcol != nullptr);
         return M3AE_ERR_UNSUPPORTED;
     };
-    int rc = run();
+    int rc = M3AE_ERR_UNSUPPORTED;
+    if (!pair || !try_bwd_pair(dy, x, gamma, mean, rstd, dx, nullptr, workspace, &nblk, M, D, dtype, M3AE_ACT_NONE, flags, s, dx_drop, drop,
+                               dcol != nullptr, &rc))
+        rc = run();
     if (rc) return rc;
-    if (!dgamma) return 0;
-    return ln_bwd_fold(workspace, dgamma, dbeta, nblk, (int)D, det, s);
+    return ln_bwd_fold(workspace, dgamma, dbeta, dcol, nblk, (int)D, det, s);
 }
 extern "C" int m3ae_layernorm_bwd_drop(const void* dy, const void* x, const float* gamma, const float* beta,
                                        const float* mean, const float* rstd, void* dx, void* dx_drop, float dropout_p,
                                        uint64_t dropout_seed, const void* dropout_salt, float* dgamma, float* dbeta,
                                        float* workspace, int64_t M, int64_t D, int dtype, void* stream) {
     return layernorm_bwd_drop_impl(dy, x, gamma, beta, mean, rstd, dx, dx_drop, dropout_p, dropout_seed, dropout_salt, dgamma, dbeta,
-                                   workspace, M, D, dtype, stream, 0);
+                                   workspace, M, D, dtype, stream, 0, DropRows{0, 1}, true);
+}
+extern "C" int m3ae_layernorm_bwd_drop_colsum(const void* dy, const void* x, const float* gamma, const float* beta,
+                                              const float* mean, const float* rstd, void* dx, void* dx_drop, float dropout_p,
+                                              uint64_t dropout_seed, const void* dropout_salt, float* dgamma, float* dbeta,
+                                              float* dx_colsum, float* workspace, int64_t M, int64_t D, int dtype, int flags,
+                                              void* stream) {
+    return layernorm_bwd_drop_impl(dy, x, gamma, beta, mean, rstd, dx, dx_drop, dropout_p, dropout_seed, dropout_salt, dgamma, dbeta,
+                                   workspace, M, D, dtype, stream, 0, DropRows{0, 1}, true, flags & ~M3AE_LN_RMS, dx_colsum);
 }
 extern "C" int m3ae_layernorm_bwd_drop_rows(const void* dy, const void* x, const float* gamma, const float* beta,
                                             const float* mean, const float* rstd, void* dx, void* dx_drop, float dropout_p,
@@ -546,8 +802,7 @@
     };
     int rc = run();
     if (rc) return rc;
-    if (!dgamma) return 0;
-    return ln_bwd_fold(workspace, dgamma, dbeta, nblk, (int)D, det, s);
+    return ln_bwd_fold(workspace, dgamma, dbeta, nullptr, nblk, (int)D, det, s);
 }
 extern "C" int m3ae_layernorm_bwd_mixed(const void* dy, const float* x, const float* gamma, const float* mean, const float* rstd,
                                         float* dx, const float* dx_add, void* dx_lo, float* dgamma, float* dbeta, float* workspace,
diff --git a/mm-vqa-healthcare_amd/csrc/xattn.hip b/mm-vqa-healthcare_amd/csrc/xattn.hip
--- a/mm-vqa-healthcare_amd/csrc/xattn.hip
+++ b/mm-vqa-healthcare_amd/csrc/xattn.hip
@@ -1153,13 +1153,15 @@
         return M3AE_ERR_ARG;
     const int64_t Mq = (int64_t)B * Lq;
     const void* dsd = d.ws_ds;
+    float* g_bo_ln = d.dir == 1 ? d.g_bo : nullptr;
+    const int ln_flags = ((d.launch_flags & M3AE_XATTN_LN_ONE_ROW) ? M3AE_LN_ONE_ROW : 0) | ((d.launch_flags & M3AE_XATTN_LN_NT) ? M3AE_LN_NT : 0);
     if (drop) {
-        XCHK(m3ae_layernorm_bwd_drop(d.d_out, d.s, d.ln_g, d.ln_b, d.mean, d.rstd, d.ws_ds, d.ws_dsd, d.dropout_p, d.seed_hidden,
-                                     d.dropout_salt, d.g_ln_g, d.g_ln_b, d.ws_ln, Mq, D, M3AE_BF16, stream));
+        XCHK(m3ae_layernorm_bwd_drop_colsum(d.d_out, d.s, d.ln_g, d.ln_b, d.mean, d.rstd, d.ws_ds, d.ws_dsd, d.dropout_p, d.seed_hidden,
+                                            d.dropout_salt, d.g_ln_g, d.g_ln_b, g_bo_ln, d.ws_ln, Mq, D, M3AE_BF16, ln_flags, stream));
         dsd = d.ws_dsd;
     } else {
-        XCHK(m3ae_layernorm_bwd(d.d_out, d.s, d.ln_g, d.ln_b, d.mean, d.rstd, d.ws_ds, nullptr, d.g_ln_g, d.g_ln_b, d.ws_ln, Mq, D,
-                                M3AE_BF16, M3AE_ACT_NONE, 0, stream));
+        XCHK(m3ae_layernorm_bwd_colsum(d.d_out, d.s, d.ln_g, d.ln_b, d.mean, d.rstd, d.ws_ds, nullptr, d.g_ln_g, d.g_ln_b, g_bo_ln, d.ws_ln,
+                                       Mq, D, M3AE_BF16, M3AE_ACT_NONE, ln_flags, stream));
     }
     const bf16_t* Pd = (const bf16_t*)(drop ? d.probs_drop : d.probs);
     const DropState drop_attn = make_drop(d.dropout_p, d.seed_attn, d.dropout_salt);
@@ -1174,7 +1176,6 @@
         bf16_t* dS = (bf16_t*)d.ws_dscores;
         bf16_t* dkv = (bf16_t*)d.ws_dproj;
         float* dcb = d.ws_vec;
-        XCHK(m3ae_colsum(dsd, d.g_bo, Mq, D, D, M3AE_BF16, 1, stream));
         {
             XgArgs a{};
             a.A = (const bf16_t*)dsd; a.lda = D; a.a_sb = (int64_t)I * D;
diff --git a/mm-vqa-healthcare_amd/m3ae_amd/_lib.py b/mm-vqa-healthcare_amd/m3ae_amd/_lib.py
--- a/mm-vqa-healthcare_amd/m3ae_amd/_lib.py
+++ b/mm-vqa-healthcare_amd/m3ae_amd/_lib.py
@@ -57,7 +57,8 @@
 GEMM_NO_PERSISTENT, GEMM_F32_X3, GEMM_DETERMINISTIC = 1, 2, 4
 DET_COLSUM, DET_EMBED_BWD, DET_BCE, DET_XENT, DET_MIM = 0, 1, 2, 3, 4
 ATTN_LEGACY_KERNELS, ATTN_F32_X3 = 1, 2
-XATTN_NO_PERSISTENT, XATTN_LEGACY_CHAIN = 1, 2
+XATTN_NO_PERSISTENT, XATTN_LEGACY_CHAIN, XATTN_LN_ONE_ROW, XATTN_LN_NT = 1, 2, 4, 8
+LN_RMS, LN_ONE_ROW, LN_NT, LN_PAIR_ANY_M = 1, 2, 4, 8
 ABI_VERSION = 4
 
 
@@ -132,6 +133,8 @@
     "m3ae_layernorm_fwd_mixed": (C.c_int, [vp, vp, vp, vp, vp, vp, i64, i64, f32, vp]),
     "m3ae_layernorm_bwd_mixed": (C.c_int, [vp, vp, vp, vp, vp, vp, vp, vp, vp, vp, vp, i64, i64, vp]),
     "m3ae_layernorm_bwd_mixed_det": (C.c_int, [vp, vp, vp, vp, vp, vp, vp, vp, vp, vp, vp, i64, i64, vp]),
+    "m3ae_layernorm_bwd_colsum": (C.c_int, [vp, vp, vp, vp, vp, vp, vp, vp, vp, vp, vp, vp, i64, i64, C.c_int, C.c_int, C.c_int, vp]),
+    "m3ae_layernorm_bwd_drop_colsum": (C.c_int, [vp, vp, vp, vp, vp, vp, vp, vp, f32, C.c_uint64, vp, vp, vp, vp, vp, i64, i64, C.c_int, C.c_int, vp]),
 }
 
 EXPORTS = tuple(_SIGS)
diff --git a/mm-vqa-healthcare_amd/m3ae_amd/ops.py b/mm-vqa-healthcare_amd/m3ae_amd/ops.py
--- a/mm-vqa-healthcare_amd/m3ae_amd/ops.py
+++ b/mm-vqa-healthcare_amd/m3ae_amd/ops.py
@@ -19,6 +19,7 @@
 
 ATTN_LEGACY = os.environ.get("M3AE_ATTN_LEGACY", "0") == "1"
 GEMM_ST_POLICY = int(os.environ.get("M3AE_GEMM_ST_POLICY", 0))
+LN_FLAGS = (_lib.LN_ONE_ROW if os.environ.get("M3AE_LN_PAIR_OFF", "0") == "1" else 0) | (_lib.LN_NT if os.environ.get("M3AE_LN_BWD_NT", "0") == "1" else 0)
 
 
 def _gemm_flags():
@@ -529,7 +530,7 @@
                   "m3ae_layernorm_fwd_mixed")
         else:
             check(_lib.lib().m3ae_layernorm_fwd(_p(xc), _p(gamma), _p(beta), _p(y), _p(mean), _p(rstd), M, D, eps, _dt(xc),
-                                                act, int(rms), _stream()), "m3ae_layernorm_fwd")
+                                                act, int(rms) | LN_FLAGS, _stream()), "m3ae_layernorm_fwd")
         ctx.save_for_backward(xc, mean, rstd)
         ctx.gamma, ctx.beta, ctx.act, ctx.rms = gamma, beta, act, rms
         return y
@@ -553,7 +554,7 @@
         else:
             ln_bwd = L.m3ae_layernorm_bwd_det if _DETERMINISTIC else L.m3ae_layernorm_bwd
             check(ln_bwd(_p(dyc), _p(xc), _p(ctx.gamma), _p(ctx.beta), _p(mean), _p(rstd), _p(dx), None,
-                         _p(gg), _p(gb), _p(ws), M, D, _dt(xc), ctx.act, int(ctx.rms), _stream()),
+                         _p(gg), _p(gb), _p(ws), M, D, _dt(xc), ctx.act, int(ctx.rms) | LN_FLAGS, _stream()),
                   "m3ae_layernorm_bwd")
         _done(ctx.gamma)
         _done(ctx.beta)
@@ -581,16 +582,18 @@
                                                   _stream()), "m3ae_layernorm_fwd_mixed")
         return y, mean, rstd
     check(_lib.lib().m3ae_layernorm_fwd(_p(x2), _p(ln.weight), _p(ln.bias), _p(y), _p(mean), _p(rstd), M, D, ln.eps,
-                                        _dt(x2), act, int(rms), _stream()), "m3ae_layernorm_fwd")
+                                        _dt(x2), act, int(rms) | LN_FLAGS, _stream()), "m3ae_layernorm_fwd")
     return y, mean, rstd
 
 
-def ln_bwd_raw(dy, x2, ln, mean, rstd, dx_add=None, act=ACT_NONE, rms=False, drop=None, rows=None, want_lo=False):
+def ln_bwd_raw(dy, x2, ln, mean, rstd, dx_add=None, act=ACT_NONE, rms=False, drop=None, rows=None, want_lo=False, colsum=None):
     M, D = x2.shape
     L = _lib.lib()
     dx = torch.empty_like(x2)
     nblk = L.m3ae_layernorm_bwd_blocks(M)
-    ws = torch.empty(2 * nblk * D, dtype=torch.float32, device=x2.device)
+    if colsum is not None and (_DETERMINISTIC or rows is not None or dy.dtype != x2.dtype):
+        raise _lib.M3AEHipError("LayerNorm backward: the fused column sum has no ordered, live-row or fp32-stream form")
+    ws = torch.empty((3 if colsum is not None else 2) * nblk * D, dtype=torch.float32, device=x2.device)
     train = ln.weight.requires_grad
     gg = _grad_buf(ln.weight) if train else None
     gb = _grad_buf(ln.bias) if (train and ln.bias is not None) else None
@@ -605,10 +608,14 @@
                 _done(ln.weight)
                 _done(ln.bias)
             return dx, dxd
-        ln_bwd_drop = L.m3ae_layernorm_bwd_drop_det if _DETERMINISTIC else L.m3ae_layernorm_bwd_drop
-        check(ln_bwd_drop(_p(dy), _p(x2), _p(ln.weight), _p(ln.bias), _p(mean), _p(rstd), _p(dx), _p(dxd),
-                          drop[0], drop[1], _salt(), _p(gg), _p(gb), _p(ws), M, D, _dt(x2), _stream()),
-              "m3ae_layernorm_bwd_drop")
+        if _DETERMINISTIC:
+            check(L.m3ae_layernorm_bwd_drop_det(_p(dy), _p(x2), _p(ln.weight), _p(ln.bias), _p(mean), _p(rstd), _p(dx), _p(dxd),
+                                                drop[0], drop[1], _salt(), _p(gg), _p(gb), _p(ws), M, D, _dt(x2), _stream()),
+                  "m3ae_layernorm_bwd_drop_det")
+        else:
+            check(L.m3ae_layernorm_bwd_drop_colsum(_p(dy), _p(x2), _p(ln.weight), _p(ln.bias), _p(mean), _p(rstd), _p(dx), _p(dxd),
+                                                   drop[0], drop[1], _salt(), _p(gg), _p(gb), _p(colsum), _p(ws), M, D, _dt(x2),
+                                                   LN_FLAGS, _stream()), "m3ae_layernorm_bwd_drop_colsum")
         if train:
             _done(ln.weight)
             _done(ln.bias)
@@ -623,9 +630,13 @@
                      _stream()), "m3ae_layernorm_bwd_mixed")
     else:
         assert not want_lo
-        ln_bwd = L.m3ae_layernorm_bwd_det if _DETERMINISTIC else L.m3ae_layernorm_bwd
-        check(ln_bwd(_p(dy), _p(x2), _p(ln.weight), _p(ln.bias), _p(mean), _p(rstd), _p(dx), _p(dx_add),
-                     _p(gg), _p(gb), _p(ws), M, D, _dt(x2), act, int(rms), _stream()), "m3ae_layernorm_bwd")
+        if _DETERMINISTIC:
+            check(L.m3ae_layernorm_bwd_det(_p(dy), _p(x2), _p(ln.weight), _p(ln.bias), _p(mean), _p(rstd), _p(dx), _p(dx_add),
+                                           _p(gg), _p(gb), _p(ws), M, D, _dt(x2), act, int(rms), _stream()), "m3ae_layernorm_bwd_det")
+        else:
+            check(L.m3ae_layernorm_bwd_colsum(_p(dy), _p(x2), _p(ln.weight), _p(ln.bias), _p(mean), _p(rstd), _p(dx), _p(dx_add),
+                                              _p(gg), _p(gb), _p(colsum), _p(ws), M, D, _dt(x2), act, int(rms) | LN_FLAGS, _stream()),
+                  "m3ae_layernorm_bwd_colsum")
     if train:
         _done(ln.weight)
         _done(ln.bias)
@@ -813,6 +824,7 @@
         d.dropout_p, d.seed_attn, d.seed_hidden = pdrop, seeds[0], seeds[1]
         d.dropout_salt = _salt()
     d.launch_flags = (_lib.XATTN_NO_PERSISTENT if NT_NO_PERSISTENT else 0) | (_lib.XATTN_LEGACY_CHAIN if XATTN_LEGACY_CHAIN else 0)
+    d.launch_flags |= (_lib.XATTN_LN_ONE_ROW if LN_FLAGS & _lib.LN_ONE_ROW else 0) | (_lib.XATTN_LN_NT if LN_FLAGS & _lib.LN_NT else 0)
     return d
 
 
@@ -911,7 +923,7 @@
     L_ = _lib.lib()
     w = {"ws_ds": e(B * L, D), "ws_dscores": torch.empty_like(t["probs"]), "ws_dprime": torch.empty_like(t["prime"]),
          "ws_dproj": torch.empty_like(t["proj"]), "ws_vec": e(3 * B * H * min(L, Lo), dt=torch.float32),
-         "ws_ln": e(2 * L_.m3ae_layernorm_bwd_blocks(B * L) * D, dt=torch.float32)}
+         "ws_ln": e(3 * L_.m3ae_layernorm_bwd_blocks(B * L) * D, dt=torch.float32)}
     if pdrop > 0:
         w["ws_dsd"] = e(B * L, D)
     if d.dir == 0:
```
